# weiaicunzai/pytorch-camvid

Measured on AMD Instinct MI355X. Metric: images/sec fwd+bwd UNet 3x360x480 bs=8, higher is better.
Workload: dtype f32; 1 GPU; UNET(3,12) train fwd+bwd+CE, per-GPU batch 8 x 3x360x480 fp32 (BASELINE.json configs[1]); global_batch=8, parallelism=dp1

## Files before the change

include/cvk.h:

```cpp
#ifndef CVK_H
#define CVK_H

#include <stddef.h>
#include <stdint.h>

#ifdef __cplusplus
extern "C" {
#endif

#define CVK_VERSION 100
#define CVK_OK 0
#define CVK_EINVAL (-1)
#define CVK_EWORKSPACE (-2)
#define CVK_STAT_ROWS 64

typedef struct cvk_view {
    float*  ptr;
    int64_t sN, sY, sX;
} cvk_view;

typedef struct cvk_viewh {
    void*   ptr;
    int64_t sN, sY, sX;
} cvk_viewh;

int         cvk_version(void);
uint64_t    cvk_abi_hash(void);
const char* cvk_last_error_string(void);

int cvk_import_nchw(const float* src, int64_t sN, int64_t sC, int64_t sH, int64_t sW,
                    float* dst, int ld, int N, int C, int H, int W, void* stream);
int cvk_export_nchw(const float* src, int ld, float* dst, int64_t dN, int64_t dC, int64_t dH, int64_t dW,
                    int N, int C, int H, int W, void* stream);
int cvk_zero_frame(cvk_view buf, int N, int H, int W, int C, int y0, int x0, int h, int w, void* stream);

int cvk_conv3x3_fwd(const float* x, const float* w, const float* bias, float* y, float* stats,
                    int N, int H, int W, int Cin, int Cout, int ldy, void* stream);
int cvk_pack_weight_fwd(const float* w_src, float* dst, int Cout, int Cin, int Cin_pad, void* stream);
int cvk_pack_weight_dgrad(const float* w_src, float* dst, int Cout, int Cin, int Cin_pad, int Cout_pad, void* stream);
size_t cvk_conv3x3_wgrad_workspace_bytes(int N, int H, int W, int Cin_pad, int Cout);
int cvk_conv3x3_wgrad(const float* x, const float* dy, float* dw, int N, int H, int W, int Cin, int Cin_pad,
                      int Cout, int ld_dy, void* workspace, size_t workspace_bytes, void* stream);

int cvk_wino_weight_transform(const float* w, float* U, int Cout, int Cin, void* stream);
size_t cvk_conv3x3_wino_workspace_bytes(int N, int H, int W, int Cout_ld);
int cvk_conv3x3_wino_gemm(const float* x, const float* U, float* Mo, int N, int H, int W, int Cin, int Cout, int ldm,
                          void* stream);
int cvk_wino_output(const float* Mo, const float* bias, float* y, float* stats, int N, int H, int W, int Cout, int ldy,
                    void* stream);

int cvk_wino4_weight_transform(const float* w, float* U, int Cout, int Cin, void* stream);
int cvk_wino4_weight_transform_dgrad(const float* w, float* U, int Cout, int Cin, void* stream);
int cvk_conv3x3_wino4_ksplit(int N, int H, int W, int Cin, int Cout_ld);
size_t cvk_conv3x3_wino4_workspace_bytes(int N, int H, int W, int Cin, int Cout_ld);
int cvk_conv3x3_wino4_gemm(const float* x, const float* U, float* Mo, int N, int H, int W, int Cin, int Cout, int ldm,
                           void* stream);
int cvk_wino4_output(const float* Mo, const float* bias, float* y, float* stats, int N, int H, int W, int Cout, int ldy,
                     int ksplit, void* stream);

int cvk_w2d_tiles(int N, int H, int W);
int cvk_w2d_tpad(int T);
int cvk_w2d_stat_partials(int N, int H, int W);
size_t cvk_conv3x3_w2d_workspace_bytes(int N, int H, int W, int Cin, int Cout);
int cvk_w2d_weight_transform(const float* w, float* U, int Cout, int Cin, void* stream);
int cvk_w2d_weight_transform_dgrad(const float* w, float* U, int Cout, int Cin, void* stream);
int cvk_conv3x3_w2d(const float* x, const float* U, const float* bias, float* y, float* stats, float* counts, int N, int H,
                    int W, int Cin, int Cout, int ldy, void* workspace, size_t workspace_bytes, void* stream);
int cvk_w2d_ksplit(int T, int Cin, int Cout);
int cvk_w2d_input_transform(const float* x, float* V, int N, int H, int W, int Cin, void* stream);
int cvk_w2d_gemm(const float* V, const float* U, float* Mo, int T, int Cin, int Cout, void* stream);
int cvk_w2d_output(const float* Mo, const float* bias, float* y, float* stats, float* counts, int N, int H, int W, int Cin,
                   int Cout, int ldy, void* stream);
size_t cvk_conv3x3_wgrad_w2d_workspace_bytes(int N, int H, int W, int Cin_pad, int Cout);
int cvk_conv3x3_wgrad_w2d(const float* x, const float* dy, float* dw, int N, int H, int W, int Cin, int Cin_pad, int Cout,
                          int ld_dy, void* workspace, size_t workspace_bytes, void* stream);
int cvk_w2d_wgrad_ksplit(int T, int Cin_pad, int Cout);
int cvk_w2d_dy_transform(const float* dy, int ld_dy, float* E, int N, int H, int W, int Cout, void* stream);
int cvk_w2d_dy_transform_both(const float* dy, int ld_dy, float* Vp, float* E, int N, int H, int W, int Cout, void* stream);
int cvk_w2d_gemm_tn(const float* E, const float* V, float* P, int T, int Cin_pad, int Cout, void* stream);
int cvk_w2d_wgrad_output(const float* P, float* dw, int T, int Cin, int Cin_pad, int Cout, void* stream);

int cvk_w6_tiles(int N, int H, int W);
int cvk_w6_stat_partials(int N, int H, int W);
size_t cvk_conv3x3_w6_workspace_bytes(int N, int H, int W, int Cin, int Cout);
int cvk_w6_weight_transform(const float* w, float* U, int Cout, int Cin, void* stream);
int cvk_w6_weight_transform_dgrad(const float* w, float* U, int Cout, int Cin, void* stream);
int cvk_w6_ksplit(int T, int Cin, int Cout);
int cvk_w6_input_transform(const float* x, float* V, int N, int H, int W, int Cin, void* stream);
int cvk_w6_gemm(const float* V, const float* U, float* Mo, int T, int Cin, int Cout, void* stream);
int cvk_w6_output(const float* Mo, const float* bias, float* y, float* stats, float* counts, int N, int H, int W, int Cin,
                  int Cout, int ldy, void* stream);
int cvk_w6_wgrad_ksplit(int T, int Cin_pad, int Cout);
int cvk_w6_dy_transform(const float* dy, int ld_dy, float* E, int N, int H, int W, int Cout, void* stream);
int cvk_w6_dy_transform_both(const float* dy, int ld_dy, float* Vp, float* E, int N, int H, int W, int Cout, void* stream);
int cvk_w6_gemm_tn(const float* E, const float* V, float* P, int T, int Cin_pad, int Cout, void* stream);
int cvk_split3_rows_pad(int R, int mult);
int cvk_split3_planes(const float* P, void* S, int NX, int R, int Rpad, int C, void* stream);
int cvk_w2d_gemm_split3(const void* V3, const void* U3, float* Mo, int NX, int T, int Tpad, int Cin, int Cout, int Cpad, void* stream);
int cvk_amax_block_words(void);
unsigned cvk_amax_block_value(const unsigned* host_words, int n);
int cvk_absmax_f32(const float* x, long rows, int C, int ld, void* amax_block, void* stream);
int cvk_split_scale_exponent(int tile, int kind, int xi, unsigned amax_block);
int cvk_split_planes(int fmt, int tile, int kind, const float* P, void* S, const void* amax, int NX, int R, int Rpad, int C, void* stream);
int cvk_w2d_gemm_split(int fmt, int tile, const void* V, const void* U, float* Mo, const void* amax_v, const void* amax_u, int NX, int T, int Tpad,
                       int Cin, int Cout, int Cpad, void* stream);
int cvk_w2d_input_transform_split3(int tile, const float* x, void* V3, int N, int H, int W, int Cin, void* stream);
int cvk_w2d_dy_transform_both_split3(int tile, const float* dy, int ld_dy, void* Vp3, void* E, int e_split, int N, int H, int W, int C,
                                     void* stream);
int cvk_w2d_weight_transform_split3(int tile, const float* w, void* U3, float* tmp, int Cout, int Cin, int dgrad, void* stream);
int cvk_w2d_input_transform_split(int fmt, int tile, const float* x, void* V, const void* amax_x, int N, int H, int W, int Cin, void* stream);
int cvk_w2d_dy_transform_both_split(int fmt, int tile, const float* dy, int ld_dy, void* Vp, void* E, int e_split, const void* amax_dy, int N, int H,
                                    int W, int C, void* stream);
int cvk_w2d_weight_transform_split(int fmt, int tile, const float* w, void* U, const void* amax_w, int Cout, int Cin, int dgrad, void* stream);
int cvk_w2d_output_plain(int tile, const float* Mo, const float* bias, float* y, float* stats, float* counts, int N, int H, int W,
                         int Cout, int ldy, void* stream);
int cvk_w2d_gemm_tn_split3_ksplit(int NX, int Tpad, int Cin, int Cout);
int cvk_w2d_gemm_tn_split3(const void* E3, const void* V3, float* P, int NX, int Tpad, int Cin, int Cout, void* stream);
int cvk_w2d_gemm_tn_split(int fmt, int tile, const void* E, const void* V, float* P, const void* amax_e, const void* amax_v, int NX, int Tpad, int Cin,
                          int Cout, void* stream);
int cvk_w2d_wgrad_output_f(int tile, const float* P, float* dw, int Cin, int Cin_pad, int Cout, int f, void* stream);
int cvk_w6_wgrad_output(const float* P, float* dw, int T, int Cin, int Cin_pad, int Cout, void* stream);
int cvk_wino4h_weight_transform(const float* w, void* Uh, const void* amax_w, int Cn, int Ck, int dgrad, void* stream);
int cvk_conv3x3_wino4h(const float* x, const void* Uh, const float* bias, float* y, float* stats, float* counts, const void* amax_x,
                       const void* amax_w, int N, int H, int W, int Cin, int Cout, int ldy, int max_workgroups, void* stream);
int cvk_conv3x3_wino4h_bnred(const float* x, const void* Uh, float* y, const void* amax_x, const void* amax_w, int N, int H, int W, int Cin,
                             int Cout, int ldy, const float* yP, const float* scale, const float* shift, const float* mean,
                             const float* rstd, float* part, int max_workgroups, void* stream);
size_t cvk_wino4f_weight_floats(int Cn, int Ck);
int cvk_wino4f_weight_transform(const float* w, float* Uf, int Cn, int Ck, int dgrad, void* stream);
#define CVK_WT_BATCH_MAX 48
typedef struct cvk_wt_job { const float* w; float* out; int rows, cols, tile, dgrad; } cvk_wt_job;
int cvk_wino4f_weight_transform_batch(const cvk_wt_job* jobs, int n, void* stream);
int cvk_w2d_weight_transform_batch(const cvk_wt_job* jobs, int n, void* stream);
int cvk_wino4f_stat_partials(int N, int H, int W);
int cvk_conv3x3_wino4f_vplanes(const float* x, const float* Uf, const float* bias, float* y, float* stats, float* counts, float* Vsm,
                               int N, int H, int W, int Cin, int Cout, int ldy, int max_workgroups, void* stream);
int cvk_conv3x3_wino4f(const float* x, const float* Uf, const float* bias, float* y, float* stats, float* counts, int N, int H,
                       int W, int Cin, int Cout, int ldy, int max_workgroups, void* stream);
int cvk_conv3x3_wino4f_bnred(const float* x, const float* Uf, float* y, int N, int H, int W, int Cin, int Cout, int ldy,
                             const float* yP, const float* scale, const float* shift, const float* mean, const float* rstd,
                             float* part, int max_workgroups, void* stream);

int cvk_thin_fwd_supported(int Cin_ld, int Cout, int ldy);
int cvk_thin_stat_partials(int N, int H, int W, int Cin_ld);
int cvk_conv3x3_thin_fwd(const float* x, const float* w, const float* bias, float* y, float* stats, float* counts, int N, int H,
                         int W, int Cin_ld, int Cout, int ldy, void* stream);
int cvk_thin_wgrad_supported(int Cin, int Cin_ld, int Cout, int ld_dy);
size_t cvk_conv3x3_thin_wgrad_workspace_bytes(int N, int H, int W, int Cin_ld, int Cout);
int cvk_conv3x3_thin_wgrad(const float* x, const float* dy, float* dw, int N, int H, int W, int Cin, int Cin_ld, int Cout,
                           int ld_dy, void* workspace, size_t workspace_bytes, void* stream);

size_t cvk_conv3x3_wgradp_workspace_bytes(int N, int H, int W, int Cin_pad, int Cout);
int cvk_conv3x3_wgradp(const float* x, const float* dy, const float* E6_pre, float* dw, int N, int H, int W, int Cin, int Cin_pad,
                       int Cout, int ld_dy, void* workspace, size_t workspace_bytes, void* stream);
long cvk_wgradp_plane_rows(int N, int H, int W);
int cvk_wgradp_planes(const float* t, int ld, float* planes, int N, int H, int W, int C, int is_dy, void* stream);
size_t cvk_wgradp_gemm_workspace_bytes(int N, int H, int W, int Cin_pad, int Cout);
int cvk_wgradp_gemm(const float* E6, const float* V6, float* dw, int N, int H, int W, int Cin, int Cin_pad, int Cout, void* workspace,
                    size_t workspace_bytes, void* stream);
int cvk_wgradp_zero_pads(float* planes, int N, int H, int W, int C, void* stream);
int cvk_wgradp_zero_pads_sm(float* planes, int N, int H, int W, int C, void* stream);
int cvk_wgradp_planes_sm(const float* x, int ld, float* planes, int N, int H, int W, int C, void* stream);
int cvk_wgradp_gemm_sm(const float* E6, const float* V6sm, float* dw, int N, int H, int W, int Cin, int Cin_pad, int Cout, void* workspace,
                       size_t workspace_bytes, void* stream);
int cvk_wgradp_zero_pads4(float* planes, int N, int H, int W, int C, void* stream);
int cvk_bn_bwd_dx_e4p(cvk_view dout, const float* y, int ldy, const float* scale, const float* shift, const float* mean,
                      const float* rstd, const float* dgamma, const float* dbeta, float* dy, int ld_dy, float* E4p, float* part,
                      int N, int H, int W, int C, int use_batch_stats, void* stream);
int cvk_wgradp_dy_slack(int W);
int cvk_wgradp_gemm_sm_dy(const float* E4p, const float* dy, const float* V6sm, float* dw, int N, int H, int W, int Cin, int Cin_pad, int Cout,
                          void* workspace, size_t workspace_bytes, void* stream);
int cvk_bn_bwd_dx_e6(cvk_view dout, const float* y, int ldy, const float* scale, const float* shift, const float* mean,
                     const float* rstd, const float* dgamma, const float* dbeta, float* dy, int ld_dy, float* E6, float* part,
                     int N, int H, int W, int C, int use_batch_stats, void* stream);

size_t cvk_conv3x3_wgrad_wino4_workspace_bytes(int N, int H, int W, int Cin_pad, int Cout, int ld_dy);
int cvk_conv3x3_wgrad_wino4(const float* x, const float* dy, const float* E_pre, float* dw, int N, int H, int W, int Cin,
                            int Cin_pad, int Cout, int ld_dy, void* workspace, size_t workspace_bytes, void* stream);
int cvk_bn_bwd_e_blocks(int N, int H, int W);
int cvk_bn_bwd_dx_e(cvk_view dout, const float* y, int ldy, const float* scale, const float* shift, const float* mean,
                    const float* rstd, const float* dgamma, const float* dbeta, float* dy, int ld_dy, float* E, float* part,
                    int N, int H, int W, int C, int use_batch_stats, void* stream);

size_t cvk_conv3x3_wgrad_wino_workspace_bytes(int N, int H, int W, int Cin_pad, int Cout);
int cvk_conv3x3_wgrad_wino(const float* x, const float* dy, float* dw, int N, int H, int W, int Cin, int Cin_pad,
                           int Cout, int ld_dy, void* workspace, size_t workspace_bytes, void* stream);

size_t cvk_bn_finalize_workspace_bytes(int P, int C);
int cvk_bn_finalize(const float* stats, int P, int M, int C, const float* gamma, const float* beta,
                    float* mean, float* rstd, float* scale, float* shift,
                    float* running_mean, float* running_var, int64_t* num_batches_tracked,
                    float momentum, float eps, void* workspace, size_t workspace_bytes, void* stream);
int cvk_bn_eval_params(const float* gamma, const float* beta, const float* running_mean, const float* running_var,
                       float* mean, float* rstd, float* scale, float* shift, int C, float eps, void* stream);
int cvk_bn_relu_apply(const float* y, int ldy, const float* scale, const float* shift, cvk_view out,
                      int N, int H, int W, int C, void* stream);
int cvk_bn_relu_apply_pool(const float* y, int ldy, const float* scale, const float* shift, cvk_view out, float* pool,
                           unsigned char* code, int N, int H, int W, int C, void* stream);
int cvk_bn_bwd_blocks(int M);
int cvk_bn_bwd_reduce(cvk_view dout, const float* y, int ldy, const float* scale, const float* shift,
                      const float* mean, const float* rstd, float* part, int N, int H, int W, int C, void* stream);
int cvk_colsum_finalize(const float* part, int PB, int C, float* out0, float* out1, void* stream);
#define CVK_COLSUM_BATCH_MAX 64
typedef struct cvk_colsum_job { const float* part; float* out; int PB, C; } cvk_colsum_job;
int cvk_colsum_finalize_batch(const cvk_colsum_job* jobs, int n, void* stream);
int cvk_bn_relu_apply_amax(const float* y, int ldy, const float* scale, const float* shift, cvk_view out, int N, int H, int W, int C,
                           void* amax_block, void* stream);
int cvk_bn_relu_apply_pool_amax(const float* y, int ldy, const float* scale, const float* shift, cvk_view out, float* pool,
                                unsigned char* code, int N, int H, int W, int C, void* amax_out, void* amax_pool, void* stream);
int cvk_bn_bwd_dx_e_amax(int six, cvk_view dout, const float* y, int ldy, const float* scale, const float* shift, const float* mean,
                         const float* rstd, const float* dgamma, const float* dbeta, float* dy, int ld_dy, float* E, float* part, int N, int H,
                         int W, int C, int use_batch_stats, void* amax_block, void* stream);
int cvk_bn_bwd_dx_amax(cvk_view dout, const float* y, int ldy, const float* scale, const float* shift, const float* mean,
                       const float* rstd, const float* dgamma, const float* dbeta, float* dy, int ld_dy, float* dbias_part, int N,
                       int H, int W, int C, int use_batch_stats, void* amax_block, void* stream);
int cvk_bn_bwd_dx(cvk_view dout, const float* y, int ldy, const float* scale, const float* shift,
                  const float* mean, const float* rstd, const float* dgamma, const float* dbeta,
                  float* dy, int ld_dy, float* dbias_part, int N, int H, int W, int C, int use_batch_stats, void* stream);

int cvk_maxpool2x2_fwd(cvk_view x, float* out, uint8_t* code, int N, int H, int W, int C, void* stream);
int cvk_maxpool2x2_bwd(const float* dout, cvk_view x, const uint8_t* code, cvk_view dx, int accumulate,
                       int N, int H, int W, int C, void* stream);
int cvk_maxpool2x2_bwd_bnred_blocks(int N, int H, int W, int C);
int cvk_maxpool2x2_bwd_bnred(const float* dout, cvk_view x, const uint8_t* code, cvk_view dx, int accumulate, int N, int H, int W, int C,
                             const float* yP, int ldp, const float* scale, const float* shift, const float* mean, const float* rstd,
                             float* part, void* stream);
int cvk_maxunpool2x2_fwd(const float* v, const uint8_t* code, float* out, int N, int H, int W, int C, void* stream);
int cvk_maxunpool2x2_bwd(const float* dout, const uint8_t* code, float* dv, int N, int H, int W, int C, void* stream);
int cvk_pool_code_to_index(const uint8_t* code, int64_t* idx, int N, int H, int W, int C, void* stream);

int cvk_bilinear_up2_fwd(const float* x, float* out, int N, int H, int W, int C, void* stream);
int cvk_bilinear_up2_bwd(const float* dout, float* dx, int N, int H, int W, int C, void* stream);

int cvk_ce_blocks(int M);
int cvk_softmax_ce_fwd(const float* logits, int ld, const int64_t* target, float* part, float* loss,
                       int M, int C, int ignore_index, void* stream);
int cvk_softmax_ce_bwd(const float* logits, int ld, const int64_t* target, const float* loss3, const float* grad_out,
                       float scale, float* dlogits, int ld_d, int M, int C, int ignore_index, void* stream);

#define CVK_REDUCTION_NONE 0
#define CVK_REDUCTION_MEAN 1
#define CVK_REDUCTION_SUM 2
int cvk_ce_ex_part_floats(int M);
int cvk_softmax_ce_fwd_ex(const float* logits, int ld, const int64_t* target, const float* weight, float label_smoothing,
                          int reduction, float* part, float* loss, float* loss_px, int M, int C, int ignore_index, void* stream);
int cvk_softmax_ce_bwd_ex(const float* logits, int ld, const int64_t* target, const float* weight, float label_smoothing,
                          int reduction, const float* loss4, const float* grad_out, float scale, float* dlogits, int ld_d,
                          int M, int C, int ignore_index, void* stream);

#define CVK_DICE_PRESENT 0
#define CVK_DICE_ALL 1
int cvk_seg_loss_part_floats(int M, int C);
int cvk_seg_loss_record_floats(int C);
int cvk_seg_loss_fwd(const float* logits, int ld, const int64_t* target, const float* weight, float ce, float dice, float focal_gamma,
// ... 208 lines not shown
```

pytorch-camvid_amd/_lib.py:

```python
import ctypes
import os
import subprocess
import threading

_HERE = os.path.dirname(os.path.abspath(__file__))
LIB_PATH = os.environ.get("CVK_LIB_PATH") or os.path.join(_HERE, "lib", "libcvk.so")
CSRC = os.path.join(_HERE, "csrc")
HEADER = os.path.join(os.path.dirname(_HERE), "include", "cvk.h")

CVK_STAT_ROWS = 64

c_f32p = ctypes.c_void_p
c_i64 = ctypes.c_int64
c_int = ctypes.c_int
c_size = ctypes.c_size_t
c_float = ctypes.c_float
c_vp = ctypes.c_void_p


class View(ctypes.Structure):
    _fields_ = [("ptr", ctypes.c_void_p), ("sN", ctypes.c_int64), ("sY", ctypes.c_int64), ("sX", ctypes.c_int64)]


class ViewH(ctypes.Structure):
    _fields_ = [("ptr", ctypes.c_void_p), ("sN", ctypes.c_int64), ("sY", ctypes.c_int64), ("sX", ctypes.c_int64)]


SIGNATURES = {
    "cvk_version": (c_int, []),
    "cvk_abi_hash": (ctypes.c_uint64, []),
    "cvk_last_error_string": (ctypes.c_char_p, []),
    "cvk_import_nchw": (c_int, [c_vp, c_i64, c_i64, c_i64, c_i64, c_vp, c_int, c_int, c_int, c_int, c_int, c_vp]),
    "cvk_export_nchw": (c_int, [c_vp, c_int, c_vp, c_i64, c_i64, c_i64, c_i64, c_int, c_int, c_int, c_int, c_vp]),
    "cvk_zero_frame": (c_int, [View, c_int, c_int, c_int, c_int, c_int, c_int, c_int, c_int, c_vp]),
    "cvk_conv3x3_fwd": (c_int, [c_vp, c_vp, c_vp, c_vp, c_vp, c_int, c_int, c_int, c_int, c_int, c_int, c_vp]),
    "cvk_pack_weight_fwd": (c_int, [c_vp, c_vp, c_int, c_int, c_int, c_vp]),
    "cvk_pack_weight_dgrad": (c_int, [c_vp, c_vp, c_int, c_int, c_int, c_int, c_vp]),
    "cvk_conv3x3_wgrad_workspace_bytes": (c_size, [c_int, c_int, c_int, c_int, c_int]),
    "cvk_conv3x3_wgrad": (c_int, [c_vp, c_vp, c_vp, c_int, c_int, c_int, c_int, c_int, c_int, c_int, c_vp, c_size, c_vp]),
    "cvk_wino_weight_transform": (c_int, [c_vp, c_vp, c_int, c_int, c_vp]),
    "cvk_conv3x3_wino_workspace_bytes": (c_size, [c_int, c_int, c_int, c_int]),
    "cvk_conv3x3_wino_gemm": (c_int, [c_vp, c_vp, c_vp, c_int, c_int, c_int, c_int, c_int, c_int, c_vp]),
    "cvk_wino_output": (c_int, [c_vp, c_vp, c_vp, c_vp, c_int, c_int, c_int, c_int, c_int, c_vp]),
    "cvk_wino4_weight_transform": (c_int, [c_vp, c_vp, c_int, c_int, c_vp]),
    "cvk_wino4_weight_transform_dgrad": (c_int, [c_vp, c_vp, c_int, c_int, c_vp]),
    "cvk_conv3x3_wino4_ksplit": (c_int, [c_int, c_int, c_int, c_int, c_int]),
    "cvk_conv3x3_wino4_workspace_bytes": (c_size, [c_int, c_int, c_int, c_int, c_int]),
    "cvk_conv3x3_wino4_gemm": (c_int, [c_vp, c_vp, c_vp, c_int, c_int, c_int, c_int, c_int, c_int, c_vp]),
    "cvk_wino4_output": (c_int, [c_vp, c_vp, c_vp, c_vp, c_int, c_int, c_int, c_int, c_int, c_int, c_vp]),
    "cvk_wino4f_weight_floats": (c_size, [c_int, c_int]),
    "cvk_wino4f_weight_transform": (c_int, [c_vp, c_vp, c_int, c_int, c_int, c_vp]),
    "cvk_wino4f_weight_transform_batch": (c_int, [c_vp, c_int, c_vp]),
    "cvk_w2d_weight_transform_batch": (c_int, [c_vp, c_int, c_vp]),
    "cvk_wino4f_stat_partials": (c_int, [c_int, c_int, c_int]),
    "cvk_conv3x3_wino4f": (c_int, [c_vp, c_vp, c_vp, c_vp, c_vp, c_vp, c_int, c_int, c_int, c_int, c_int, c_int, c_int, c_vp]),
    "cvk_conv3x3_wino4f_bnred": (c_int, [c_vp, c_vp, c_vp, c_int, c_int, c_int, c_int, c_int, c_int, c_vp, c_vp, c_vp, c_vp, c_vp, c_vp, c_int, c_vp]),
    "cvk_wino4h_weight_transform": (c_int, [c_vp, c_vp, c_vp, c_int, c_int, c_int, c_vp]),
    "cvk_conv3x3_wino4h": (c_int, [c_vp, c_vp, c_vp, c_vp, c_vp, c_vp, c_vp, c_vp, c_int, c_int, c_int, c_int, c_int, c_int, c_int, c_vp]),
    "cvk_conv3x3_wino4h_bnred": (c_int, [c_vp, c_vp, c_vp, c_vp, c_vp, c_int, c_int, c_int, c_int, c_int, c_int, c_vp, c_vp, c_vp, c_vp, c_vp, c_vp,
                                         c_int, c_vp]),
    "cvk_thin_fwd_supported": (c_int, [c_int, c_int, c_int]),
    "cvk_thin_stat_partials": (c_int, [c_int, c_int, c_int, c_int]),
    "cvk_conv3x3_thin_fwd": (c_int, [c_vp, c_vp, c_vp, c_vp, c_vp, c_vp, c_int, c_int, c_int, c_int, c_int, c_int, c_vp]),
    "cvk_thin_wgrad_supported": (c_int, [c_int, c_int, c_int, c_int]),
    "cvk_conv3x3_thin_wgrad_workspace_bytes": (c_size, [c_int, c_int, c_int, c_int, c_int]),
    "cvk_conv3x3_thin_wgrad": (c_int, [c_vp, c_vp, c_vp, c_int, c_int, c_int, c_int, c_int, c_int, c_int, c_vp, c_size, c_vp]),
    "cvk_conv3x3_wgradp_workspace_bytes": (c_size, [c_int, c_int, c_int, c_int, c_int]),
    "cvk_conv3x3_wgradp": (c_int, [c_vp, c_vp, c_vp, c_vp, c_int, c_int, c_int, c_int, c_int, c_int, c_int, c_vp, c_size, c_vp]),
    "cvk_wgradp_plane_rows": (ctypes.c_long, [c_int, c_int, c_int]),
    "cvk_wgradp_planes": (c_int, [c_vp, c_int, c_vp, c_int, c_int, c_int, c_int, c_int, c_vp]),
    "cvk_wgradp_gemm_workspace_bytes": (c_size, [c_int, c_int, c_int, c_int, c_int]),
    "cvk_wgradp_gemm": (c_int, [c_vp, c_vp, c_vp, c_int, c_int, c_int, c_int, c_int, c_int, c_vp, c_size, c_vp]),
    "cvk_wgradp_zero_pads": (c_int, [c_vp, c_int, c_int, c_int, c_int, c_vp]),
    "cvk_wgradp_zero_pads_sm": (c_int, [c_vp, c_int, c_int, c_int, c_int, c_vp]),
    "cvk_wgradp_planes_sm": (c_int, [c_vp, c_int, c_vp, c_int, c_int, c_int, c_int, c_vp]),
    "cvk_wgradp_gemm_sm": (c_int, [c_vp, c_vp, c_vp, c_int, c_int, c_int, c_int, c_int, c_int, c_vp, c_size, c_vp]),
    "cvk_wgradp_zero_pads4": (c_int, [c_vp, c_int, c_int, c_int, c_int, c_vp]),
    "cvk_bn_bwd_dx_e4p": (c_int, [View, c_vp, c_int, c_vp, c_vp, c_vp, c_vp, c_vp, c_vp, c_vp, c_int, c_vp, c_vp,
                                  c_int, c_int, c_int, c_int, c_int, c_vp]),
    "cvk_wgradp_dy_slack": (c_int, [c_int]),
    "cvk_wgradp_gemm_sm_dy": (c_int, [c_vp, c_vp, c_vp, c_vp, c_int, c_int, c_int, c_int, c_int, c_int, c_vp, c_size, c_vp]),
    "cvk_conv3x3_wino4f_vplanes": (c_int, [c_vp, c_vp, c_vp, c_vp, c_vp, c_vp, c_vp, c_int, c_int, c_int, c_int, c_int, c_int, c_int, c_vp]),
    "cvk_bn_bwd_dx_e6": (c_int, [View, c_vp, c_int, c_vp, c_vp, c_vp, c_vp, c_vp, c_vp, c_vp, c_int, c_vp, c_vp,
                                 c_int, c_int, c_int, c_int, c_int, c_vp]),
    "cvk_w2d_tiles": (c_int, [c_int, c_int, c_int]),
    "cvk_w6_tiles": (c_int, [c_int, c_int, c_int]),
    "cvk_w6_stat_partials": (c_int, [c_int, c_int, c_int]),
    "cvk_conv3x3_w6_workspace_bytes": (c_size, [c_int, c_int, c_int, c_int, c_int]),
    "cvk_w6_weight_transform": (c_int, [c_vp, c_vp, c_int, c_int, c_vp]),
    "cvk_w6_weight_transform_dgrad": (c_int, [c_vp, c_vp, c_int, c_int, c_vp]),
    "cvk_w6_input_transform": (c_int, [c_vp, c_vp, c_int, c_int, c_int, c_int, c_vp]),
    "cvk_w6_gemm": (c_int, [c_vp, c_vp, c_vp, c_int, c_int, c_int, c_vp]),
    "cvk_w6_wgrad_ksplit": (c_int, [c_int, c_int, c_int]),
    "cvk_w6_dy_transform": (c_int, [c_vp, c_int, c_vp, c_int, c_int, c_int, c_int, c_vp]),
    "cvk_w6_gemm_tn": (c_int, [c_vp, c_vp, c_vp, c_int, c_int, c_int, c_vp]),
    "cvk_w6_wgrad_output": (c_int, [c_vp, c_vp, c_int, c_int, c_int, c_int, c_vp]),
    "cvk_w6_ksplit": (c_int, [c_int, c_int, c_int]),
    "cvk_w6_output": (c_int, [c_vp, c_vp, c_vp, c_vp, c_vp, c_int, c_int, c_int, c_int, c_int, c_int, c_vp]),
    "cvk_w2d_stat_partials": (c_int, [c_int, c_int, c_int]),
    "cvk_conv3x3_w2d_workspace_bytes": (c_size, [c_int, c_int, c_int, c_int, c_int]),
    "cvk_w2d_weight_transform": (c_int, [c_vp, c_vp, c_int, c_int, c_vp]),
    "cvk_w2d_weight_transform_dgrad": (c_int, [c_vp, c_vp, c_int, c_int, c_vp]),
    "cvk_w2d_input_transform": (c_int, [c_vp, c_vp, c_int, c_int, c_int, c_int, c_vp]),
    "cvk_w2d_gemm": (c_int, [c_vp, c_vp, c_vp, c_int, c_int, c_int, c_vp]),
    "cvk_conv3x3_wgrad_w2d_workspace_bytes": (c_size, [c_int, c_int, c_int, c_int, c_int]),
    "cvk_conv3x3_wgrad_w2d": (c_int, [c_vp, c_vp, c_vp, c_int, c_int, c_int, c_int, c_int, c_int, c_int, c_vp, c_size, c_vp]),
    "cvk_w2d_tpad": (c_int, [c_int]),
    "cvk_split3_rows_pad": (c_int, [c_int, c_int]),
    "cvk_split3_planes": (c_int, [c_vp, c_vp, c_int, c_int, c_int, c_int, c_vp]),
    "cvk_w2d_gemm_split3": (c_int, [c_vp, c_vp, c_vp, c_int, c_int, c_int, c_int, c_int, c_int, c_vp]),
    "cvk_w2d_input_transform_split3": (c_int, [c_int, c_vp, c_vp, c_int, c_int, c_int, c_int, c_vp]),
    "cvk_w2d_dy_transform_both_split3": (c_int, [c_int, c_vp, c_int, c_vp, c_vp, c_int, c_int, c_int, c_int, c_int, c_vp]),
    "cvk_w2d_weight_transform_split3": (c_int, [c_int, c_vp, c_vp, c_vp, c_int, c_int, c_int, c_vp]),
    "cvk_w2d_output_plain": (c_int, [c_int, c_vp, c_vp, c_vp, c_vp, c_vp, c_int, c_int, c_int, c_int, c_int, c_vp]),
    "cvk_w2d_gemm_tn_split3_ksplit": (c_int, [c_int, c_int, c_int, c_int]),
    "cvk_w2d_gemm_tn_split3": (c_int, [c_vp, c_vp, c_vp, c_int, c_int, c_int, c_int, c_vp]),
    "cvk_amax_block_words": (c_int, []),
    "cvk_amax_block_value": (ctypes.c_uint, [c_vp, c_int]),
    "cvk_absmax_f32": (c_int, [c_vp, ctypes.c_long, c_int, c_int, c_vp, c_vp]),
    "cvk_split_scale_exponent": (c_int, [c_int, c_int, c_int, ctypes.c_uint]),
    "cvk_split_planes": (c_int, [c_int, c_int, c_int, c_vp, c_vp, c_vp, c_int, c_int, c_int, c_int, c_vp]),
    "cvk_w2d_gemm_split": (c_int, [c_int, c_int, c_vp, c_vp, c_vp, c_vp, c_vp, c_int, c_int, c_int, c_int, c_int, c_int, c_vp]),
    "cvk_w2d_input_transform_split": (c_int, [c_int, c_int, c_vp, c_vp, c_vp, c_int, c_int, c_int, c_int, c_vp]),
    "cvk_w2d_dy_transform_both_split": (c_int, [c_int, c_int, c_vp, c_int, c_vp, c_vp, c_int, c_vp, c_int, c_int, c_int, c_int, c_vp]),
    "cvk_w2d_weight_transform_split": (c_int, [c_int, c_int, c_vp, c_vp, c_vp, c_int, c_int, c_int, c_vp]),
    "cvk_w2d_gemm_tn_split": (c_int, [c_int, c_int, c_vp, c_vp, c_vp, c_vp, c_vp, c_int, c_int, c_int, c_int, c_vp]),
    "cvk_w2d_wgrad_output_f": (c_int, [c_int, c_vp, c_vp, c_int, c_int, c_int, c_int, c_vp]),
    "cvk_w2d_wgrad_ksplit": (c_int, [c_int, c_int, c_int]),
    "cvk_w2d_dy_transform": (c_int, [c_vp, c_int, c_vp, c_int, c_int, c_int, c_int, c_vp]),
    "cvk_w2d_dy_transform_both": (c_int, [c_vp, c_int, c_vp, c_vp, c_int, c_int, c_int, c_int, c_vp]),
    "cvk_w6_dy_transform_both": (c_int, [c_vp, c_int, c_vp, c_vp, c_int, c_int, c_int, c_int, c_vp]),
    "cvk_w2d_gemm_tn": (c_int, [c_vp, c_vp, c_vp, c_int, c_int, c_int, c_vp]),
    "cvk_w2d_wgrad_output": (c_int, [c_vp, c_vp, c_int, c_int, c_int, c_int, c_vp]),
    "cvk_w2d_ksplit": (c_int, [c_int, c_int, c_int]),
    "cvk_w2d_output": (c_int, [c_vp, c_vp, c_vp, c_vp, c_vp, c_int, c_int, c_int, c_int, c_int, c_int, c_vp]),
    "cvk_conv3x3_w2d": (c_int, [c_vp, c_vp, c_vp, c_vp, c_vp, c_vp, c_int, c_int, c_int, c_int, c_int, c_int, c_vp, c_size, c_vp]),
    "cvk_conv3x3_wgrad_wino4_workspace_bytes": (c_size, [c_int, c_int, c_int, c_int, c_int, c_int]),
    "cvk_conv3x3_wgrad_wino4": (c_int, [c_vp, c_vp, c_vp, c_vp, c_int, c_int, c_int, c_int, c_int, c_int, c_int, c_vp, c_size, c_vp]),
    "cvk_bn_bwd_e_blocks": (c_int, [c_int, c_int, c_int]),
    "cvk_bn_bwd_dx_e": (c_int, [View, c_vp, c_int, c_vp, c_vp, c_vp, c_vp, c_vp, c_vp, c_vp, c_int, c_vp, c_vp,
                                c_int, c_int, c_int, c_int, c_int, c_vp]),
    "cvk_conv3x3_wgrad_wino_workspace_bytes": (c_size, [c_int, c_int, c_int, c_int, c_int]),
    "cvk_conv3x3_wgrad_wino": (c_int, [c_vp, c_vp, c_vp, c_int, c_int, c_int, c_int, c_int, c_int, c_int, c_vp, c_size, c_vp]),
    "cvk_bn_finalize_workspace_bytes": (c_size, [c_int, c_int]),
    "cvk_bn_finalize": (c_int, [c_vp, c_int, c_int, c_int, c_vp, c_vp, c_vp, c_vp, c_vp, c_vp, c_vp, c_vp, c_vp,
                                c_float, c_float, c_vp, c_size, c_vp]),
    "cvk_bn_eval_params": (c_int, [c_vp, c_vp, c_vp, c_vp, c_vp, c_vp, c_vp, c_vp, c_int, c_float, c_vp]),
    "cvk_bn_relu_apply": (c_int, [c_vp, c_int, c_vp, c_vp, View, c_int, c_int, c_int, c_int, c_vp]),
    "cvk_bn_relu_apply_pool": (c_int, [c_vp, c_int, c_vp, c_vp, View, c_vp, c_vp, c_int, c_int, c_int, c_int, c_vp]),
    "cvk_bn_bwd_blocks": (c_int, [c_int]),
    "cvk_bn_bwd_reduce": (c_int, [View, c_vp, c_int, c_vp, c_vp, c_vp, c_vp, c_vp, c_int, c_int, c_int, c_int, c_vp]),
    "cvk_colsum_finalize": (c_int, [c_vp, c_int, c_int, c_vp, c_vp, c_vp]),
    "cvk_colsum_finalize_batch": (c_int, [c_vp, c_int, c_vp]),
    "cvk_bn_bwd_dx": (c_int, [View, c_vp, c_int, c_vp, c_vp, c_vp, c_vp, c_vp, c_vp, c_vp, c_int, c_vp,
                              c_int, c_int, c_int, c_int, c_int, c_vp]),
    "cvk_bn_relu_apply_amax": (c_int, [c_vp, c_int, c_vp, c_vp, View, c_int, c_int, c_int, c_int, c_vp, c_vp]),
    "cvk_bn_relu_apply_pool_amax": (c_int, [c_vp, c_int, c_vp, c_vp, View, c_vp, c_vp, c_int, c_int, c_int, c_int, c_vp, c_vp, c_vp]),
    "cvk_bn_bwd_dx_e_amax": (c_int, [c_int, View, c_vp, c_int, c_vp, c_vp, c_vp, c_vp, c_vp, c_vp, c_vp, c_int, c_vp, c_vp,
                                     c_int, c_int, c_int, c_int, c_int, c_vp, c_vp]),
    "cvk_bn_bwd_dx_amax": (c_int, [View, c_vp, c_int, c_vp, c_vp, c_vp, c_vp, c_vp, c_vp, c_vp, c_int, c_vp,
                                   c_int, c_int, c_int, c_int, c_int, c_vp, c_vp]),
    "cvk_maxpool2x2_fwd": (c_int, [View, c_vp, c_vp, c_int, c_int, c_int, c_int, c_vp]),
    "cvk_maxpool2x2_bwd": (c_int, [c_vp, View, c_vp, View, c_int, c_int, c_int, c_int, c_int, c_vp]),
    "cvk_maxpool2x2_bwd_bnred_blocks": (c_int, [c_int, c_int, c_int, c_int]),
# ... 227 lines not shown
```

pytorch-camvid_amd/conv_fp32.py:

```python
import torch

from . import _lib
from ._lib import check
from .engine import _BF16, _F32, Op, Saved, _empty, _timed, amax_blocks, channels_last
from .route import pad4


def w2fn(lib, tile, name):
    return getattr(lib, ("cvk_w6_" if tile == 6 else "cvk_w2d_") + name)


_PLANE_DT = {0: _F32, 2: torch.float16, 3: _BF16}


def planes2d(lib, tile, N, H, W, fmt=0):
    T = w2fn(lib, tile, "tiles")(N, H, W)
    return 64 if tile == 6 else 36, T, lib.cvk_split3_rows_pad(T, 256) if fmt else lib.cvk_w2d_tpad(T)


def plane_elems(NX, Tp, C, fmt=0):
    return NX * (C // 32) * fmt * Tp * 32 if fmt else NX * Tp * C + 128


def absmax(R, t, rows, cols, ld, s, what):
# ... 114 lines not shown
        return (P2, cnt) if self.sp is not None else None

    def w4f(self, vplanes=False, bnred=None, h2=False, x_amax=None):
        R, lib, s, x, d, wt = self.R, self.lib, self.s, self.x, self.dgrad_of, self.wt
        N, H, W, M, k_ch, cout, ldy, flops = self.N, self.H, self.W, self.M, self.k_ch, self.cout, self.ldy, self.flops
        floats, dg, f = lib.cvk_wino4f_weight_floats(cout, k_ch), int(d is not None), "h" if h2 else "f"
        am_w = self._amax_w() if h2 else None

        def build():
            u, name = _empty(floats, x.device), "cvk_wino4%s_weight_transform" % f
            _timed(R, "k_wino4%s_weight" % f, 4.0 * (9 + 18) * cout * k_ch, lambda: check(getattr(lib, name)(
                wt.data_ptr(), u.data_ptr(), *((am_w.data_ptr(),) if h2 else ()), cout, k_ch, dg, s), name + ("(dgrad)" if dg and not h2 else "")), "byte")
            return u
        U = self._filter("w4" + f, build, None if h2 else ("w4f", floats, cout, k_ch, 0, dg))
        am = ()
        if h2:
            am_x = x_amax if x_amax is not None else absmax(R, x, M, k_ch, k_ch, s, "x")
            am = (am_x.data_ptr(), am_w.data_ptr())
        executed = (1.5 if h2 else 0.5) * flops
        Pf = lib.cvk_wino4f_stat_partials(N, H, W)
        cnt = self._counts(Pf)
        if bnred is not None:
            bpart = _empty(2 * Pf * cout, x.device)
            name = "cvk_conv3x3_wino4%s_bnred" % f
            _timed(R, "k_conv3x3_wino4%s<bnred>" % f, flops, lambda: check(getattr(lib, name)(
                x.data_ptr(), U.data_ptr(), self.y.data_ptr(), *am, N, H, W, k_ch, cout, ldy, *bnred, bpart.data_ptr(), R.launch_wgs(), s), name), executed=executed)
            self.bnred_sums = (bpart, Pf)
            return None
        if vplanes:
            self.v = _empty(6 * lib.cvk_wgradp_plane_rows(N, H, W) * k_ch, x.device)
            check(lib.cvk_wgradp_zero_pads_sm(self.v.data_ptr(), N, H, W, k_ch, s), "cvk_wgradp_zero_pads_sm")
            _timed(R, "k_conv3x3_wino4f<vplanes>", flops, lambda: check(
                lib.cvk_conv3x3_wino4f_vplanes(x.data_ptr(), U.data_ptr(), self.bias, self.y.data_ptr(), self.sp, cnt, self.v.data_ptr(), N, H, W,
                                               k_ch, cout, ldy, R.launch_wgs(), s), "cvk_conv3x3_wino4f_vplanes" + self.what), executed=executed)
        else:
            name = "cvk_conv3x3_wino4" + f
            _timed(R, "k_conv3x3_wino4" + f, flops, lambda: check(getattr(lib, name)(
                x.data_ptr(), U.data_ptr(), self.bias, self.y.data_ptr(), self.sp, cnt, *am, N, H, W, k_ch, cout, ldy, R.launch_wgs(), s),
                name + self.what), executed=executed)
        return (Pf, cnt) if self.sp is not None else None

    def w4(self):
        R, lib, s, x, d = self.R, self.lib, self.s, self.x, self.dgrad_of
        N, H, W, M, k_ch, cout, ldy = self.N, self.H, self.W, self.M, self.k_ch, self.cout, self.ldy

        dg = d is not None and d[1] == k_ch and d[2] == cout

        def build():
            u, wt = _empty(6 * cout * 3 * k_ch, x.device), d[0] if dg else (self.w() if callable(self.w) else self.w)
            kind = "weight_transform_dgrad" if dg else "weight_transform"
            _timed(R, "k_wino4_weight_dgrad" if dg else "k_wino4_weight", 4.0 * (9 + 18) * cout * k_ch, lambda: check(getattr(lib, "cvk_wino4_" + kind)(
                wt.data_ptr(), u.data_ptr(), *((d[1], d[2]) if dg else (cout, k_ch)), s), "cvk_wino4_" + kind), "byte")
            return u
        U = self._filter("w4", build)
        ws = R.workspace(lib.cvk_conv3x3_wino4_workspace_bytes(N, H, W, k_ch, ldy), x.device)
        ksplit = lib.cvk_conv3x3_wino4_ksplit(N, H, W, k_ch, ldy)
        _timed(R, conv_kernel_name("wino4", ldy), self.flops, lambda: check(
            lib.cvk_conv3x3_wino4_gemm(x.data_ptr(), U.data_ptr(), ws.data_ptr(), N, H, W, k_ch, cout, ldy, s), "cvk_conv3x3_wino4_gemm" + self.what))
        _timed(R, "k_wino4_output", (4.0 + 6.0 * ksplit) * M * ldy, lambda: check(
            lib.cvk_wino4_output(ws.data_ptr(), self.bias, self.y.data_ptr(), self.sp, N, H, W, cout, ldy, ksplit, s), "cvk_wino4_output"), "byte")

    def w2(self):
        R, lib, s, x = self.R, self.lib, self.s, self.x
        N, H, W, M, k_ch, cout, ldy = self.N, self.H, self.W, self.M, self.k_ch, self.cout, self.ldy

        def build():
            wt = self.w() if callable(self.w) else self.w
            u = _empty(4 * cout * 3 * k_ch, x.device)
            _timed(R, "k_wino_weight", 4.0 * (9 + 12) * cout * k_ch, lambda: check(
                lib.cvk_wino_weight_transform(wt.data_ptr(), u.data_ptr(), cout, k_ch, s), "cvk_wino_weight_transform"), "byte")
            return u
        U = self._filter("w", build)
        ws = R.workspace(lib.cvk_conv3x3_wino_workspace_bytes(N, H, W, ldy), x.device)
        _timed(R, conv_kernel_name("wino", ldy), self.flops, lambda: check(
            lib.cvk_conv3x3_wino_gemm(x.data_ptr(), U.data_ptr(), ws.data_ptr(), N, H, W, k_ch, cout, ldy, s), "cvk_conv3x3_wino_gemm" + self.what))
        _timed(R, "k_wino_output", 12.0 * M * ldy, lambda: check(
            lib.cvk_wino_output(ws.data_ptr(), self.bias, self.y.data_ptr(), self.sp, N, H, W, cout, ldy, s), "cvk_wino_output"), "byte")


class WeightGrad:

    def __init__(self, R, s, x, dy, gw, N, H, W, cin, k_ch, cout, ldy, flops):
        self.R, self.lib, self.s, self.x, self.dy, self.gw = R, R.lib, s, x, dy, gw
        self.N, self.H, self.W, self.M, self.cin, self.k_ch, self.cout, self.ldy, self.flops = N, H, W, N * H * W, cin, k_ch, cout, ldy, flops

    def run(self, fam, tile=0, fmt=0, V=None, am_v=None, E=None, dy_e=False, Eb=None, am_dy=None):
        if fam == "w2d":
            return self.w2d(tile, V, Eb)
        if fam == "w2d_split":
            return self.w2d_split(tile, fmt, V, am_v, Eb, am_dy)
        if fam in ("wgradp", "wgradp_sm"):
            return self.wgradp(fam == "wgradp", V, E, dy_e and E is not None)
        return self.w4(E) if fam == "w4" else self.direct(fam)

    def w2d(self, tile, V, Eb):
        R, lib, s, x, dy = self.R, self.lib, self.s, self.x, self.dy
        N, H, W, M, k_ch, C, ldy = self.N, self.H, self.W, self.M, self.k_ch, self.cout, self.ldy
        NX, T, Tp = planes2d(lib, tile, N, H, W)
        efl = plane_elems(NX, Tp, C)
        f = w2fn(lib, tile, "wgrad_ksplit")(T, k_ch, C)
        if V is None:
            V = _empty(plane_elems(NX, Tp, k_ch), x.device)
            _timed(R, "k_w2d_input", 4.0 * (M + NX * T) * k_ch, lambda: check(
                w2fn(lib, tile, "input_transform")(x.data_ptr(), V.data_ptr(), N, H, W, k_ch, s), "cvk_w2d_input_transform(wgrad)"), "byte")
        ws = R.workspace(4 * ((0 if Eb is not None else efl) + f * NX * C * k_ch), x.device)
        Ep, Pp = (Eb.data_ptr(), ws.data_ptr()) if Eb is not None else (ws.data_ptr(), ws.data_ptr() + 4 * efl)
        if Eb is None:
            _timed(R, "k_w2d_dy", 4.0 * (M + NX * T) * C, lambda: check(
                w2fn(lib, tile, "dy_transform")(dy.data_ptr(), ldy, Ep, N, H, W, C, s), "cvk_w2d_dy_transform"), "byte")
        _timed(R, "k_w2d_gemm_tn", self.flops, lambda: check(
            w2fn(lib, tile, "gemm_tn")(Ep, V.data_ptr(), Pp, T, k_ch, C, s), "cvk_w2d_gemm_tn"), executed=2.0 * NX * Tp * k_ch * C)
        _timed(R, "k_w2d_wgrad_out", 4.0 * (NX * f + 9) * C * self.cin, lambda: check(
            w2fn(lib, tile, "wgrad_output")(Pp, self.gw, T, self.cin, k_ch, C, s), "cvk_w2d_wgrad_output"), "byte")

    def w2d_split(self, tile, fmt, V, am_v, Eb, am_dy):
        R, lib, s, k_ch, C = self.R, self.lib, self.s, self.k_ch, self.cout
        NX, _, Tp = planes2d(lib, tile, self.N, self.H, self.W, fmt)
        f = lib.cvk_w2d_gemm_tn_split3_ksplit(NX, Tp, k_ch, C)
        ws = R.workspace(4 * f * NX * C * k_ch, self.x.device)
        _timed(R, "k_gemm_tn_" + ("split3" if fmt == 3 else "split2h"), self.flops, lambda: check(
            lib.cvk_w2d_gemm_tn_split(fmt, tile, Eb.data_ptr(), V.data_ptr(), ws.data_ptr(), am_dy.data_ptr() if am_dy is not None else None,
                                      am_v.data_ptr() if am_v is not None else None, NX, Tp, k_ch, C, s), "cvk_w2d_gemm_tn_split"),
            executed=2.0 * (6 if fmt == 3 else 3) * NX * Tp * k_ch * C)
        _timed(R, "k_w2d_wgrad_out", 4.0 * (NX * f + 9) * C * self.cin, lambda: check(
            lib.cvk_w2d_wgrad_output_f(tile, ws.data_ptr(), self.gw, self.cin, k_ch, C, f, s), "cvk_w2d_wgrad_output_f"), "byte")

    def wgradp(self, own_v, V, E, sm_dy):
        R, lib, s, x, dy = self.R, self.lib, self.s, self.x, self.dy
        N, H, W, M, k_ch, C, ldy = self.N, self.H, self.W, self.M, self.k_ch, self.cout, self.ldy
        rows6 = lib.cvk_wgradp_plane_rows(N, H, W)
        wsb = lib.cvk_wgradp_gemm_workspace_bytes(N, H, W, k_ch, C)
        nE = 0 if E is not None else 6 * rows6 * C
        nV = 6 * rows6 * k_ch if own_v else 0
        ws = R.workspace(4 * (nV + nE) + wsb, x.device)
        V6p = ws.data_ptr() if own_v else V.data_ptr()
        E6p = E.data_ptr() if E is not None else ws.data_ptr() + 4 * nV
        slabp = ws.data_ptr() + 4 * (nV + nE)
        if own_v:
            _timed(R, "k_wgradp_planes", 4.0 * (M + 6.0 * rows6) * k_ch, lambda: check(
                lib.cvk_wgradp_planes(x.data_ptr(), k_ch, V6p, N, H, W, k_ch, 0, s), "cvk_wgradp_planes(x)"), "byte")
        if E is None:
            _timed(R, "k_wgradp_planes", 4.0 * (M + 6.0 * rows6) * C, lambda: check(
                lib.cvk_wgradp_planes(dy.data_ptr(), ldy, E6p, N, H, W, C, 1, s), "cvk_wgradp_planes(dy)"), "byte")
        fn = "cvk_wgradp_gemm_sm_dy" if sm_dy else ("cvk_wgradp_gemm" if own_v else "cvk_wgradp_gemm_sm")
        ev = (E6p, dy.data_ptr(), V6p) if sm_dy else (E6p, V6p)
        _timed(R, "k_wgradp_gemm", self.flops, lambda: check(getattr(lib, fn)(*ev, self.gw, N, H, W, self.cin, k_ch, C, slabp, wsb, s), fn),
               executed=9.0 * M * C * self.cin)

    def w4(self, E):
        R, lib, N, H, W, k_ch, C, ldy = self.R, self.lib, self.N, self.H, self.W, self.k_ch, self.cout, self.ldy
        wsb = lib.cvk_conv3x3_wgrad_wino4_workspace_bytes(N, H, W, k_ch, C, ldy)
        ws = R.workspace(wsb, self.x.device)
        _timed(R, f"k_wgrad_wino4<{'128' if C > 64 else '64'}, 128, 2, 2>", self.flops, lambda: check(
            lib.cvk_conv3x3_wgrad_wino4(self.x.data_ptr(), self.dy.data_ptr(), E.data_ptr() if E is not None else None, self.gw, N, H, W,
                                        self.cin, k_ch, C, ldy, ws.data_ptr(), wsb, self.s), "cvk_conv3x3_wgrad_wino4"))

    def direct(self, fam):
        R, lib, N, H, W, M, k_ch, C, ldy = self.R, self.lib, self.N, self.H, self.W, self.M, self.k_ch, self.cout, self.ldy
        fn = {"thin": "cvk_conv3x3_thin_wgrad", "w2": "cvk_conv3x3_wgrad_wino", "direct": "cvk_conv3x3_wgrad"}[fam]
        wsb = getattr(lib, fn + "_workspace_bytes")(N, H, W, k_ch, C)
        ws = R.workspace(wsb, self.x.device)
        head = k_ch == 64
        name, kw = {"thin": ("k_thin_co_wgrad" if head else "k_thin_ci_wgrad",
                             dict(executed=18.0 * M * (16 * self.cin if head else C * 16 / 3.0), nbytes=4.0 * M * (k_ch + ldy))),
                    "w2": (f"k_wgrad_wino<{'128' if C > 64 else '64'}, 128, 2, 2>", {}), "direct": (conv_kernel_name("wgrad", C, k_ch), {})}[fam]
        _timed(R, name, self.flops, lambda: check(getattr(lib, fn)(
            self.x.data_ptr(), self.dy.data_ptr(), self.gw, N, H, W, self.cin, k_ch, C, ldy, ws.data_ptr(), wsb, self.s), fn), **kw)


def conv_kernel_name(kind, n_cols, k_ch=32):
    if kind in ("wino4", "wino"):
        return "k_conv3x3_%s<%s>" % (kind, "128, 128, 2, 2" if n_cols > 64 else ("128, 64, 2, 2" if n_cols > 32 else "128, 32, 4, 1"))
    if kind == "wgrad":
        if n_cols <= 16 and k_ch == 64:
            return "k_wgrad_smallco"
        t = "128, 128, 2, 2" if n_cols > 64 else ("64, 128, 2, 2" if n_cols > 32 else "32, 256, 1, 4")
        if 32 < n_cols <= 64 and k_ch * 9 <= 64:
            t = "64, 64, 2, 2"
        return f"k_conv3x3_wgrad<{t}>"
    t = "128, 128, 2, 2" if n_cols > 64 else ("128, 64, 2, 2" if n_cols > 32 else "256, 32, 4, 1")
    return f"k_conv3x3_igemm<{t}, {'true' if kind == 'fwd' else 'false'}, {'true' if k_ch % 32 == 0 else 'false'}>"


class ConvBnRelu(Op):
    _pitch, _ydt = staticmethod(pad4), _F32
# ... 121 lines not shown
            P, Pw = self._stat_partials(R, wk)
            stats = _empty(2 * Pw * C + Pw, dev)
        counted, kept = self._conv(R, st, rt, st.act[src.id], wk, b, y, stats, P)
        self._bn_params(R, st, stats, counted, P, Pw, gamma, beta, ptrs)
        self._bn_apply(R, st, y, ptrs[2], ptrs[3])
        if st.need_grad and self.active:
            st.saved[self.idx] = Saved(y, bnp, rt, kept)

    def _bn_sums(self, R, st, bn, gg, gbe):
        lib, s, src, C, (blocks, fn, name) = R.lib, st.stream, self.src, self.cout, self._BN
        PB = getattr(lib, blocks)(src.M)
        part = _empty(2 * PB * C, st.device)
        pre = st.bnred.pop(self.idx, None)
        if pre is not None:
            check(lib.cvk_colsum_finalize(pre[0].data_ptr(), pre[1], C, gbe, gg, s), "cvk_colsum_finalize")
        elif self.bn_train or self.g_req or self.be_req:
            _timed(R, name, float(self.dst.buf.esize + self._ydt.itemsize) * src.M * C, lambda: check(
                getattr(lib, fn)(*bn, part.data_ptr(), src.N, src.H, src.W, C, s), fn), "byte")
            check(lib.cvk_colsum_finalize(part.data_ptr(), PB, C, gbe, gg, s), "cvk_colsum_finalize")
        if self.w_req or self.b_req or self.src_needs_grad:
            return part, PB
        R.grads_ready(st, self.pslot)
        return None

    _BN_E = {"dx+E": (0, "cvk_bn_bwd_dx_e", 16.0), "dx+E6": (1, "cvk_bn_bwd_dx_e6", 24.0), "dx+E4p": (2, "cvk_bn_bwd_dx_e4p", 16.0)}

    def _bn_bwd(self, R, st, rt, bn, gg, gbe, part, PB, gb):
        lib, s, src, kind = R.lib, st.stream, self.src, rt.bn_bwd
        N, H, W, M, C, ldy = src.N, src.H, src.W, src.M, self.cout, pad4(self.cout)
        if kind == "dx+E4p":
            dyb = _empty(M * ldy + lib.cvk_wgradp_dy_slack(W) * ldy, st.device)
            dyb[M * ldy:].zero_()
            dy = dyb[:M * ldy]
        else:
            dy = torch.zeros(M * ldy, device=st.device, dtype=_F32) if ldy != C else _empty(M * ldy, st.device)
        want_amax = rt.dy_amax and bool(st.amax_spare)
        head, tail = (*bn, gg, gbe, dy.data_ptr(), ldy), (part.data_ptr(), N, H, W, C, 1 if self.bn_train else 0)
        if kind != "dx":
            mode, plain, eb = self._BN_E[kind]
            if kind == "dx+E":
                E = _empty(4 * N * H * ((W + 3) // 4) * ldy, st.device)
            else:
                E = _empty((4 if mode == 2 else 6) * lib.cvk_wgradp_plane_rows(N, H, W) * C, st.device)
                check((lib.cvk_wgradp_zero_pads4 if mode == 2 else lib.cvk_wgradp_zero_pads)(E.data_ptr(), N, H, W, C, s), "cvk_wgradp_zero_pads")
            blk = st.amax_spare[-1] if want_amax else None
            rc = _timed(R, "k_bn_bwd<%s>" % kind, (12.0 * M + eb * N * H * ((W + 3) // 4)) * C, lambda: (
                lib.cvk_bn_bwd_dx_e_amax(mode, *head, E.data_ptr(), *tail, blk.data_ptr(), s) if blk is not None
                else getattr(lib, plain)(*head, E.data_ptr(), *tail, s)), "byte")
            if rc == 0:
                if gb is not None:
                    R.defer_colsum(st, part, lib.cvk_bn_bwd_e_blocks(N, H, W), C, gb)
                return dy, E, (st.amax_spare.pop() if blk is not None else None)
        am = st.amax_spare.pop() if want_amax else None
        _timed(R, "k_bn_bwd<dx>", 12.0 * M * C, lambda: check(amax_call(lib, "cvk_bn_bwd_dx", (*head, *tail), (am,), s), "cvk_bn_bwd_dx"), "byte")
        if gb is not None:
            R.defer_colsum(st, part, PB, C, gb)
        return dy, None, am

    def _dy_both(self, R, st, rt, dy, am_dy):
        if rt is None or not rt.dy_both:
            return None, None, am_dy
        lib, s, src = R.lib, st.stream, self.src
        N, H, W, M, C, ldy = src.N, src.H, src.W, src.M, self.cout, pad4(self.cout)
        tile, fmt = rt.tile, rt.split
        NX, T, Tp = planes2d(lib, tile, N, H, W, fmt)
        Eb, Vb = (torch.empty(plane_elems(NX, Tp, C, fmt), device=st.device, dtype=_PLANE_DT[fmt]) for _ in range(2))
        if fmt:
            if fmt == 2 and am_dy is None:
                am_dy = absmax(R, dy, M, C, ldy, s, "dy")
            _timed(R, "k_w2d_dy<both,%s>" % ("split3" if fmt == 3 else "split2h"), (4.0 * M + 4.0 * fmt * NX * T) * C, lambda: check(
                lib.cvk_w2d_dy_transform_both_split(fmt, tile, dy.data_ptr(), ldy, Vb.data_ptr(), Eb.data_ptr(), 1,
                                                    am_dy.data_ptr() if am_dy is not None else None, N, H, W, C, s), "cvk_w2d_dy_transform_both_split"), "byte")
        else:
            _timed(R, "k_w2d_dy<both>", 4.0 * (M + 2 * NX * T) * C, lambda: check(
                w2fn(lib, tile, "dy_transform_both")(dy.data_ptr(), ldy, Vb.data_ptr(), Eb.data_ptr(), N, H, W, C, s), "cvk_w2d_dy_transform_both"), "byte")
        return Eb, Vb, am_dy

    def _data_grad(self, R, st, rt, dy, Vb, am_dy):
        lib, s, src = R.lib, st.stream, self.src
        N, H, W, M, C, ldy, dev = src.N, src.H, src.W, src.M, self.cout, pad4(self.cout), st.device
        flops = 18.0 * M * C * self.cin
        if src.id in st.grad:
            raise NotImplementedError("conv data-grad must be the first writer of its input's gradient buffer")
        w = st.params[4 * self.pslot]
        wc = channels_last(w)

        def packed():
            wd_ = _empty(src.ld * 9 * ldy, dev)
            _timed(R, "k_pack_weight_dgrad", 4.0 * 9 * (C * self.cin + src.ld * ldy), lambda: check(
                lib.cvk_pack_weight_dgrad(wc.data_ptr(), wd_.data_ptr(), C, self.cin, src.ld, ldy, s), "cvk_pack_weight_dgrad"), "byte")
            return wd_
        dX = _empty(M * src.ld, dev).view(N, H, W, src.ld)
        wd = R.derived(((self.pslot, "d"), "pack"), w, packed) if rt.dgrad in ("thin", "direct") else None
        if rt.dgrad == "thin":
            _timed(R, "k_thin_ci_fwd(dgrad)", flops, lambda: check(
                lib.cvk_conv3x3_thin_fwd(dy.data_ptr(), wd.data_ptr(), None, dX.data_ptr(), None, None, N, H, W, ldy, src.ld, src.ld, s),
                "cvk_conv3x3_thin_fwd(dgrad)"), executed=18.0 * M * ldy * src.ld, nbytes=4.0 * M * (src.ld + ldy))
        elif rt.dgrad == "direct":
            _timed(R, conv_kernel_name("dgrad", src.ld, ldy), flops, lambda: check(
                lib.cvk_conv3x3_fwd(dy.data_ptr(), wd.data_ptr(), None, dX.data_ptr(), None, N, H, W, ldy, src.ld, src.ld, s), "cvk_conv3x3_fwd(dgrad)"))
        else:
            prod = st.plan.sole_producer(src) if rt.dgrad_bnred else None
            bnred = None
            if prod is not None and prod.bn_train and prod.idx in st.saved and pad4(prod.cout) == prod.cout == src.ld:
                bnred = st.saved[prod.idx].pointers(src.ld)
            c = WinoConv(R, s, dy, packed, None, dX, None, N, H, W, ldy, src.ld, src.ld, flops, w, (self.pslot, "d"), "(dgrad)", dgrad_of=(wc, C, self.cin))
            c.run(rt.dgrad, rt.dgrad_tile, rt.split, v_pre=Vb, x_amax=am_dy, bnred=bnred)
            if c.bnred_sums is not None:
                st.bnred[prod.idx] = c.bnred_sums
        st.grad[src.id] = dX

    def _dout(self, st):
        return (self.dst.cview(st.grad[self.dst.buf.id]),)

    def _weight_grad(self, R, st, saved, dy, gw, E, Eb, am_dy):
        src, rt = self.src, saved.rt
        WeightGrad(R, st.stream, st.act[src.id], dy, gw, src.N, src.H, src.W, self.cin, src.ld, self.cout, pad4(self.cout),
                   18.0 * src.M * self.cout * self.cin).run(rt.wgrad, rt.tile, rt.split, *(saved.kept or (None, None)), E, rt.bn_bwd == "dx+E4p", Eb, am_dy)

    def bwd(self, R, st):
        saved = st.saved.pop(self.idx, None)
        if not self.active:
            return
        rt, ld = saved.rt, self._pitch(self.cout)
        gw, gb, gg, gbe = self._grad_targets(R, st, ld)
        yp, *bnp = saved.pointers(ld)
        bn = (*self._dout(st), yp, ld, *bnp)
        sums = self._bn_sums(R, st, bn, gg, gbe)
        if sums is None:
            return
        dy, E, am_dy = self._bn_bwd(R, st, rt, bn, gg, gbe, *sums, gb)
        Eb, Vb, am_dy = self._dy_both(R, st, rt, dy, am_dy)
        if self.src_needs_grad:
            self._data_grad(R, st, rt, dy, Vb, am_dy)
        if gw is not None:
            self._weight_grad(R, st, saved, dy, gw, E, Eb, am_dy)
        R.grads_ready(st, self.pslot)
```

pytorch-camvid_amd/csrc/wgradp.hip:

```cpp
#include "conv_tile.h"
#include "lds_dma.h"
#include <utility>

namespace {

template <int... Ks, class F>
__device__ __forceinline__ void p_static_for(std::integer_sequence<int, Ks...>, F&& f) {
    (f(std::integral_constant<int, Ks>{}), ...);
}

__device__ __forceinline__ void p_dma16(const void* sbase, unsigned voff, unsigned lds_byte_addr) {
    asm volatile("s_mov_b32 m0, %2\n\ts_nop 0\n\tglobal_load_lds_dwordx4 %0, %1" : : "v"(voff), "s"(sbase), "s"(lds_byte_addr) : "memory");
}

__host__ __device__ inline long p_rows(int N, int H, int Wtp) { return (long)N * (H + 2) * Wtp + 2L * Wtp; }

template <int MODE, bool SM = false>
__global__ __launch_bounds__(256) void k_wgradp_planes(const float* __restrict__ X, int ld, float* __restrict__ P, int N, int H, int W,
                                                      int Wt, int Wtp, int C) {
    const int cvn = C >> 2;
    const long rows = p_rows(N, H, Wtp);
    const long idx = (long)blockIdx.x * 256 + threadIdx.x;
    if (idx >= rows * cvn) return;
    const long row = idx / cvn;
    const int c = (int)(idx - row * cvn) * 4;
    const f32x4 z = {0.f, 0.f, 0.f, 0.f};
    f32x4 v[6] = {z, z, z, z, z, z};
    const long q = row - Wtp;
    if (q >= 0 && q < (long)N * (H + 2) * Wtp) {
        const int xt = (int)(q % Wtp);
        const long ry = q / Wtp;
        const int yp = (int)(ry % (H + 2)), n = (int)(ry / (H + 2));
        if (yp >= 1 && yp <= H && xt < Wt) {
            const float* p = X + (((size_t)n * H + (yp - 1)) * W + 4 * (size_t)xt) * ld + c;
            if (MODE == 0) {
                f32x4 d[6];
#pragma unroll
                for (int j = 0; j < 6; ++j) {
                    const int col = 4 * xt - 1 + j;
                    d[j] = (col >= 0 && col < W) ? *reinterpret_cast<const f32x4*>(p + (long)(j - 1) * ld) : z;
                }
                const f32x4 a = d[4] - 4.f * d[2], b = d[3] - 4.f * d[1], e = d[4] - d[2], f = d[3] - d[1];
                v[0] = 4.f * d[0] - 5.f * d[2] + d[4];
                v[1] = a + b;
                v[2] = a - b;
                v[3] = e + 2.f * f;
                v[4] = e - 2.f * f;
                v[5] = 4.f * d[1] - 5.f * d[3] + d[5];
            } else {
                f32x4 d[4];
#pragma unroll
                for (int i = 0; i < 4; ++i) d[i] = (4 * xt + i < W) ? *reinterpret_cast<const f32x4*>(p + (long)i * ld) : z;
                const f32x4 a = d[0] + d[2], b = d[1] + d[3], cc = d[0] + 4.f * d[2], dd = 2.f * d[1] + 8.f * d[3];
                v[0] = d[0];
                v[1] = a + b;
                v[2] = a - b;
                v[3] = cc + dd;
                v[4] = cc - dd;
                v[5] = d[3];
            }
        }
    }
    float* o = SM ? P + ((size_t)(c >> 4) * rows + (size_t)row) * 16 + (c & 15) : P + (size_t)row * C + c;
    const size_t ps = (size_t)rows * C;
#pragma unroll
    for (int x = 0; x < 6; ++x) *reinterpret_cast<f32x4*>(o + x * ps) = v[x];
}

template <bool SM = false>
__global__ __launch_bounds__(256) void k_wgradp_zero_pads(float* __restrict__ P, int N, int H, int Wt, int Wtp, int C, int nplanes) {
    const int cvn = C >> 2;
    const long rows = p_rows(N, H, Wtp);
    const int padc = Wtp - Wt;
    const long n_end = 2L * Wtp, n_border = (long)N * 2 * Wtp, n_col = (long)N * H * padc;
    const long idx = (long)blockIdx.x * 256 + threadIdx.x;
    const long pr = idx / cvn;
    const int c = (int)(idx - pr * cvn) * 4;
    if (pr >= n_end + n_border + n_col) return;
    long row;
    if (pr < n_end) {
        row = pr < Wtp ? pr : rows - Wtp + (pr - Wtp);
    } else if (pr < n_end + n_border) {
        const long k = pr - n_end;
        const int n = (int)(k / (2 * Wtp)), rem = (int)(k - (long)n * 2 * Wtp);
        const int yp = rem < Wtp ? 0 : H + 1, xt = rem < Wtp ? rem : rem - Wtp;
        row = (long)Wtp + ((long)n * (H + 2) + yp) * Wtp + xt;
    } else {
        const long k = pr - n_end - n_border;
        const long ry = k / padc;
        const int xt = Wt + (int)(k - ry * padc);
        const int n = (int)(ry / H), yy = (int)(ry - (long)n * H);
        row = (long)Wtp + ((long)n * (H + 2) + yy + 1) * Wtp + xt;
    }
    const f32x4 z = {0.f, 0.f, 0.f, 0.f};
    const size_t ps = (size_t)rows * C;
    for (int x = 0; x < nplanes; ++x)
        *reinterpret_cast<f32x4*>(P + x * ps + (SM ? ((size_t)(c >> 4) * rows + (size_t)row) * 16 + (c & 15) : (size_t)row * C + c)) = z;
}

template <bool VSM, bool EDY>
__global__ __launch_bounds__(64, 2) void k_wgradp_gemm(const float* __restrict__ E6, const float* __restrict__ V6, float* __restrict__ slab,
                                                      int H, int Wtp, int Cin_ld, int Cout, long rows, int Q, int runs, int nci, int nco,
                                                      const float* __restrict__ dy, int W) {
    __shared__ __attribute__((aligned(1024))) char smem[12 * 1024];
    const unsigned smem_addr = cvk_lds_addr(smem);
    const int lane = threadIdx.x;
    const int lj = lane & 15, kq = lane >> 4;

    const int per = 6 * nci * nco;
    const int id = cvk_xcd_remap(blockIdx.x, gridDim.x);
    const int run = id / per, u = id - run * per;
    const int xi = u % 6, cit = (u / 6) % nci, cot = u / (6 * nci);
    const int qb = (int)((long)run * Q / runs), qe = (int)((long)(run + 1) * Q / runs);
    if (qb >= qe) return;
    const int so = Wtp >> 3;

    const bool edy = EDY && (xi == 0 || xi == 5);
    const float* const Eb = edy ? dy + cot * 64 + (xi == 5 ? 3 * Cout : 0) : E6 + (size_t)(EDY ? xi - 1 : xi) * rows * Cout + cot * 64;
    const int epitch = edy ? 4 * Cout : Cout;
    const float* const Vb = V6 + (size_t)xi * rows * Cin_ld + (VSM ? (size_t)cit * 4 * rows * 16 : (size_t)cit * 64);
    const int vpitch = VSM ? 16 : Cin_ld;
    const unsigned evoff = (unsigned)(((lane >> 4) * epitch + (lane & 15) * 4) * 4);
    const unsigned vvoff = VSM ? (unsigned)((((unsigned long)((lane & 15) >> 2) * (unsigned long)rows + (lane >> 4)) * 16 + (lane & 3) * 4) * 4)
                               : (unsigned)(((lane >> 4) * Cin_ld + (lane & 15) * 4) * 4);
    auto block_row = [&](int strip, int yp) -> long {
        const int n = strip / so, xg = strip - n * so;
        return (long)Wtp + ((long)n * (H + 2) + yp) * Wtp + 8 * xg;
    };
    auto dma_V = [&](int strip, int yp) {
        const float* src = Vb + (size_t)block_row(strip, yp) * vpitch;
        const unsigned dst = smem_addr + (yp & 3) * 2048;
        p_dma16(src, vvoff, dst);
        p_dma16(src + 4 * (size_t)vpitch, vvoff, dst + 1024);
    };
    auto dma_E = [&](int strip, int yp, int slot) {
        const int en = strip / so, exg = strip - en * so;
        const float* src = edy ? Eb + (((size_t)en * H + (yp - 1)) * W + 32 * (size_t)exg) * Cout : Eb + (size_t)block_row(strip, yp) * Cout;
        const unsigned dst = smem_addr + 8192 + slot * 2048;
        p_dma16(src, evoff, dst);
        p_dma16(src + 4 * (size_t)epitch, evoff, dst + 1024);
    };

    f32x4 acc[3][16];
#pragma unroll
    for (int r = 0; r < 3; ++r)
#pragma unroll
        for (int b = 0; b < 16; ++b) acc[r][b] = f32x4{0.f, 0.f, 0.f, 0.f};

    const int frag = kq * 256 + lj * 16;

    int strip = qb / H, y = qb - strip * H;
    dma_V(strip, y);
    dma_V(strip, y + 1);
    dma_V(strip, y + 2);
    dma_E(strip, y + 1, 0);
    int es = 0;
    for (int q = qb; q < qe; ++q) {
        const bool last_in_strip = (y == H - 1);
        const bool more = q + 1 < qe;
        asm volatile("s_waitcnt lgkmcnt(0)" ::: "memory");
        if (more && !last_in_strip) {
            dma_V(strip, y + 3);
            dma_E(strip, y + 2, es ^ 1);
            cvk_wait_vm<4>();
        } else {
            cvk_wait_vm<0>();
        }
        __builtin_amdgcn_s_setprio(1);
        const char* const eblk = smem + 8192 + es * 2048;
        const char* const v0 = smem + ((y + 0) & 3) * 2048;
        const char* const v1 = smem + ((y + 1) & 3) * 2048;
        const char* const v2 = smem + ((y + 2) & 3) * 2048;
#pragma unroll
        for (int ks = 0; ks < 2; ++ks) {
            const f32x4 a = *reinterpret_cast<const f32x4*>(eblk + ks * 1024 + frag);
            const f32x4 b0 = *reinterpret_cast<const f32x4*>(v0 + ks * 1024 + frag);
            const f32x4 b1 = *reinterpret_cast<const f32x4*>(v1 + ks * 1024 + frag);
            const f32x4 b2 = *reinterpret_cast<const f32x4*>(v2 + ks * 1024 + frag);
#pragma unroll
            for (int i = 0; i < 4; ++i)
#pragma unroll
                for (int j = 0; j < 4; ++j) {
                    acc[0][i * 4 + j] = __builtin_amdgcn_mfma_f32_16x16x4f32(a[i], b0[j], acc[0][i * 4 + j], 0, 0, 0);
                    acc[1][i * 4 + j] = __builtin_amdgcn_mfma_f32_16x16x4f32(a[i], b1[j], acc[1][i * 4 + j], 0, 0, 0);
                    acc[2][i * 4 + j] = __builtin_amdgcn_mfma_f32_16x16x4f32(a[i], b2[j], acc[2][i * 4 + j], 0, 0, 0);
                }
        }
        __builtin_amdgcn_s_setprio(0);
        if (more) {
            if (last_in_strip) {
                ++strip;
                y = 0;
                asm volatile("s_waitcnt lgkmcnt(0)" ::: "memory");
                dma_V(strip, 0);
                dma_V(strip, 1);
                dma_V(strip, 2);
                dma_E(strip, 1, es ^ 1);
            } else {
                ++y;
            }
            es ^= 1;
        }
    }

    const int K3 = 3 * Cin_ld;
    float* const out = slab + ((size_t)(run * 6 + xi) * Cout + cot * 64) * K3 + cit * 64 + 4 * lj;
#pragma unroll
    for (int r = 0; r < 3; ++r)
#pragma unroll
        for (int i = 0; i < 4; ++i)
#pragma unroll
            for (int e = 0; e < 4; ++e) {
                const int co = 4 * (4 * kq + e) + i;
                const f32x4 v = {acc[r][i * 4 + 0][e], acc[r][i * 4 + 1][e], acc[r][i * 4 + 2][e], acc[r][i * 4 + 3][e]};
                *reinterpret_cast<f32x4*>(out + (size_t)co * K3 + r * Cin_ld) = v;
            }
}

__global__ __launch_bounds__(1024) void k_wgradp_reduce(const float* __restrict__ slab, float* __restrict__ dw, int runs, int Cout, int Cin,
                                                       int Cin_pad) {
    __shared__ float red[6][16][64];
    const int o = threadIdx.x & 63, g = threadIdx.x >> 6;
    const size_t total = (size_t)Cout * 3 * Cin;
    const size_t i = (size_t)blockIdx.x * 64 + o;
    const size_t plane = (size_t)Cout * 3 * Cin_pad;
    const bool ok = i < total;
    const int ci = ok ? (int)(i % Cin) : 0;
    const size_t cr = ok ? i / Cin : 0;
    const float* p = slab + cr * Cin_pad + ci;
    float P[6] = {0.f, 0.f, 0.f, 0.f, 0.f, 0.f};
    if (ok)
        for (int s = g; s < runs; s += 16) {
#pragma unroll
            for (int x = 0; x < 6; ++x) P[x] += p[((size_t)s * 6 + x) * plane];
        }
#pragma unroll
    for (int x = 0; x < 6; ++x) red[x][g][o] = P[x];
    __syncthreads();
    if (g == 0 && ok) {
#pragma unroll
        for (int x = 0; x < 6; ++x) {
            float a = 0.f;
#pragma unroll
            for (int k = 0; k < 16; ++k) a += red[x][k][o];
            P[x] = a;
        }
        const float s12 = P[1] + P[2], d12 = P[2] - P[1], s34 = P[3] + P[4], d34 = P[3] - P[4];
        float* out = dw + (cr * 3) * Cin + ci;
        out[0] = 0.25f * P[0] - s12 * (1.f / 6.f) + s34 * (1.f / 24.f);
        out[Cin] = d12 * (1.f / 6.f) + d34 * (1.f / 12.f);
        out[2 * (size_t)Cin] = (s34 - s12) * (1.f / 6.f) + P[5];
    }
}

struct PPlan { int Wt, Wtp, nci, nco, Q, runs; long rows; };
PPlan plan_wgradp(int N, int H, int W, int Cin_ld, int Cout) {
    PPlan p;
    p.Wt = (W + 3) / 4;
    p.Wtp = (p.Wt + 7) / 8 * 8;
    p.nci = Cin_ld / 64;
    p.nco = Cout / 64;
    p.rows = p_rows(N, H, p.Wtp);
    p.Q = N * (p.Wtp / 8) * H;
    const int per = 6 * p.nci * p.nco;
    int runs = 2048 / per;
    if (runs < 1) runs = 1;
    if (runs > p.Q / 16) runs = p.Q / 16 > 0 ? p.Q / 16 : 1;
    p.runs = runs;
    return p;
}

}

extern "C" long cvk_wgradp_plane_rows(int N, int H, int W) {
    if (N <= 0 || H <= 0 || W <= 0) return 0;
    return p_rows(N, H, ((W + 3) / 4 + 7) / 8 * 8);
}

extern "C" int cvk_wgradp_zero_pads(float* planes, int N, int H, int W, int C, void* stream) {
    CVK_CHECK_ARG(planes && N > 0 && H > 0 && W > 0 && C > 0 && C % 4 == 0 && cvk_aligned16(planes), "cvk_wgradp_zero_pads: bad arguments");
    const int Wt = (W + 3) / 4, Wtp = (Wt + 7) / 8 * 8;
    const long pr = 2L * Wtp + (long)N * 2 * Wtp + (long)N * H * (Wtp - Wt);
    const long threads = pr * (C / 4);
    hipLaunchKernelGGL(k_wgradp_zero_pads<false>, dim3((unsigned)((threads + 255) / 256)), dim3(256), 0, (hipStream_t)stream, planes, N, H, Wt, Wtp, C, 6);
    CVK_LAUNCH_RETURN("cvk_wgradp_zero_pads");
}

extern "C" int cvk_wgradp_zero_pads4(float* planes, int N, int H, int W, int C, void* stream) {
    CVK_CHECK_ARG(planes && N > 0 && H > 0 && W > 0 && C > 0 && C % 4 == 0 && cvk_aligned16(planes), "cvk_wgradp_zero_pads4: bad arguments");
    const int Wt = (W + 3) / 4, Wtp = (Wt + 7) / 8 * 8;
    const long pr = 2L * Wtp + (long)N * 2 * Wtp + (long)N * H * (Wtp - Wt);
    const long threads = pr * (C / 4);
    hipLaunchKernelGGL(k_wgradp_zero_pads<false>, dim3((unsigned)((threads + 255) / 256)), dim3(256), 0, (hipStream_t)stream, planes, N, H, Wt, Wtp, C, 4);
    CVK_LAUNCH_RETURN("cvk_wgradp_zero_pads4");
}

extern "C" int cvk_wgradp_zero_pads_sm(float* planes, int N, int H, int W, int C, void* stream) {
    CVK_CHECK_ARG(planes && N > 0 && H > 0 && W > 0 && C > 0 && C % 16 == 0 && cvk_aligned16(planes), "cvk_wgradp_zero_pads_sm: bad arguments");
    const int Wt = (W + 3) / 4, Wtp = (Wt + 7) / 8 * 8;
    const long pr = 2L * Wtp + (long)N * 2 * Wtp + (long)N * H * (Wtp - Wt);
    const long threads = pr * (C / 4);
    hipLaunchKernelGGL(k_wgradp_zero_pads<true>, dim3((unsigned)((threads + 255) / 256)), dim3(256), 0, (hipStream_t)stream, planes, N, H, Wt, Wtp, C, 6);
    CVK_LAUNCH_RETURN("cvk_wgradp_zero_pads_sm");
}

extern "C" size_t cvk_conv3x3_wgradp_workspace_bytes(int N, int H, int W, int Cin_ld, int Cout) {
    if (N <= 0 || H <= 0 || W <= 0 || Cin_ld < 64 || Cout < 64 || Cin_ld % 64 || Cout % 64) return 0;
    const PPlan p = plan_wgradp(N, H, W, Cin_ld, Cout);
    return ((size_t)6 * p.rows * (Cin_ld + Cout) + (size_t)p.runs * 6 * Cout * 3 * Cin_ld) * sizeof(float);
}

extern "C" int cvk_wgradp_planes(const float* t, int ld, float* planes, int N, int H, int W, int C, int is_dy, void* stream) {
    CVK_CHECK_ARG(t && planes && N > 0 && H > 0 && W > 0 && C > 0 && C % 4 == 0 && ld >= C && ld % 4 == 0, "cvk_wgradp_planes: bad arguments");
    CVK_CHECK_ARG(cvk_aligned16(t) && cvk_aligned16(planes), "cvk_wgradp_planes: pointers must be 16-byte aligned");
    const int Wt = (W + 3) / 4, Wtp = (Wt + 7) / 8 * 8;
    const long th = p_rows(N, H, Wtp) * (C / 4);
    hipStream_t s = (hipStream_t)stream;
    if (is_dy) hipLaunchKernelGGL(k_wgradp_planes<1>, dim3((unsigned)((th + 255) / 256)), dim3(256), 0, s, t, ld, planes, N, H, W, Wt, Wtp, C);
    else hipLaunchKernelGGL(k_wgradp_planes<0>, dim3((unsigned)((th + 255) / 256)), dim3(256), 0, s, t, ld, planes, N, H, W, Wt, Wtp, C);
    CVK_LAUNCH_RETURN("cvk_wgradp_planes");
}

extern "C" int cvk_wgradp_planes_sm(const float* x, int ld, float* planes, int N, int H, int W, int C, void* stream) {
    CVK_CHECK_ARG(x && planes && N > 0 && H > 0 && W > 0 && C > 0 && C % 16 == 0 && ld >= C && ld % 4 == 0, "cvk_wgradp_planes_sm: bad arguments");
    CVK_CHECK_ARG(cvk_aligned16(x) && cvk_aligned16(planes), "cvk_wgradp_planes_sm: pointers must be 16-byte aligned");
    const int Wt = (W + 3) / 4, Wtp = (Wt + 7) / 8 * 8;
    const long th = p_rows(N, H, Wtp) * (C / 4);
    hipLaunchKernelGGL((k_wgradp_planes<0, true>), dim3((unsigned)((th + 255) / 256)), dim3(256), 0, (hipStream_t)stream, x, ld, planes, N, H, W, Wt, Wtp, C);
    CVK_LAUNCH_RETURN("cvk_wgradp_planes_sm");
}

extern "C" size_t cvk_wgradp_gemm_workspace_bytes(int N, int H, int W, int Cin_ld, int Cout) {
    if (N <= 0 || H <= 0 || W <= 0 || Cin_ld < 64 || Cout < 64 || Cin_ld % 64 || Cout % 64) return 0;
    const PPlan p = plan_wgradp(N, H, W, Cin_ld, Cout);
    return (size_t)p.runs * 6 * Cout * 3 * Cin_ld * sizeof(float);
}

static int wgradp_gemm_go(bool vsm, const float* E6, const float* V6, float* dw, int N, int H, int W, int Cin, int Cin_ld, int Cout,
                          void* workspace, size_t workspace_bytes, void* stream, const float* dy = nullptr) {
    CVK_CHECK_ARG(E6 && V6 && dw && workspace, "cvk_wgradp_gemm: null pointer");
    CVK_CHECK_ARG(N > 0 && H > 0 && W > 0 && Cin > 0 && Cin <= Cin_ld && Cin_ld % 64 == 0 && Cout % 64 == 0 && Cout >= 64,
                  "cvk_wgradp_gemm: Cin_ld=%d and Cout=%d must be multiples of 64", Cin_ld, Cout);
    CVK_CHECK_ARG(cvk_aligned16(E6) && cvk_aligned16(V6) && cvk_aligned16(workspace), "cvk_wgradp_gemm: pointers must be 16-byte aligned");
    const PPlan p = plan_wgradp(N, H, W, Cin_ld, Cout);
    if (workspace_bytes < cvk_wgradp_gemm_workspace_bytes(N, H, W, Cin_ld, Cout)) {
        cvk_set_error("cvk_wgradp_gemm: workspace too small");
        return CVK_EWORKSPACE;
    }
    hipStream_t s = (hipStream_t)stream;
    float* slab = (float*)workspace;
    const int per = 6 * p.nci * p.nco;
    if (vsm) {
        CVK_CHECK_ARG(3L * p.rows * 64 + 4096 < (1L << 32), "cvk_wgradp_gemm_sm: %ld plane rows exceed the 32-bit lane offset of the slice-major V block", p.rows);
        if (dy) hipLaunchKernelGGL((k_wgradp_gemm<true, true>), dim3(per * p.runs), dim3(64), 0, s, E6, V6, slab, H, p.Wtp, Cin_ld, Cout, p.rows, p.Q, p.runs, p.nci, p.nco, dy, W);
        else hipLaunchKernelGGL((k_wgradp_gemm<true, false>), dim3(per * p.runs), dim3(64), 0, s, E6, V6, slab, H, p.Wtp, Cin_ld, Cout, p.rows, p.Q, p.runs, p.nci, p.nco, dy, W);
    } else {
        hipLaunchKernelGGL((k_wgradp_gemm<false, false>), dim3(per * p.runs), dim3(64), 0, s, E6, V6, slab, H, p.Wtp, Cin_ld, Cout, p.rows, p.Q, p.runs, p.nci, p.nco, dy, W);
    }
    hipError_t e = hipGetLastError();
    if (e != hipSuccess) {
        cvk_set_error("cvk_wgradp_gemm: launch failed: %s", hipGetErrorString(e));
        return (int)e;
    }
    const size_t total = (size_t)Cout * 3 * Cin;
    hipLaunchKernelGGL(k_wgradp_reduce, dim3((unsigned)((total + 63) / 64)), dim3(1024), 0, s, slab, dw, p.runs, Cout, Cin, Cin_ld);
    CVK_LAUNCH_RETURN("cvk_wgradp_gemm");
}

extern "C" int cvk_wgradp_gemm(const float* E6, const float* V6, float* dw, int N, int H, int W, int Cin, int Cin_ld, int Cout,
                               void* workspace, size_t workspace_bytes, void* stream) {
    return wgradp_gemm_go(false, E6, V6, dw, N, H, W, Cin, Cin_ld, Cout, workspace, workspace_bytes, stream);
}
extern "C" int cvk_wgradp_gemm_sm(const float* E6, const float* V6sm, float* dw, int N, int H, int W, int Cin, int Cin_ld, int Cout,
                                  void* workspace, size_t workspace_bytes, void* stream) {
    return wgradp_gemm_go(true, E6, V6sm, dw, N, H, W, Cin, Cin_ld, Cout, workspace, workspace_bytes, stream);
}

extern "C" int cvk_wgradp_dy_slack(int W) { return W > 0 ? 4 * (((W + 3) / 4 + 7) / 8 * 8) - W + 4 : 0; }
extern "C" int cvk_wgradp_gemm_sm_dy(const float* E4p, const float* dy, const float* V6sm, float* dw, int N, int H, int W, int Cin, int Cin_ld, int Cout,
                                     void* workspace, size_t workspace_bytes, void* stream) {
    CVK_CHECK_ARG(dy && cvk_aligned16(dy), "cvk_wgradp_gemm_sm_dy: dy must be a 16-byte aligned pointer");
    CVK_CHECK_ARG(W % 4 == 0, "cvk_wgradp_gemm_sm_dy: W=%d must be a multiple of 4 (use cvk_wgradp_gemm_sm with six planes)", W);
    return wgradp_gemm_go(true, E4p, V6sm, dw, N, H, W, Cin, Cin_ld, Cout, workspace, workspace_bytes, stream, dy);
}

extern "C" int cvk_conv3x3_wgradp(const float* x, const float* dy, const float* E6_pre, float* dw, int N, int H, int W, int Cin, int Cin_ld,
                                  int Cout, int ld_dy, void* workspace, size_t workspace_bytes, void* stream) {
    CVK_CHECK_ARG(x && (dy || E6_pre) && dw && workspace, "cvk_conv3x3_wgradp: null pointer");
    CVK_CHECK_ARG(N > 0 && H > 0 && W > 0 && Cin > 0 && Cin <= Cin_ld, "cvk_conv3x3_wgradp: bad shape");
    CVK_CHECK_ARG(Cin_ld % 64 == 0 && Cout % 64 == 0 && Cout >= 64 && ld_dy >= Cout && ld_dy % 4 == 0,
                  "cvk_conv3x3_wgradp: Cin_ld=%d and Cout=%d must be multiples of 64", Cin_ld, Cout);
    CVK_CHECK_ARG(cvk_aligned16(workspace), "cvk_conv3x3_wgradp: workspace must be 16-byte aligned");
    const size_t need = cvk_conv3x3_wgradp_workspace_bytes(N, H, W, Cin_ld, Cout);
    if (workspace_bytes < need) {
        cvk_set_error("cvk_conv3x3_wgradp: workspace %zu < %zu bytes", workspace_bytes, need);
        return CVK_EWORKSPACE;
    }
    const PPlan p = plan_wgradp(N, H, W, Cin_ld, Cout);
    float* V6 = (float*)workspace;
    float* E6 = V6 + (size_t)6 * p.rows * Cin_ld;
    float* slab = E6 + (size_t)6 * p.rows * Cout;
    int rc = cvk_wgradp_planes(x, Cin_ld, V6, N, H, W, Cin_ld, 0, stream);
    if (rc == CVK_OK && E6_pre == nullptr) rc = cvk_wgradp_planes(dy, ld_dy, E6, N, H, W, Cout, 1, stream);
    if (rc == CVK_OK)
        rc = cvk_wgradp_gemm(E6_pre != nullptr ? E6_pre : E6, V6, dw, N, H, W, Cin, Cin_ld, Cout, slab,
                             cvk_wgradp_gemm_workspace_bytes(N, H, W, Cin_ld, Cout), stream);
    return rc;
}
```

pytorch-camvid_amd/csrc/wino2d.hip:

```cpp
#include "cvk_common.h"
#include "lds_dma.h"
#include "split_fmt.h"

namespace {

constexpr int W2_BN = 128;
__host__ __device__ inline int w2_tb(int T) { return T >= 8192 ? 16 : 4; }

template <typename T>
__host__ __device__ __forceinline__ void w2_bt(const T* d, T* v) {
    const T a = d[4] - 4.f * d[2], b = d[3] - 4.f * d[1], c = d[4] - d[2], e = 2.f * (d[3] - d[1]);
    v[0] = 4.f * d[0] - 5.f * d[2] + d[4];
    v[1] = a + b;
    v[2] = a - b;
    v[3] = c + e;
    v[4] = c - e;
    v[5] = 4.f * d[1] - 5.f * d[3] + d[5];
}
template <typename T>
__device__ __forceinline__ void w2_at(const T* m, T* y) {
    const T s12 = m[1] + m[2], d12 = m[1] - m[2], s34 = m[3] + m[4], d34 = m[3] - m[4];
    y[0] = m[0] + s12 + s34;
    y[1] = d12 + 2.f * d34;
    y[2] = s12 + 4.f * s34;
// ... 551 lines not shown
        if (cs >= C / 32) return;
    } else {
        t = (int)(idx / cvn); c = (int)(idx % cvn) * VW;
    }
    if (t >= Tpad) return;
    const VT zero = {};
    const size_t plane = (size_t)Tpad * C, planeE = (size_t)TpadE * C;
    float* const vb = Vp + (size_t)t * C + c;
    float* const eb = E + (size_t)t * C + c;
    SplitDst sv = {}, se = {};
    if (SPL & 1) sv = split_dst<VW, FMT>(Vp, C, Tpad, t, c, amax, tabB);
    if (SPL & 2) se = split_dst<VW, FMT>(E, C, TpadE, t, c, amax, tabA);
    if (t >= T) {
        for (int xi = 0; xi < NX; ++xi) {
            if (SPL & 1) split_store<VW, FMT>(sv, xi, 0, 0, zero); else *reinterpret_cast<VT*>(vb + (size_t)xi * plane) = zero;
            if (t < TpadE) { if (SPL & 2) split_store<VW, FMT>(se, xi, 0, 0, zero); else *reinterpret_cast<VT*>(eb + (size_t)xi * planeE) = zero; }
        }
        return;
    }
    const int n = t / (th * tw), r = t - n * th * tw, ty = r / tw, tx = r - ty * tw;
    const float* const db = DY + (size_t)n * H * W * ld + c;
    {
        const int y0 = MT * ty - 1, x0 = MT * tx - 1;
        VT w[NT][NT];
#pragma unroll
        for (int j = 0; j < NT; ++j) {
            VT d[NT], v[NT];
            const int xx = x0 + j;
#pragma unroll
            for (int i = 0; i < NT; ++i) {
                const int yy = y0 + i;
                const bool ok = ((unsigned)yy < (unsigned)H) & ((unsigned)xx < (unsigned)W);
                d[i] = ok ? *reinterpret_cast<const VT*>(db + ((size_t)yy * W + xx) * ld) : zero;
            }
            TR::bt(d, v);
#pragma unroll
            for (int i = 0; i < NT; ++i) w[i][j] = v[i];
        }
#pragma unroll
        for (int i = 0; i < NT; ++i) {
            VT v[NT];
            TR::bt(w[i], v);
#pragma unroll
            for (int j = 0; j < NT; ++j) {
                if (SPL & 1) split_store<VW, FMT>(sv, i * NT + j, i, j, v[j]);
                else *reinterpret_cast<VT*>(vb + (size_t)(i * NT + j) * plane) = v[j];
            }
        }
    }
    {
        VT w[NT][MT];
#pragma unroll
        for (int j = 0; j < MT; ++j) {
            VT d[MT], e[NT];
            const int xx = MT * tx + j;
#pragma unroll
            for (int i = 0; i < MT; ++i) {
                const int yy = MT * ty + i;
                d[i] = (yy < H && xx < W) ? *reinterpret_cast<const VT*>(db + ((size_t)yy * W + xx) * ld) : zero;
            }
            TR::a(d, e);
#pragma unroll
            for (int i = 0; i < NT; ++i) w[i][j] = e[i];
        }
#pragma unroll
        for (int i = 0; i < NT; ++i) {
            VT e[NT];
            TR::a(w[i], e);
#pragma unroll
            for (int j = 0; j < NT; ++j) {
                if (SPL & 2) split_store<VW, FMT>(se, i * NT + j, i, j, e[j]);
                else *reinterpret_cast<VT*>(eb + (size_t)(i * NT + j) * planeE) = e[j];
            }
        }
    }
}

#ifndef CVK_TN_SPLIT_ISSUE
#define CVK_TN_SPLIT_ISSUE 1
#endif
template <int ABL = 0>
__global__ __launch_bounds__(256, 2) void k_w2d_gemm_tn(const float* __restrict__ A, int lda, const float* __restrict__ B, int ldb,
                                                       float* __restrict__ D, int Kp, int Mm, int Nn, int tilesM, int tilesN,
                                                       int f, int NX) {
    constexpr int STAGE = 32 * 256 * 4, PPW = 8;
    __shared__ __attribute__((aligned(1024))) char smem[2 * STAGE];
    const unsigned smem_addr = cvk_lds_addr(smem);
    const int tid = threadIdx.x, lane = tid & 63;
    const int wave = __builtin_amdgcn_readfirstlane(tid >> 6);
    const int r = lane & 31, h = lane >> 5;
    const int wm = wave >> 1, wn = wave & 1;
    const int id = cvk_xcd_remap(blockIdx.x, gridDim.x);
    const int part = id % f, tile = id / f;
    const int tn = tile % tilesN, tm = (tile / tilesN) % tilesM, xi = tile / (tilesN * tilesM);
    const int nK = Kp / 32, kb = part * nK / f, ke = (part + 1) * nK / f;
    A += (size_t)xi * Kp * lda + tm * 128;
    B += (size_t)xi * Kp * ldb + tn * 128;
    D += ((size_t)part * NX + xi) * Mm * Nn;

    const float* src[PPW];
    int sstep[PPW];
#pragma unroll
    for (int q = 0; q < PPW; ++q) {
        const int p = wave * PPW + q, pa = p & 15;
        const int krow = pa * 2 + (lane >> 5), col = (lane & 31) * 4;
        src[q] = p < 16 ? A + (size_t)krow * lda + col : B + (size_t)krow * ldb + col;
        sstep[q] = p < 16 ? 32 * lda : 32 * ldb;
    }
    auto issue = [&](int ks, int buf) {
#pragma unroll
        for (int q = 0; q < PPW; ++q) cvk_dma16(src[q] + (size_t)ks * sstep[q], smem_addr + buf * STAGE + (wave * PPW + q) * 1024);
    };
    f32x16 acc[2][2];
#pragma unroll
    for (int i = 0; i < 2; ++i)
#pragma unroll
        for (int j = 0; j < 2; ++j)
#pragma unroll
            for (int e = 0; e < 16; ++e) acc[i][j][e] = 0.f;
    const int a_off = h * 512 + (wm * 64 + 2 * r) * 4, b_off = 16384 + h * 512 + (wn * 64 + 2 * r) * 4;
    typedef float f32x2 __attribute__((ext_vector_type(2)));

    if (kb < ke) issue(kb, 0);
    int buf = 0;
    for (int ks = kb; ks < ke; ++ks) {
        if (ABL != 2) cvk_wait_vm<0>();
        if (ABL != 1) cvk_lds_retire_barrier();
        const int ksn = ABL == 5 ? kb : min(ks + 1, ke - 1);
        if (!CVK_TN_SPLIT_ISSUE && ABL != 2) issue(ksn, buf ^ 1);
        __builtin_amdgcn_s_setprio(1);
        const char* const st = smem + buf * STAGE;
#pragma unroll
        for (int q = 0; q < 16; ++q) {
            f32x2 a, b;
            if (ABL == 4) { a = f32x2{acc[0][0][0], 1.f}; b = f32x2{acc[0][0][1], 2.f}; asm volatile("" : "+v"(a), "+v"(b)); }
            else {
                a = *reinterpret_cast<const f32x2*>(st + a_off + q * 1024);
                b = *reinterpret_cast<const f32x2*>(st + b_off + q * 1024);
            }
            if (CVK_TN_SPLIT_ISSUE && ABL != 2 && (q == 0 || q == 4)) {
#pragma unroll
                for (int p = (q ? PPW / 2 : 0); p < (q ? PPW : PPW / 2); ++p)
                    cvk_dma16(src[p] + (size_t)ksn * sstep[p], smem_addr + (buf ^ 1) * STAGE + (wave * PPW + p) * 1024);
            }
#pragma unroll
            for (int i = 0; i < 2; ++i)
#pragma unroll
                for (int j = 0; j < 2; ++j) acc[i][j] = __builtin_amdgcn_mfma_f32_32x32x2f32(a[i], b[j], acc[i][j], 0, 0, 0);
        }
        __builtin_amdgcn_s_setprio(0);
        buf ^= 1;
    }
    cvk_wait_vm<0>();
    const int col = tn * 128 + wn * 64 + 2 * r;
#pragma unroll
    for (int i = 0; i < 2; ++i)
#pragma unroll
        for (int e = 0; e < 16; ++e) {
            const int row = tm * 128 + wm * 64 + 2 * ((e & 3) + 8 * (e >> 2) + 4 * h) + i;
            if (ABL == 3 ? (row < Mm && acc[i][0][e] == 123.456f) : row < Mm) {
                float* const dp = D + (size_t)row * Nn + col;
                if (col + 1 < Nn) { const f32x2 v = {acc[i][0][e], acc[i][1][e]}; *reinterpret_cast<f32x2*>(dp) = v; }
                else if (col < Nn) dp[0] = acc[i][0][e];
            }
        }
}

template <int MT>
__global__ __launch_bounds__(256) void k_w2d_wgrad_out(const float* __restrict__ P, float* __restrict__ dw, int Co, int Ci, int Cip, int f) {
    typedef W2T<MT> TR;
    constexpr int NT = TR::NT, NX = TR::NX;
    const size_t total = (size_t)Co * Ci, plane = (size_t)Co * Cip;
    for (size_t idx = (size_t)blockIdx.x * 256 + threadIdx.x; idx < total; idx += (size_t)gridDim.x * 256) {
        const int ci = (int)(idx % Ci);
        const size_t co = idx / Ci;
        const float* const pp = P + co * Cip + ci;
        float mx[NX];
#pragma unroll
        for (int q = 0; q < NX; ++q) mx[q] = pp[(size_t)q * plane];
        for (int k = 1; k < f; ++k) {
            float v[NX];
#pragma unroll
            for (int q = 0; q < NX; ++q) v[q] = pp[(size_t)(k * NX + q) * plane];
#pragma unroll
            for (int q = 0; q < NX; ++q) mx[q] += v[q];
        }
        float t[NT][3];
#pragma unroll
        for (int a = 0; a < NT; ++a) TR::gt(mx + a * NT, t[a]);
#pragma unroll
        for (int kx = 0; kx < 3; ++kx) {
            float col[NT], w3[3];
#pragma unroll
            for (int a = 0; a < NT; ++a) col[a] = t[a][kx];
            TR::gt(col, w3);
            dw[(co * 9 + 0 + kx) * Ci + ci] = w3[0];
            dw[(co * 9 + 3 + kx) * Ci + ci] = w3[1];
            dw[(co * 9 + 6 + kx) * Ci + ci] = w3[2];
        }
    }
}

template <int MT, bool STATS>
__global__ __launch_bounds__(256) void k_w2d_output(const float* __restrict__ Mo, int ldm, const float* __restrict__ bias,
                                                   float* __restrict__ Y, int ldy, float* __restrict__ stats,
                                                   float* __restrict__ counts, int P, int H, int W, int th, int tw, int T,
                                                   int Cout, int cvn, int BM, int tmn, int tilesN, int split_start, int f) {
    typedef W2T<MT> TR;
    typedef typename TR::VT VT;
    constexpr int NT = TR::NT, NX = TR::NX, VW = TR::VW;
    __shared__ float red[2][256 * VW];
    const int t = threadIdx.x;
    const int pl = 256 / cvn, cv = t % cvn, lanep = t / cvn;
    const int c = (blockIdx.y * cvn + cv) * VW;
    const bool cok = c < Cout;
    VT sh = {};
    if (cok && bias != nullptr) sh = *reinterpret_cast<const VT*>(bias + c);
    VT s1 = {}, s2 = {};
    const size_t plane = (size_t)T * ldm;
    const int TB = w2_tb(T);
    const int tile_end = min(T, (int)(blockIdx.x + 1) * TB);
    for (int tile = blockIdx.x * TB + lanep; tile < tile_end && cok; tile += pl) {
        const int n = tile / (th * tw), rr = tile - n * th * tw, ty = rr / tw, tx = rr - ty * tw;
        const float* const mp = Mo + (size_t)tile * ldm + c;
        const int xi0 = f > 1 ? (split_start - ((tile / BM) * tilesN + c / W2_BN) + tmn - 1) / tmn : NX;
        VT o[MT][MT];
#pragma unroll
        for (int i = 0; i < MT; ++i)
#pragma unroll
            for (int jj = 0; jj < MT; ++jj) o[i][jj] = VT{};
#pragma unroll
        for (int j = 0; j < NT; ++j) {
            VT m[NT], z[MT];
#pragma unroll
            for (int i = 0; i < NT; ++i) {
                m[i] = *reinterpret_cast<const VT*>(mp + (size_t)(i * NT + j) * plane);
                if (i * NT + j >= xi0)
                    for (int k = 1; k < f; ++k) m[i] += *reinterpret_cast<const VT*>(mp + (size_t)(k * NX + i * NT + j) * plane);
            }
            if constexpr (MT == 4) {
                w2_at(m, z);
#pragma unroll
                for (int i = 0; i < 4; ++i) {
                    if (j == 0) { o[i][0] = z[i]; }
                    else if (j == 1) { o[i][0] += z[i]; o[i][1] = z[i]; o[i][2] = z[i]; o[i][3] = z[i]; }
                    else if (j == 2) { o[i][0] += z[i]; o[i][1] -= z[i]; o[i][2] += z[i]; o[i][3] -= z[i]; }
                    else if (j == 3) { o[i][0] += z[i]; o[i][1] += 2.f * z[i]; o[i][2] += 4.f * z[i]; o[i][3] += 8.f * z[i]; }
                    else if (j == 4) { o[i][0] += z[i]; o[i][1] -= 2.f * z[i]; o[i][2] += 4.f * z[i]; o[i][3] -= 8.f * z[i]; }
// ... 153 lines not shown
    const size_t part_stride = (size_t)nx * T * Cout;
    hipStream_t s = (hipStream_t)stream;
    static int cus = 0;
    if (cus == 0) {
        int dev = 0, v = 0;
        cus = (hipGetDevice(&dev) == hipSuccess && hipDeviceGetAttribute(&v, hipDeviceAttributeMultiprocessorCount, dev) == hipSuccess && v > 0) ? v : 256;
    }
    const int no_stagger = cvk_knob("CVK_W2D_NO_STAGGER", 0);
    const int stagger = (!no_stagger && (int)grid.x >= 2 * cus && p.split_start >= 2 * cus) ? cus : 0;
#ifdef CVK_EXPERIMENTS
#define CVK_W2D_ABL_GO(A_) hipLaunchKernelGGL((k_w2d_gemm<128, 32, 2, 2, A_>), grid, dim3(256), 0, s, V, U, Mo, T, w2_tpad(T), Cout, Cin, Cout, p.tilesM, p.tilesN, p.split_start, p.f, part_stride, stagger)
    switch (cvk_knob("CVK_W2D_ABL", 0)) {
        case 1: CVK_W2D_ABL_GO(1); CVK_LAUNCH_RETURN(who);
        case 2: CVK_W2D_ABL_GO(2); CVK_LAUNCH_RETURN(who);
        case 3: CVK_W2D_ABL_GO(3); CVK_LAUNCH_RETURN(who);
        case 4: CVK_W2D_ABL_GO(4); CVK_LAUNCH_RETURN(who);
        case 5: CVK_W2D_ABL_GO(5); CVK_LAUNCH_RETURN(who);
        case 6: CVK_W2D_ABL_GO(6); CVK_LAUNCH_RETURN(who);
        case 8: CVK_W2D_ABL_GO(8); CVK_LAUNCH_RETURN(who);
        case 10: CVK_W2D_ABL_GO(10); CVK_LAUNCH_RETURN(who);
        case 11: CVK_W2D_ABL_GO(11); CVK_LAUNCH_RETURN(who);
        case 12: CVK_W2D_ABL_GO(12); CVK_LAUNCH_RETURN(who);
        default: break;
    }
#endif
    hipLaunchKernelGGL((k_w2d_gemm<128, 32, 2, 2>), grid, dim3(256), 0, s, V, U, Mo, T, w2_tpad(T), Cout, Cin, Cout, p.tilesM, p.tilesN,
                       p.split_start, p.f, part_stride, stagger);
    CVK_LAUNCH_RETURN(who);
}

static int w2i_output(int mt, const char* who, const float* Mo, const float* bias, float* y, float* stats, float* counts, int N, int H,
                      int W, int Cin, int Cout, int ldy, void* stream) {
    CVK_CHECK_ARG(Mo && y && N > 0 && H > 0 && W > 0, "%s: bad arguments", who);
    CVK_CHECK_ARG(Cout >= 64 && Cout % 4 == 0 && ldy >= Cout && ldy % 4 == 0, "%s: needs Cout %% 4 == 0, Cout >= 64 (got %d)", who, Cout);
    CVK_CHECK_ARG((stats == nullptr) == (counts == nullptr), "%s: stats and counts go together", who);
    CVK_CHECK_ARG(cvk_aligned16(Mo) && cvk_aligned16(y), "%s: pointers must be 16-byte aligned", who);
    CVK_CHECK_ARG(Cin >= 32 && Cin % 32 == 0, "%s: Cin (the GEMM depth, which fixes the K split of the planes) must be a multiple of 32", who);
    const int th = (H + mt - 1) / mt, tw = (W + mt - 1) / mt, T = N * th * tw;
    const int vw = mt == 4 ? 4 : 2, nv = Cout / vw;
    const int cvn = nv >= 64 ? 64 : (nv >= 32 ? 32 : 16);
    const int P = cvk_cdiv(T, w2_tb(T));
    const W2Plan p = plan_w2d(w2_nx(mt), T, Cin, Cout);
    dim3 grid(P, cvk_cdiv(nv, cvn));
    hipStream_t s = (hipStream_t)stream;
#define CVK_W2_OUT(MT_, ST_) hipLaunchKernelGGL((k_w2d_output<MT_, ST_>), grid, dim3(256), 0, s, Mo, Cout, bias, y, ldy, stats, counts, P, H, W, th, tw, T, Cout, cvn, \
                                                p.BM, p.tilesM * p.tilesN, p.tilesN, p.split_start, p.f)
    if (mt == 4) { if (stats) CVK_W2_OUT(4, true); else CVK_W2_OUT(4, false); }
    else         { if (stats) CVK_W2_OUT(6, true); else CVK_W2_OUT(6, false); }
#undef CVK_W2_OUT
    CVK_LAUNCH_RETURN(who);
}

struct W2WPlan { int Tpad, tilesM, tilesN, f; };
static W2WPlan plan_w2d_wgrad(int nx, int T, int Cin_pad, int Cout) {
    W2WPlan p;
    p.Tpad = w2_tpad(T);
    p.tilesM = cvk_cdiv(Cout, 128);
    p.tilesN = cvk_cdiv(Cin_pad, 128);
    const int nt = nx * p.tilesM * p.tilesN, nK = p.Tpad / 32;
    int f = cvk_cdiv(1024, nt);
    if (f > nK / 4) f = nK / 4;
    if (f > 16) f = 16;
    if (f < 1) f = 1;
    p.f = f;
    return p;
}

static int w2i_wgrad_ksplit(int mt, int T, int Cin_pad, int Cout) {
    if (T <= 0 || Cin_pad <= 0 || Cout <= 0) return 0;
    return plan_w2d_wgrad(w2_nx(mt), T, Cin_pad, Cout).f;
}

static int w2i_dy_transform(int mt, const char* who, const float* dy, int ld_dy, float* E, int N, int H, int W, int Cout, void* stream) {
    CVK_CHECK_ARG(dy && E && N > 0 && H > 0 && W > 0 && Cout >= 4 && Cout % 4 == 0 && ld_dy >= Cout && ld_dy % 4 == 0, "%s: bad arguments", who);
    CVK_CHECK_ARG(cvk_aligned16(dy) && cvk_aligned16(E), "%s: pointers must be 16-byte aligned", who);
    const int th = (H + mt - 1) / mt, tw = (W + mt - 1) / mt, T = N * th * tw, Tpad = w2_tpad(T);
    const long threads = (long)Tpad * (Cout / (mt == 4 ? 4 : 2));
    const dim3 grid((unsigned)((threads + 255) / 256));
    if (mt == 4) hipLaunchKernelGGL(k_w2d_dy<4>, grid, dim3(256), 0, (hipStream_t)stream, dy, ld_dy, E, H, W, Cout, th, tw, T, Tpad);
    else hipLaunchKernelGGL(k_w2d_dy<6>, grid, dim3(256), 0, (hipStream_t)stream, dy, ld_dy, E, H, W, Cout, th, tw, T, Tpad);
    CVK_LAUNCH_RETURN(who);
}

static int w2i_gemm_tn(int mt, const char* who, const float* E, const float* V, float* P, int T, int Cin_pad, int Cout, void* stream) {
    CVK_CHECK_ARG(E && V && P && T > 0 && Cin_pad > 0 && Cin_pad % 4 == 0 && Cout > 0 && Cout % 4 == 0, "%s: bad arguments", who);
    CVK_CHECK_ARG(cvk_aligned16(E) && cvk_aligned16(V) && cvk_aligned16(P), "%s: pointers must be 16-byte aligned", who);
    const int nx = w2_nx(mt);
    const W2WPlan p = plan_w2d_wgrad(nx, T, Cin_pad, Cout);
#ifdef CVK_EXPERIMENTS
#define CVK_TN_ABL_GO(A_) hipLaunchKernelGGL(k_w2d_gemm_tn<A_>, dim3(nx * p.tilesM * p.tilesN * p.f), dim3(256), 0, (hipStream_t)stream, E, Cout, V, Cin_pad, P, p.Tpad, Cout, Cin_pad, p.tilesM, p.tilesN, p.f, nx)
    switch (cvk_knob("CVK_W2D_TN_ABL", 0)) {
        case 1: CVK_TN_ABL_GO(1); CVK_LAUNCH_RETURN(who);
        case 2: CVK_TN_ABL_GO(2); CVK_LAUNCH_RETURN(who);
        case 3: CVK_TN_ABL_GO(3); CVK_LAUNCH_RETURN(who);
        case 4: CVK_TN_ABL_GO(4); CVK_LAUNCH_RETURN(who);
        case 5: CVK_TN_ABL_GO(5); CVK_LAUNCH_RETURN(who);
        default: break;
    }
#endif
    hipLaunchKernelGGL(k_w2d_gemm_tn<0>, dim3(nx * p.tilesM * p.tilesN * p.f), dim3(256), 0, (hipStream_t)stream, E, Cout, V, Cin_pad, P, p.Tpad,
                       Cout, Cin_pad, p.tilesM, p.tilesN, p.f, nx);
    CVK_LAUNCH_RETURN(who);
}

static int w2i_wgrad_output(int mt, const char* who, const float* P, float* dw, int T, int Cin, int Cin_pad, int Cout, void* stream) {
    CVK_CHECK_ARG(P && dw && T > 0 && Cin > 0 && Cin <= Cin_pad && Cout > 0, "%s: bad arguments", who);
    const W2WPlan p = plan_w2d_wgrad(w2_nx(mt), T, Cin_pad, Cout);
    const size_t total = (size_t)Cout * Cin;
    const int blocks = (int)((total + 255) / 256 < 16384 ? (total + 255) / 256 : 16384);
    if (mt == 4) hipLaunchKernelGGL(k_w2d_wgrad_out<4>, dim3(blocks), dim3(256), 0, (hipStream_t)stream, P, dw, Cout, Cin, Cin_pad, p.f);
    else hipLaunchKernelGGL(k_w2d_wgrad_out<6>, dim3(blocks), dim3(256), 0, (hipStream_t)stream, P, dw, Cout, Cin, Cin_pad, p.f);
    CVK_LAUNCH_RETURN(who);
}

static size_t w2i_wgrad_workspace_bytes(int mt, int N, int H, int W, int Cin_pad, int Cout) {
    if (N <= 0 || H <= 0 || W <= 0 || Cin_pad <= 0 || Cout <= 0) return 0;
    const int nx = w2_nx(mt);
    const W2WPlan p = plan_w2d_wgrad(nx, w2_tiles(mt, N, H, W), Cin_pad, Cout);
    return ((size_t)nx * p.Tpad * ((size_t)Cin_pad + Cout) + 2 * 128 + (size_t)p.f * nx * Cout * Cin_pad) * sizeof(float);
}

static int w2i_dy_both(int mt, const char* who, const float* dy, int ld_dy, float* Vp, float* E, int N, int H, int W, int C, void* stream) {
    CVK_CHECK_ARG(dy && Vp && E && N > 0 && H > 0 && W > 0 && C >= 4 && C % 4 == 0 && ld_dy >= C && ld_dy % 4 == 0, "%s: bad arguments", who);
    CVK_CHECK_ARG(cvk_aligned16(dy) && cvk_aligned16(Vp) && cvk_aligned16(E), "%s: pointers must be 16-byte aligned", who);
    const int th = (H + mt - 1) / mt, tw = (W + mt - 1) / mt, T = N * th * tw, Tpad = w2_tpad(T);
    const long threads = (long)Tpad * (C / (mt == 4 ? 4 : 2));
    const dim3 grid((unsigned)((threads + 255) / 256));
    if (mt == 4) hipLaunchKernelGGL(k_w2d_dy_both<4>, grid, dim3(256), 0, (hipStream_t)stream, dy, ld_dy, Vp, E, H, W, C, th, tw, T, Tpad, Tpad, (const unsigned*)nullptr, CvkSplitTab{}, CvkSplitTab{});
    else hipLaunchKernelGGL(k_w2d_dy_both<6>, grid, dim3(256), 0, (hipStream_t)stream, dy, ld_dy, Vp, E, H, W, C, th, tw, T, Tpad, Tpad, (const unsigned*)nullptr, CvkSplitTab{}, CvkSplitTab{});
    CVK_LAUNCH_RETURN(who);
}

template <int MT>
static CvkSplitTab w2_split_tab(int kind) {
    typedef W2T<MT> TR;
    constexpr int NT = TR::NT;
    const int nin = kind == CVK_SPLIT_KIND_B ? NT : (kind == CVK_SPLIT_KIND_G ? 3 : MT);
    double rs[8] = {};
    for (int k = 0; k < nin; ++k) {
        float d[8] = {}, v[8] = {};
        d[k] = 1.f;
        if (kind == CVK_SPLIT_KIND_B) TR::bt(d, v);
        else if (kind == CVK_SPLIT_KIND_G) TR::g(d, v);
        else TR::a(d, v);
        for (int i = 0; i < NT; ++i) rs[i] += v[i] < 0.f ? -(double)v[i] : (double)v[i];
    }
    CvkSplitTab t;
    t.c8 = 0ull;
    t.nt = NT;
    for (int i = 0; i < NT; ++i) {
        int c = -20;
        while (rs[i] > ldexp(1.0, c) * (1.0 + 1e-6)) ++c;
        t.c8 |= (unsigned long long)(unsigned)(c + 64) << (8 * i);
    }
    return t;
}
CvkSplitTab cvk_split_tab(int tile, int kind) { return tile == 4 ? w2_split_tab<4>(kind) : w2_split_tab<6>(kind); }

extern "C" int cvk_split_scale_exponent(int tile, int kind, int xi, unsigned amax_bits) {
    if (!(tile == 4 || tile == 6) || kind < 0 || kind > 2 || xi < 0 || xi >= w2_nx(tile)) return 0;
    const CvkSplitTab t = cvk_split_tab(tile, kind);
    return cvk_split_exp(amax_bits, cvk_split_tab_c(t, xi / t.nt), cvk_split_tab_c(t, xi % t.nt));
}

typedef unsigned u32x4a __attribute__((ext_vector_type(4)));
__device__ __forceinline__ unsigned absmax4(u32x4a v, unsigned m) {
    v &= 0x7FFFFFFFu;
    const unsigned m01 = v[0] > v[1] ? v[0] : v[1], m23 = v[2] > v[3] ? v[2] : v[3];
    const unsigned mv = m01 > m23 ? m01 : m23;
    return mv > m ? mv : m;
}
template <bool DENSE>
__global__ __launch_bounds__(256) void k_absmax(const float* __restrict__ X, long rows, int C, int ld, unsigned* __restrict__ out) {
    const int c4n = C >> 2;
    const long total = rows * c4n;
    const long step = (long)gridDim.x * 256;
    unsigned m = 0u;
    auto piece = [&](long i) -> const u32x4a* {
        if (DENSE) return reinterpret_cast<const u32x4a*>(X) + i;
        const long r = i / c4n;
        return reinterpret_cast<const u32x4a*>(X + r * ld + ((int)(i - r * c4n) << 2));
    };
    long i = (long)blockIdx.x * 256 + threadIdx.x;
    for (; i + 3 * step < total; i += 4 * step) {
// ... 118 lines not shown
}
extern "C" int cvk_w2d_weight_transform_split3(int tile, const float* w, void* U3, float* tmp, int Cout, int Cin, int dgrad, void* stream) {
    (void)tmp;
    return cvk_w2d_weight_transform_split(3, tile, w, U3, nullptr, Cout, Cin, dgrad, stream);
}

extern "C" int cvk_w2d_output_plain(int tile, const float* Mo, const float* bias, float* y, float* stats, float* counts, int N, int H, int W,
                                    int Cout, int ldy, void* stream) {
    const char* who = "cvk_w2d_output_plain";
    CVK_CHECK_ARG((tile == 4 || tile == 6) && Mo && y && N > 0 && H > 0 && W > 0, "%s: bad arguments", who);
    CVK_CHECK_ARG(Cout >= 64 && Cout % 4 == 0 && ldy >= Cout && ldy % 4 == 0, "%s: needs Cout %% 4 == 0, Cout >= 64 (got %d)", who, Cout);
    CVK_CHECK_ARG((stats == nullptr) == (counts == nullptr), "%s: stats and counts go together", who);
    CVK_CHECK_ARG(cvk_aligned16(Mo) && cvk_aligned16(y), "%s: pointers must be 16-byte aligned", who);
    const int mt = tile, th = (H + mt - 1) / mt, tw = (W + mt - 1) / mt, T = N * th * tw;
    const int vw = mt == 4 ? 4 : 2, nv = Cout / vw;
    const int cvn = nv >= 64 ? 64 : (nv >= 32 ? 32 : 16);
    const int P = cvk_cdiv(T, w2_tb(T));
    const int tilesM = cvk_cdiv(T, 128), tilesN = cvk_cdiv(Cout, 128);
    dim3 grid(P, cvk_cdiv(nv, cvn));
    hipStream_t s = (hipStream_t)stream;
#define CVK_W2_OUTP(MT_, ST_) hipLaunchKernelGGL((k_w2d_output<MT_, ST_>), grid, dim3(256), 0, s, Mo, Cout, bias, y, ldy, stats, counts, P, H, W, th, tw, T, Cout, cvn, \
                                                 128, tilesM * tilesN, tilesN, tilesM * tilesN, 1)
    if (mt == 4) { if (stats) CVK_W2_OUTP(4, true); else CVK_W2_OUTP(4, false); }
    else         { if (stats) CVK_W2_OUTP(6, true); else CVK_W2_OUTP(6, false); }
#undef CVK_W2_OUTP
    CVK_LAUNCH_RETURN(who);
}

extern "C" int cvk_w2d_wgrad_output_f(int tile, const float* P, float* dw, int Cin, int Cin_pad, int Cout, int f, void* stream) {
    CVK_CHECK_ARG((tile == 4 || tile == 6) && P && dw && Cin > 0 && Cin <= Cin_pad && Cout > 0 && f >= 1 && f <= 64, "cvk_w2d_wgrad_output_f: bad arguments");
    const size_t total = (size_t)Cout * Cin;
    const int blocks = (int)((total + 255) / 256 < 16384 ? (total + 255) / 256 : 16384);
    if (tile == 4) hipLaunchKernelGGL(k_w2d_wgrad_out<4>, dim3(blocks), dim3(256), 0, (hipStream_t)stream, P, dw, Cout, Cin, Cin_pad, f);
    else hipLaunchKernelGGL(k_w2d_wgrad_out<6>, dim3(blocks), dim3(256), 0, (hipStream_t)stream, P, dw, Cout, Cin, Cin_pad, f);
    CVK_LAUNCH_RETURN("cvk_w2d_wgrad_output_f");
}

extern "C" int cvk_w2d_tiles(int N, int H, int W) { return w2i_tiles(4, N, H, W); }
extern "C" int cvk_w2d_stat_partials(int N, int H, int W) { return w2i_stat_partials(4, N, H, W); }
extern "C" int cvk_w2d_ksplit(int T, int Cin, int Cout) { return w2i_ksplit(4, T, Cin, Cout); }
extern "C" size_t cvk_conv3x3_w2d_workspace_bytes(int N, int H, int W, int Cin, int Cout) { return w2i_workspace_bytes(4, N, H, W, Cin, Cout); }
extern "C" int cvk_w2d_weight_transform(const float* w, float* U, int Cout, int Cin, void* stream) {
    return w2i_weight_transform(4, "cvk_w2d_weight_transform", w, U, Cout, Cin, stream);
}
extern "C" int cvk_w2d_weight_transform_dgrad(const float* w, float* U, int Cout, int Cin, void* stream) {
    return w2i_weight_transform_dgrad(4, "cvk_w2d_weight_transform_dgrad", w, U, Cout, Cin, stream);
}
extern "C" int cvk_w2d_input_transform(const float* x, float* V, int N, int H, int W, int Cin, void* stream) {
    return w2i_input_transform(4, "cvk_w2d_input_transform", x, V, N, H, W, Cin, stream);
}
extern "C" int cvk_w2d_gemm(const float* V, const float* U, float* Mo, int T, int Cin, int Cout, void* stream) {
    return w2i_gemm(4, "cvk_w2d_gemm", V, U, Mo, T, Cin, Cout, stream);
}
extern "C" int cvk_w2d_output(const float* Mo, const float* bias, float* y, float* stats, float* counts, int N, int H, int W,
                              int Cin, int Cout, int ldy, void* stream) {
    return w2i_output(4, "cvk_w2d_output", Mo, bias, y, stats, counts, N, H, W, Cin, Cout, ldy, stream);
}

extern "C" int cvk_conv3x3_w2d(const float* x, const float* U, const float* bias, float* y, float* stats, float* counts,
                               int N, int H, int W, int Cin, int Cout, int ldy, void* workspace, size_t workspace_bytes,
                               void* stream) {
    CVK_CHECK_ARG(workspace && N > 0 && H > 0 && W > 0, "cvk_conv3x3_w2d: bad arguments");
    CVK_CHECK_ARG(cvk_aligned16(workspace) && workspace_bytes >= cvk_conv3x3_w2d_workspace_bytes(N, H, W, Cin, Cout),
                  "cvk_conv3x3_w2d: workspace too small or misaligned");
    const int T = w2_tiles(4, N, H, W);
    float* const V = (float*)workspace;
    float* const Mo = V + (size_t)36 * w2_tpad(T) * Cin + 128;
    int rc = cvk_w2d_input_transform(x, V, N, H, W, Cin, stream);
    if (rc == CVK_OK) rc = cvk_w2d_gemm(V, U, Mo, T, Cin, Cout, stream);
    if (rc == CVK_OK) rc = cvk_w2d_output(Mo, bias, y, stats, counts, N, H, W, Cin, Cout, ldy, stream);
    return rc;
}

extern "C" int cvk_w2d_wgrad_ksplit(int T, int Cin_pad, int Cout) { return w2i_wgrad_ksplit(4, T, Cin_pad, Cout); }
extern "C" int cvk_w2d_dy_transform(const float* dy, int ld_dy, float* E, int N, int H, int W, int Cout, void* stream) {
    return w2i_dy_transform(4, "cvk_w2d_dy_transform", dy, ld_dy, E, N, H, W, Cout, stream);
}
extern "C" int cvk_w2d_dy_transform_both(const float* dy, int ld_dy, float* Vp, float* E, int N, int H, int W, int Cout, void* stream) {
    return w2i_dy_both(4, "cvk_w2d_dy_transform_both", dy, ld_dy, Vp, E, N, H, W, Cout, stream);
}
extern "C" int cvk_w2d_gemm_tn(const float* E, const float* V, float* P, int T, int Cin_pad, int Cout, void* stream) {
    return w2i_gemm_tn(4, "cvk_w2d_gemm_tn", E, V, P, T, Cin_pad, Cout, stream);
}
extern "C" int cvk_w2d_wgrad_output(const float* P, float* dw, int T, int Cin, int Cin_pad, int Cout, void* stream) {
    return w2i_wgrad_output(4, "cvk_w2d_wgrad_output", P, dw, T, Cin, Cin_pad, Cout, stream);
}
extern "C" size_t cvk_conv3x3_wgrad_w2d_workspace_bytes(int N, int H, int W, int Cin_pad, int Cout) {
    return w2i_wgrad_workspace_bytes(4, N, H, W, Cin_pad, Cout);
}

extern "C" int cvk_conv3x3_wgrad_w2d(const float* x, const float* dy, float* dw, int N, int H, int W, int Cin, int Cin_pad,
                                     int Cout, int ld_dy, void* workspace, size_t workspace_bytes, void* stream) {
    CVK_CHECK_ARG(dy && dw && workspace, "cvk_conv3x3_wgrad_w2d: null pointer");
    CVK_CHECK_ARG(N > 0 && H > 0 && W > 0 && Cin > 0 && Cin <= Cin_pad && Cin_pad % 4 == 0 && Cout > 0 && Cout % 4 == 0 && ld_dy >= Cout && ld_dy % 4 == 0,
                  "cvk_conv3x3_wgrad_w2d: bad shape (channel counts must be multiples of 4)");
    CVK_CHECK_ARG(cvk_aligned16(workspace) && workspace_bytes >= cvk_conv3x3_wgrad_w2d_workspace_bytes(N, H, W, Cin_pad, Cout),
                  "cvk_conv3x3_wgrad_w2d: workspace too small or misaligned");
    const int T = w2_tiles(4, N, H, W), Tpad = w2_tpad(T);
    float* const V = (float*)workspace;
    float* const E = V + (size_t)36 * Tpad * Cin_pad + 128;
    float* const P = E + (size_t)36 * Tpad * Cout + 128;
    int rc = x ? cvk_w2d_input_transform(x, V, N, H, W, Cin_pad, stream) : CVK_OK;
    if (rc == CVK_OK) rc = cvk_w2d_dy_transform(dy, ld_dy, E, N, H, W, Cout, stream);
    if (rc == CVK_OK) rc = cvk_w2d_gemm_tn(E, V, P, T, Cin_pad, Cout, stream);
    if (rc == CVK_OK) rc = cvk_w2d_wgrad_output(P, dw, T, Cin, Cin_pad, Cout, stream);
    return rc;
}

extern "C" int cvk_w6_tiles(int N, int H, int W) { return w2i_tiles(6, N, H, W); }
extern "C" int cvk_w6_stat_partials(int N, int H, int W) { return w2i_stat_partials(6, N, H, W); }
extern "C" int cvk_w6_ksplit(int T, int Cin, int Cout) { return w2i_ksplit(6, T, Cin, Cout); }
extern "C" size_t cvk_conv3x3_w6_workspace_bytes(int N, int H, int W, int Cin, int Cout) { return w2i_workspace_bytes(6, N, H, W, Cin, Cout); }
extern "C" int cvk_w6_weight_transform(const float* w, float* U, int Cout, int Cin, void* stream) {
    return w2i_weight_transform(6, "cvk_w6_weight_transform", w, U, Cout, Cin, stream);
}
extern "C" int cvk_w6_weight_transform_dgrad(const float* w, float* U, int Cout, int Cin, void* stream) {
    return w2i_weight_transform_dgrad(6, "cvk_w6_weight_transform_dgrad", w, U, Cout, Cin, stream);
}
extern "C" int cvk_w6_input_transform(const float* x, float* V, int N, int H, int W, int Cin, void* stream) {
    return w2i_input_transform(6, "cvk_w6_input_transform", x, V, N, H, W, Cin, stream);
}
extern "C" int cvk_w6_gemm(const float* V, const float* U, float* Mo, int T, int Cin, int Cout, void* stream) {
    return w2i_gemm(6, "cvk_w6_gemm", V, U, Mo, T, Cin, Cout, stream);
}
extern "C" int cvk_w6_output(const float* Mo, const float* bias, float* y, float* stats, float* counts, int N, int H, int W, int Cin,
                             int Cout, int ldy, void* stream) {
    return w2i_output(6, "cvk_w6_output", Mo, bias, y, stats, counts, N, H, W, Cin, Cout, ldy, stream);
}
extern "C" int cvk_w6_wgrad_ksplit(int T, int Cin_pad, int Cout) { return w2i_wgrad_ksplit(6, T, Cin_pad, Cout); }
extern "C" int cvk_w6_dy_transform(const float* dy, int ld_dy, float* E, int N, int H, int W, int Cout, void* stream) {
    return w2i_dy_transform(6, "cvk_w6_dy_transform", dy, ld_dy, E, N, H, W, Cout, stream);
}
extern "C" int cvk_w6_dy_transform_both(const float* dy, int ld_dy, float* Vp, float* E, int N, int H, int W, int Cout, void* stream) {
    return w2i_dy_both(6, "cvk_w6_dy_transform_both", dy, ld_dy, Vp, E, N, H, W, Cout, stream);
}
extern "C" int cvk_w6_gemm_tn(const float* E, const float* V, float* P, int T, int Cin_pad, int Cout, void* stream) {
    return w2i_gemm_tn(6, "cvk_w6_gemm_tn", E, V, P, T, Cin_pad, Cout, stream);
}
extern "C" int cvk_w6_wgrad_output(const float* P, float* dw, int T, int Cin, int Cin_pad, int Cout, void* stream) {
    return w2i_wgrad_output(6, "cvk_w6_wgrad_output", P, dw, T, Cin, Cin_pad, Cout, stream);
}
```

pytorch-camvid_amd/engine.py:

```python
import ctypes
import os
from collections import namedtuple

import torch

from . import _lib
from ._lib import View, ViewH, check
from .route import conv_route, pad4, split_fmt
from .route import layer_tile, wgrad2d_pays, wino2d_ok, wino2d_pays, wino4_pays

_F32, _BF16 = torch.float32, torch.bfloat16


class ActBuf:
    __slots__ = ("id", "N", "H", "W", "C", "ld", "name", "dtype")

    def __init__(self, id_, N, H, W, C, name="", dtype=_F32):
        self.id, self.N, self.H, self.W, self.C, self.name, self.dtype = id_, N, H, W, C, name, dtype
        self.ld = pad4(C) if dtype == _F32 else max(32, (C + 7) // 8 * 8)

    @property
    def esize(self):
        return 4 if self.dtype == _F32 else 2

    @property
    def M(self):
        return self.N * self.H * self.W

    def full_view(self):
        return BufView(self, 0, self.C, 0, 0, self.H, self.W)

    def __repr__(self):
        return f"ActBuf({self.name}#{self.id} {self.N}x{self.H}x{self.W}x{self.C}/{self.ld})"


class BufView:
    __slots__ = ("buf", "c0", "C", "y0", "x0", "H", "W")

    def __init__(self, buf, c0, C, y0, x0, H, W):
        assert 0 <= c0 and c0 + C <= buf.ld and 0 <= y0 and y0 + H <= buf.H and 0 <= x0 and x0 + W <= buf.W
        self.buf, self.c0, self.C, self.y0, self.x0, self.H, self.W = buf, c0, C, y0, x0, H, W

    def cview(self, tensor):
        b = self.buf
        ptr = tensor.data_ptr() + 4 * ((self.y0 * b.W + self.x0) * b.ld + self.c0)
        return View(ptr, b.H * b.W * b.ld, b.W * b.ld, b.ld)

    def hview(self, tensor):
        b = self.buf
        ptr = tensor.data_ptr() + b.esize * ((self.y0 * b.W + self.x0) * b.ld + self.c0)
        return ViewH(ptr, b.H * b.W * b.ld, b.W * b.ld, b.ld)

    @property
    def is_full(self):
        b = self.buf
        return self.c0 == 0 and self.C == b.C and self.y0 == 0 and self.x0 == 0 and self.H == b.H and self.W == b.W


class RunState:

    def __init__(self, params, training, need_grad):
        self.params = params
        self.training = training
        self.need_grad = need_grad
        self.act = {}
        self.saved = {}
        self.routes = None
        self.grad = {}
        self.gflat = None
        self.stream = None
        self.sync = None
        self.pooled_by_block = {}
        self.colsums = []
        self.wreduces = []
        self.pass_token = 0
        self.bnred = {}
        self.amax = {}
        self.amax_spare = []
        self.scratch = []
        self.fold = None


def _empty(n, dev, dtype=_F32):
    return torch.empty(n, device=dev, dtype=dtype)


def channels_last(w):
    return w if w.is_contiguous(memory_format=torch.channels_last) else w.contiguous(memory_format=torch.channels_last)


class Saved(namedtuple("Saved", "y bnp rt kept", defaults=(None, None))):
    def pointers(self, ld):
        pb = self.bnp.data_ptr()
        return self.y.data_ptr(), pb + 8 * ld, pb + 12 * ld, pb, pb + 4 * ld


WINO_DEFAULT = os.environ.get("CVK_WINO", "1") != "0"
WINO4_DEFAULT = {"0": False, "1": True, "always": "always"}[os.environ.get("CVK_WINO4", "1")]
WINO2D_DEFAULT = {"0": False, "1": True, "always": "always"}[os.environ.get("CVK_WINO2D", "1")]
W2TILE_DEFAULT = {"auto": None, "4": 4, "6": 6}[os.environ.get("CVK_W2D_TILE", "auto")]
WINO4F_DEFAULT = os.environ.get("CVK_WINO4F", "1") != "0"
WGRADP_DEFAULT = {"0": False, "1": True, "always": "always"}[os.environ.get("CVK_WGRADP", "1")]
VPLANES_DEFAULT = os.environ.get("CVK_VPLANES", "1") != "0"


def amax_blocks(lib, n, dev):
    nw = lib.cvk_amax_block_words()
    t = torch.zeros(n * nw, device=dev, dtype=torch.int32)
    return [t[i * nw:(i + 1) * nw] for i in range(n)]


WEIGHT_EPOCH = [0]
WCACHE_DEFAULT = os.environ.get("CVK_WEIGHT_CACHE", "1") != "0"


def _bump_epoch(*_a, **_k):
    WEIGHT_EPOCH[0] += 1


try:
    from torch.optim.optimizer import register_optimizer_step_post_hook as _reg_opt_hook
    _reg_opt_hook(_bump_epoch)
except ImportError:
    WCACHE_DEFAULT = False


def mark_weights_dirty(module):
    from .modules import runner_of
    runner_of(module).wepoch += 1


PROF = None
PROF_OPS = None
_CUR_OP = [None]


def _timed(R, name, work, fn, unit="flop", executed=None, nbytes=None):
    if PROF is None:
        return fn()
    e0, e1 = torch.cuda.Event(enable_timing=True), torch.cuda.Event(enable_timing=True)
    e0.record()
    r = fn()
    e1.record()
    PROF.append((name, work, e0, e1, unit, executed, nbytes))
    if PROF_OPS is not None:
        PROF_OPS.append(_CUR_OP[0])
    return r


class Op:
    idx = -1

    def fwd(self, R, st):
        raise NotImplementedError

    def bwd(self, R, st):
        pass


class MaxPool(Op):

    def __init__(self, src_view, dst_buf, keep_code):
        self.src, self.dst, self.keep_code = src_view, dst_buf, keep_code
        self.fused = False
        self.producer_idx = -1
        self.wants = True
        if src_view.H < 2 or src_view.W < 2:
            raise RuntimeError(f"max_pool2d: input {src_view.H}x{src_view.W} is too small for a 2x2 window")

    def fwd(self, R, st):
        v, d = self.src, self.dst
        X = st.act[v.buf.id]
        if st.plan.bf16:
            if not self.fused:
                raise NotImplementedError("bf16 mode: a max pool must directly follow a conv block (it is fused into its BN pass)")
            return
        if self.fused and st.pooled_by_block.get(self.producer_idx, False):
            return
        out = R.alloc_act(st, d, X.device)
        code = None
        if self.keep_code:
            code = torch.empty(d.M * d.ld, device=X.device, dtype=torch.uint8)
            st.saved[self.idx] = code
        _timed(R, "k_maxpool_fwd", 5.0 * v.buf.N * v.H * v.W * v.C, lambda: check(
            R.lib.cvk_maxpool2x2_fwd(v.cview(X), out.data_ptr(), code.data_ptr() if code is not None else None,
                                     v.buf.N, v.H, v.W, v.C, st.stream), "cvk_maxpool2x2_fwd"), "byte")
# ... 251 lines not shown
        v = pool_op.src
        dst = self.new_buf(v.C, v.H, v.W, "unpool")
        self._reads(src_buf)
        op = self.add(Unpool(src_buf, pool_op, dst))
        op.wants = self._needs_grad(src_buf)
        self._writes(dst, 0, dst.C, op)
        return dst

    def upsample(self, src_buf):
        dst = self.new_buf(src_buf.C, 2 * src_buf.H, 2 * src_buf.W, "up")
        self._reads(src_buf)
        op = self.add(Upsample(src_buf, dst))
        op.wants = self._needs_grad(src_buf)
        self._writes(dst, 0, dst.C, op)
        return dst

    def zero_frame(self, view):
        self.add(ZeroFrame(view))

    def seal(self, thin=True):
        if self.bf16:
            b = self.output.buf
            if not self.output.is_full:
                raise NotImplementedError("bf16 mode: the network output must be a whole buffer")
            b.dtype = _F32
            b.ld = pad4(b.C)
            readers = [op for op in self.ops if getattr(op, "src", None) is self.input]
            if (thin and not self.input_needs_grad and self.input.C <= 4 and readers and self.input is not self.output.buf
                    and all(isinstance(op, ConvBnRelu) and op.cout == 64 for op in readers)
                    and self.input.H * self.input.W * 64 * 2 < 2 ** 31):
                self.input.ld = 8


_SPLIT_ENV_LOGGED = False


def _split_mode_from_env():
    global _SPLIT_ENV_LOGGED
    raw = os.environ.get("CVK_W2D_SPLIT")
    if raw is None:
        return 0
    modes = {"0": 0, "1": 3, "3": 3, "2": 2}
    if raw.strip() not in modes:
        raise ValueError(f"CVK_W2D_SPLIT={raw!r}: allowed values are 0 (off, the default), 2 (two fp16 terms) and 3 or 1 (three bf16 terms); "
                         "or leave it unset and call pytorch_camvid_amd.set_split_operands(net, mode)")
    mode = modes[raw.strip()]
    if mode and not _SPLIT_ENV_LOGGED:
        _SPLIT_ENV_LOGGED = True
        import sys
        print(f"pytorch_camvid_amd: CVK_W2D_SPLIT={raw} — fp32 convolution products run as split {'fp16 x 2' if mode == 2 else 'bf16 x 3'} operands "
              "(opt-in, not the exact-fp32 default)", file=sys.stderr)
    return mode


class Runner:

    def __init__(self):
        self.lib = _lib.load()
        self._ws = None
        self._dp_wgs = None
        self._collectives_in_flight = False
        self.grad_sync = None
        self.accumulator = None
        self.wino = WINO_DEFAULT
        self.wino4 = WINO4_DEFAULT
        self.wino4f = WINO4F_DEFAULT
        self.wgradp = WGRADP_DEFAULT
        self.vplanes = VPLANES_DEFAULT
        self.thin = os.environ.get("CVK_THIN", "1") != "0"
        self.pool_bnred = os.environ.get("CVK_POOL_BNRED", "1") != "0"
        self.wino2d = WINO2D_DEFAULT
        self.w2d_split = _split_mode_from_env()
        self.w2tile_cfg = W2TILE_DEFAULT
        self.w2tile = 6
        self.w2tile_dgrad = 6
        self.bf16 = False
        self.wcache = WCACHE_DEFAULT
        self.wepoch = 0
        self._wc = {}
        self._wjobs, self._wjobs_cfg = {}, None
        self._pass_token = 0
        self._passes = 0
        self.wcache_builds = 0

    def persistent_wgs(self):
        gs = self.grad_sync
        if gs is None or (getattr(gs, "world", 1) <= 1 and not getattr(gs, "always_issue", False)):
            return 0
        if self._dp_wgs is None:
            cus = torch.cuda.get_device_properties(torch.cuda.current_device()).multi_processor_count
            self._dp_wgs = max(8, cus - int(os.environ.get("CVK_DP_RESERVE_CUS", "8")))
        return self._dp_wgs

    def launch_wgs(self):
        return self.persistent_wgs() if self._collectives_in_flight else 0

    def derived(self, key, src, build, job=None):
        if not self.wcache or key is None or torch.cuda.is_current_stream_capturing():
            self.wcache_builds += 1
            return build()
        if job is not None:
            self._wjobs[key] = (src, job)
        return self._cache(key, src, build)

    def _cache(self, key, src, build=None):
        sig = (WEIGHT_EPOCH[0], self.wepoch, src.data_ptr(), src._version, self._pass_token)
        ent = self._wc.get(key)
        if (ent is None or ent[0] != sig) and build is not None:
            ent = self._wc[key] = (sig, build())
            self.wcache_builds += 1
        return ent[1] if ent is not None and ent[0] == sig else None

    def prebuild_fp32(self, plan, st, need_grad):
        if not self.wcache or torch.cuda.is_current_stream_capturing():
            return
        cfg = (id(plan),) + self.kernel_config()
        if cfg != self._wjobs_cfg:
            self._wjobs, self._wjobs_cfg = {}, cfg
            return
        live = {p.data_ptr() for p in st.params}
        lib, fam_jobs = self.lib, {"w4f": [], "w2d": []}
        for key, (src, (fam, floats, rows, cols, tile, dgrad)) in self._wjobs.items():
            if src.data_ptr() not in live or (dgrad and not need_grad):
                continue
            if self._cache(key, src) is not None:
                continue
            t = self._cache(key, src, lambda: _empty(floats, src.device))
            fam_jobs[fam].append((_lib.WtJob(src.data_ptr(), t.data_ptr(), rows, cols, tile, dgrad), 4.0 * (src.numel() + floats)))
        for fam, fn in (("w4f", lib.cvk_wino4f_weight_transform_batch), ("w2d", lib.cvk_w2d_weight_transform_batch)):
            jobs = fam_jobs[fam]
            for i in range(0, len(jobs), _lib.WT_BATCH_MAX):
                chunk = jobs[i:i + _lib.WT_BATCH_MAX]
                arr = (_lib.WtJob * len(chunk))(*[j for j, _ in chunk])
                _timed(self, "k_weight_transform_batch", sum(b for _, b in chunk),
                       lambda: check(fn(ctypes.addressof(arr), len(chunk), st.stream), "cvk_%s_weight_transform_batch" % fam), "byte")

    def prepack_bf16(self, plan, st, need_grad):
        if not self.wcache or torch.cuda.is_current_stream_capturing():
            return
        lib, jobs, keep = self.lib, [], []
        for op in plan.ops:
            if not isinstance(op, ConvBnRelu):
                continue
            w = st.params[4 * op.pslot]
            for key, dgrad, rows, kpad in op.packs_wanted(self, need_grad):
                if self._cache(key, w) is not None:
                    continue
                wc = channels_last(w)
                t = self._cache(key, w, lambda: torch.empty(lib.cvk_bf16s_rows_pad(rows) * 9 * kpad, device=w.device, dtype=_BF16))
                jobs.append(_lib.PackJob(wc.data_ptr(), t.data_ptr(), op.cout, op.cin, kpad, dgrad))
                keep.append(wc)
        for i in range(0, len(jobs), _lib.PACK_BATCH_MAX):
            chunk = jobs[i:i + _lib.PACK_BATCH_MAX]
            arr = (_lib.PackJob * len(chunk))(*chunk)
            check(lib.cvk_pack_weights_bf16_batch(ctypes.addressof(arr), len(chunk), st.stream), "cvk_pack_weights_bf16_batch")

    def workspace(self, nbytes, dev):
        if self._ws is None or self._ws.numel() < nbytes or self._ws.device != dev:
            self._ws = torch.empty(max(nbytes, 1 << 20), device=dev, dtype=torch.uint8)
        return self._ws

    def alloc_act(self, st, buf, dev):
        t = st.act.get(buf.id)
        if t is None:
            shape = (buf.N, buf.H, buf.W, buf.ld)
            t = torch.zeros(shape, device=dev, dtype=buf.dtype) if buf.ld != buf.C else torch.empty(shape, device=dev, dtype=buf.dtype)
# ... 76 lines not shown
        want, ok = [], {}

        def fusable(buf):
            if buf.id in ok:
                return ok[buf.id]
            ok[buf.id] = False
            ws = writers(buf)
            good = bool(ws) and buf is not plan.input
            for op in ws:
                if isinstance(op, Upsample):
                    good = good and fusable(op.src)
                elif not isinstance(op, (ConvBnRelu, ZeroFrame)):
                    good = False
            ok[buf.id] = good
            if good:
                want.append(buf)
            return good
        for op in layers:
            fusable(op.src)
        blocks = amax_blocks(self.lib, len(want) + len(layers), st.device)
        for i, buf in enumerate(want):
            st.amax[buf.id] = blocks[i]
        st.amax_spare = blocks[len(want):]

    def kernel_config(self):
        return (self.wino, self.wino4, self.wino4f, self.wino2d, self.wgradp, self.vplanes, self.thin, self.pool_bnred, self.w2d_split,
                self.w2tile_cfg)

    def routes(self, plan, training, need_grad):
        key = (self.kernel_config(), training, need_grad)
        r = plan.routes.get(key)
        if r is None:
            if split_fmt(self):
                check_bn_modes(plan, training, "set_split_operands")
            self.w2tile, self.w2tile_dgrad = self.tile_for(plan)
            r = plan.routes[key] = {op.idx: conv_route(self, op, training, need_grad) for op in plan.ops if isinstance(op, ConvBnRelu)}
        return r

    def tile_for(self, plan):
        if self.w2tile_cfg in (4, 6):
            return self.w2tile_cfg, self.w2tile_cfg
        return (4, 6) if any(isinstance(op, Unpool) for op in plan.ops) else (6, 6)

    def forward(self, plan, x, params, training, need_grad):
        dev = x.device
        self._collectives_in_flight = False
        st = RunState(params, training, need_grad)
        st.device = dev
        st.plan = plan
        if training and need_grad:
            self._passes += 1
            st.pass_token = self._passes
        self._pass_token = st.pass_token
        st.stream = torch.cuda.current_stream(dev).cuda_stream
        st.act[plan.input.id] = self.import_nchw(st, x, plan.input, _BF16 if plan.bf16 else _F32)
        if plan.bf16:
            check_bn_modes(plan, training, "bf16 mode", need_grad, forward_only_ok=True)
            self.prepack_bf16(plan, st, need_grad)
        else:
            st.routes = self.routes(plan, training, need_grad)
            self.prebuild_fp32(plan, st, need_grad)
            self.plan_amax(plan, st)
        for op in plan.ops:
            _CUR_OP[0] = (op.idx, "fwd")
            op.fwd(self, st)
        _CUR_OP[0] = None
        ov = plan.output
        out = st.act[ov.buf.id][..., :ov.buf.C].permute(0, 3, 1, 2)
        if not need_grad:
            st.act.clear()
            st.saved.clear()
        return out, st

    def backward(self, plan, st, gout):
        dev = gout.device
        st.stream = torch.cuda.current_stream(dev).cuda_stream
        self._pass_token = st.pass_token
        params = st.params
        st.goffs, total = layout_grads(params)
        st.gflat = torch.empty(total, device=dev, dtype=_F32)
        fold = st.fold = self.accumulator.open_pass(st, plan, total) if self.accumulator is not None else None
        st.sync = self.begin_sync(st, plan, fold)
        self._collectives_in_flight = False
        st.grad[plan.output.buf.id] = self.import_nchw(st, gout, plan.output.buf, _F32, zero_pad=True)
        for op in reversed(plan.ops):
            _CUR_OP[0] = (op.idx, "bwd")
            op.bwd(self, st)
        _CUR_OP[0] = None
        self.flush_colsums(st)
        self.flush_wreduces(st)
        if fold is not None and st.sync is None:
            fold.whole(st)
        dx = None
        if plan.input_needs_grad:
            gi = st.grad[plan.input.id]
            dx = gi[..., :plan.input.C].permute(0, 3, 1, 2)
            if plan.bf16:
                dx = dx.float()
        grads = []
        hand_out = fold is None or fold.closing
        for i, p in enumerate(params):
            op = plan.convs[i // 4]
            if not hand_out or not (op.w_req, op.b_req, op.g_req, op.be_req)[i % 4]:
                grads.append(None)
                continue
            n = p.numel()
            seg = st.gflat[st.goffs[i]:st.goffs[i] + n]
            if p.dim() == 4:
                co, ci, kh, kw = p.shape
                seg = seg.view(co, kh, kw, ci).permute(0, 3, 1, 2)
            else:
                seg = seg.view(p.shape)
            grads.append(seg)
        if st.sync is not None:
            st.sync.finish(st)
        self._collectives_in_flight = False
        st.act.clear(); st.saved.clear(); st.grad.clear(); st.scratch.clear()
        if fold is not None:
            fold.done()
            st.fold = None
            if not hand_out:
                st.gflat = None
        return dx, grads


def check_bn_modes(plan, training, what, need_grad=True, forward_only_ok=False):
    for op in plan.convs:
        if forward_only_ok and not (need_grad and op.active):
            continue
        if op.bn_train != bool(training):
            raise NotImplementedError(f"{what}: BatchNorm of {op.label} is in {'training' if op.bn_train else 'eval'} mode inside a "
                                      f"{'training' if training else 'eval'} pass; per-block BatchNorm modes run in the fp32 mode only")


def layout_grads(params):
    offs = [0] * len(params)
    o = 0
    for slot in range(len(params) // 4 - 1, -1, -1):
        for j in range(4):
            i = 4 * slot + j
            offs[i] = o
            o += (params[i].numel() + 3) // 4 * 4
    return offs, o


class _PlanFunction(torch.autograd.Function):

    @staticmethod
    def forward(ctx, runner, plan, training, x, *params):
        out, st = runner.forward(plan, x, params, training, True)
        ctx.runner, ctx.plan, ctx.st = runner, plan, st
        return out

    @staticmethod
    def backward(ctx, gout):
        st = ctx.st
        if st is None:
            raise RuntimeError("Trying to backward through the plan a second time (activations were already freed)")
        ctx.st = None
        dx, grads = ctx.runner.backward(ctx.plan, st, gout)
        return (None, None, None, dx, *grads)


def run_plan(runner, plan, training, x, params):
    need = torch.is_grad_enabled() and (x.requires_grad or any(p.requires_grad for p in params))
    if not need:
        out, _ = runner.forward(plan, x, params, training, False)
        return out
    return _PlanFunction.apply(runner, plan, training, x, *params)


# ... 3 lines not shown
```

Baseline: 246.3 images/s.

## Run conv weight-gradient kernels on a low-priority side stream overlapping dgrad

Adds a per-device low-priority side HIP stream with fork/join events, and launches conv weight-gradient work (wgradp, w2d, thin families) on it so it can overlap the next data-gradient kernels on the main stream. Before each dgrad and at the end of backward the main stream joins the side stream, and the Python side keeps temporary tensors alive until the join. The wgrad GEMM kernels are also turned into grid-stride persistent loops with an optional workgroup cap, so they could leave compute units free for concurrent work. The cost is extra event traffic, a risk of workspace aliasing between streams, and contention that could slow the critical path.

```diff
diff --git a/include/cvk.h b/include/cvk.h
--- a/include/cvk.h
+++ b/include/cvk.h
@@ -94,6 +94,8 @@
 int cvk_w6_dy_transform(const float* dy, int ld_dy, float* E, int N, int H, int W, int Cout, void* stream);
 int cvk_w6_dy_transform_both(const float* dy, int ld_dy, float* Vp, float* E, int N, int H, int W, int Cout, void* stream);
 int cvk_w6_gemm_tn(const float* E, const float* V, float* P, int T, int Cin_pad, int Cout, void* stream);
+int cvk_w2d_gemm_tn_wg(const float* E, const float* V, float* P, int T, int Cin_pad, int Cout, int max_workgroups, void* stream);
+int cvk_w6_gemm_tn_wg(const float* E, const float* V, float* P, int T, int Cin_pad, int Cout, int max_workgroups, void* stream);
 int cvk_split3_rows_pad(int R, int mult);
 int cvk_split3_planes(const float* P, void* S, int NX, int R, int Rpad, int C, void* stream);
 int cvk_w2d_gemm_split3(const void* V3, const void* U3, float* Mo, int NX, int T, int Tpad, int Cin, int Cout, int Cpad, void* stream);
@@ -170,6 +172,15 @@
 int cvk_wgradp_dy_slack(int W);
 int cvk_wgradp_gemm_sm_dy(const float* E4p, const float* dy, const float* V6sm, float* dw, int N, int H, int W, int Cin, int Cin_pad, int Cout,
                           void* workspace, size_t workspace_bytes, void* stream);
+int cvk_wgradp_gemm_wg(const float* E6, const float* V6, float* dw, int N, int H, int W, int Cin, int Cin_pad, int Cout, void* workspace,
+                       size_t workspace_bytes, int max_workgroups, void* stream);
+int cvk_wgradp_gemm_sm_wg(const float* E6, const float* V6sm, float* dw, int N, int H, int W, int Cin, int Cin_pad, int Cout, void* workspace,
+                          size_t workspace_bytes, int max_workgroups, void* stream);
+int cvk_wgradp_gemm_sm_dy_wg(const float* E4p, const float* dy, const float* V6sm, float* dw, int N, int H, int W, int Cin, int Cin_pad, int Cout,
+                             void* workspace, size_t workspace_bytes, int max_workgroups, void* stream);
+void* cvk_side_begin(void* main_stream);
+int cvk_side_join(void* main_stream);
+long cvk_side_launches(void);
 int cvk_bn_bwd_dx_e6(cvk_view dout, const float* y, int ldy, const float* scale, const float* shift, const float* mean,
                      const float* rstd, const float* dgamma, const float* dbeta, float* dy, int ld_dy, float* E6, float* part,
                      int N, int H, int W, int C, int use_batch_stats, void* stream);
diff --git a/pytorch-camvid_amd/_lib.py b/pytorch-camvid_amd/_lib.py
--- a/pytorch-camvid_amd/_lib.py
+++ b/pytorch-camvid_amd/_lib.py
@@ -80,6 +80,14 @@
                                   c_int, c_int, c_int, c_int, c_int, c_vp]),
     "cvk_wgradp_dy_slack": (c_int, [c_int]),
     "cvk_wgradp_gemm_sm_dy": (c_int, [c_vp, c_vp, c_vp, c_vp, c_int, c_int, c_int, c_int, c_int, c_int, c_vp, c_size, c_vp]),
+    "cvk_wgradp_gemm_wg": (c_int, [c_vp, c_vp, c_vp, c_int, c_int, c_int, c_int, c_int, c_int, c_vp, c_size, c_int, c_vp]),
+    "cvk_wgradp_gemm_sm_wg": (c_int, [c_vp, c_vp, c_vp, c_int, c_int, c_int, c_int, c_int, c_int, c_vp, c_size, c_int, c_vp]),
+    "cvk_wgradp_gemm_sm_dy_wg": (c_int, [c_vp, c_vp, c_vp, c_vp, c_int, c_int, c_int, c_int, c_int, c_int, c_vp, c_size, c_int, c_vp]),
+    "cvk_w2d_gemm_tn_wg": (c_int, [c_vp, c_vp, c_vp, c_int, c_int, c_int, c_int, c_vp]),
+    "cvk_w6_gemm_tn_wg": (c_int, [c_vp, c_vp, c_vp, c_int, c_int, c_int, c_int, c_vp]),
+    "cvk_side_begin": (c_vp, [c_vp]),
+    "cvk_side_join": (c_int, [c_vp]),
+    "cvk_side_launches": (ctypes.c_long, []),
     "cvk_conv3x3_wino4f_vplanes": (c_int, [c_vp, c_vp, c_vp, c_vp, c_vp, c_vp, c_vp, c_int, c_int, c_int, c_int, c_int, c_int, c_int, c_vp]),
     "cvk_bn_bwd_dx_e6": (c_int, [View, c_vp, c_int, c_vp, c_vp, c_vp, c_vp, c_vp, c_vp, c_vp, c_int, c_vp, c_vp,
                                  c_int, c_int, c_int, c_int, c_int, c_vp]),
diff --git a/pytorch-camvid_amd/conv_fp32.py b/pytorch-camvid_amd/conv_fp32.py
--- a/pytorch-camvid_amd/conv_fp32.py
+++ b/pytorch-camvid_amd/conv_fp32.py
@@ -220,6 +220,7 @@
 
     def __init__(self, R, s, x, dy, gw, N, H, W, cin, k_ch, cout, ldy, flops):
         self.R, self.lib, self.s, self.x, self.dy, self.gw = R, R.lib, s, x, dy, gw
+        self.keep = []
         self.N, self.H, self.W, self.M, self.cin, self.k_ch, self.cout, self.ldy, self.flops = N, H, W, N * H * W, cin, k_ch, cout, ldy, flops
 
     def run(self, fam, tile=0, fmt=0, V=None, am_v=None, E=None, dy_e=False, Eb=None, am_dy=None):
@@ -239,6 +240,7 @@
         f = w2fn(lib, tile, "wgrad_ksplit")(T, k_ch, C)
         if V is None:
             V = _empty(plane_elems(NX, Tp, k_ch), x.device)
+            self.keep.append(V)
             _timed(R, "k_w2d_input", 4.0 * (M + NX * T) * k_ch, lambda: check(
                 w2fn(lib, tile, "input_transform")(x.data_ptr(), V.data_ptr(), N, H, W, k_ch, s), "cvk_w2d_input_transform(wgrad)"), "byte")
         ws = R.workspace(4 * ((0 if Eb is not None else efl) + f * NX * C * k_ch), x.device)
@@ -526,6 +528,7 @@
         flops = 18.0 * M * C * self.cin
         if src.id in st.grad:
             raise NotImplementedError("conv data-grad must be the first writer of its input's gradient buffer")
+        R.side_join(st)
         w = st.params[4 * self.pslot]
         wc = channels_last(w)
 
@@ -558,9 +561,18 @@
         return (self.dst.cview(st.grad[self.dst.buf.id]),)
 
     def _weight_grad(self, R, st, saved, dy, gw, E, Eb, am_dy):
-        src, rt = self.src, saved.rt
-        WeightGrad(R, st.stream, st.act[src.id], dy, gw, src.N, src.H, src.W, self.cin, src.ld, self.cout, pad4(self.cout),
-                   18.0 * src.M * self.cout * self.cin).run(rt.wgrad, rt.tile, rt.split, *(saved.kept or (None, None)), E, rt.bn_bwd == "dx+E4p", Eb, am_dy)
+        src, rt, s = self.src, saved.rt, st.stream
+        x = st.act[src.id]
+        side = st.side and rt.wgrad in R.side_families
+        if side:
+            s = R.side_begin(st, x, dy, E, Eb, am_dy, saved)
+        else:
+            R.side_join(st)
+        wg = WeightGrad(R, s, x, dy, gw, src.N, src.H, src.W, self.cin, src.ld, self.cout, pad4(self.cout), 18.0 * src.M * self.cout * self.cin)
+        wg.run(rt.wgrad, rt.tile, rt.split, *(saved.kept or (None, None)), E, rt.bn_bwd == "dx+E4p", Eb, am_dy)
+        if side:
+            st.side_keep.extend(wg.keep)
+            st.side_keep.append(R.workspace(0, x.device))
 
     def bwd(self, R, st):
         saved = st.saved.pop(self.idx, None)
diff --git a/pytorch-camvid_amd/csrc/side.cpp b/pytorch-camvid_amd/csrc/side.cpp
--- /dev/null
+++ b/pytorch-camvid_amd/csrc/side.cpp
@@ -0,0 +1,72 @@
+#include "cvk_common.h"
+#include <atomic>
+#include <mutex>
+
+namespace {
+
+constexpr int kMaxDev = 64;
+struct Side {
+    hipStream_t stream = nullptr;
+    hipEvent_t fork = nullptr, join = nullptr;
+};
+Side g_side[kMaxDev];
+std::mutex g_mu;
+std::atomic<long> g_forks{0};
+
+Side* side_of_current_device(const char* who) {
+    int dev = -1;
+    hipError_t e = hipGetDevice(&dev);
+    if (e != hipSuccess || dev < 0 || dev >= kMaxDev) {
+        cvk_set_error("%s: no current device (%s)", who, hipGetErrorString(e));
+        return nullptr;
+    }
+    Side& sd = g_side[dev];
+    if (sd.stream == nullptr) {
+        int least = 0, greatest = 0;
+        e = hipDeviceGetStreamPriorityRange(&least, &greatest);
+        if (e == hipSuccess) e = hipEventCreateWithFlags(&sd.fork, hipEventDisableTiming);
+        if (e == hipSuccess) e = hipEventCreateWithFlags(&sd.join, hipEventDisableTiming);
+        hipStream_t s = nullptr;
+        if (e == hipSuccess) e = hipStreamCreateWithPriority(&s, hipStreamNonBlocking, least);
+        if (e != hipSuccess) {
+            cvk_set_error("%s: creating the side stream failed: %s", who, hipGetErrorString(e));
+            if (sd.fork) (void)hipEventDestroy(sd.fork);
+            if (sd.join) (void)hipEventDestroy(sd.join);
+            sd.fork = sd.join = nullptr;
+            return nullptr;
+        }
+        sd.stream = s;
+    }
+    return &sd;
+}
+
+}
+
+extern "C" void* cvk_side_begin(void* main_stream) {
+    std::lock_guard<std::mutex> lock(g_mu);
+    Side* sd = side_of_current_device("cvk_side_begin");
+    if (sd == nullptr) return nullptr;
+    hipError_t e = hipEventRecord(sd->fork, (hipStream_t)main_stream);
+    if (e == hipSuccess) e = hipStreamWaitEvent(sd->stream, sd->fork, 0);
+    if (e != hipSuccess) {
+        cvk_set_error("cvk_side_begin: %s", hipGetErrorString(e));
+        return nullptr;
+    }
+    g_forks.fetch_add(1, std::memory_order_relaxed);
+    return sd->stream;
+}
+
+extern "C" int cvk_side_join(void* main_stream) {
+    std::lock_guard<std::mutex> lock(g_mu);
+    Side* sd = side_of_current_device("cvk_side_join");
+    if (sd == nullptr) return CVK_EINVAL;
+    hipError_t e = hipEventRecord(sd->join, sd->stream);
+    if (e == hipSuccess) e = hipStreamWaitEvent((hipStream_t)main_stream, sd->join, 0);
+    if (e != hipSuccess) {
+        cvk_set_error("cvk_side_join: %s", hipGetErrorString(e));
+        return (int)e;
+    }
+    return CVK_OK;
+}
+
+extern "C" long cvk_side_launches(void) { return g_forks.load(std::memory_order_relaxed); }
diff --git a/pytorch-camvid_amd/csrc/wgradp.hip b/pytorch-camvid_amd/csrc/wgradp.hip
--- a/pytorch-camvid_amd/csrc/wgradp.hip
+++ b/pytorch-camvid_amd/csrc/wgradp.hip
@@ -101,120 +101,123 @@
 template <bool VSM, bool EDY>
 __global__ __launch_bounds__(64, 2) void k_wgradp_gemm(const float* __restrict__ E6, const float* __restrict__ V6, float* __restrict__ slab,
                                                       int H, int Wtp, int Cin_ld, int Cout, long rows, int Q, int runs, int nci, int nco,
-                                                      const float* __restrict__ dy, int W) {
+                                                      const float* __restrict__ dy, int W, int njobs) {
     __shared__ __attribute__((aligned(1024))) char smem[12 * 1024];
     const unsigned smem_addr = cvk_lds_addr(smem);
     const int lane = threadIdx.x;
     const int lj = lane & 15, kq = lane >> 4;
 
     const int per = 6 * nci * nco;
-    const int id = cvk_xcd_remap(blockIdx.x, gridDim.x);
-    const int run = id / per, u = id - run * per;
-    const int xi = u % 6, cit = (u / 6) % nci, cot = u / (6 * nci);
-    const int qb = (int)((long)run * Q / runs), qe = (int)((long)(run + 1) * Q / runs);
-    if (qb >= qe) return;
-    const int so = Wtp >> 3;
-
-    const bool edy = EDY && (xi == 0 || xi == 5);
-    const float* const Eb = edy ? dy + cot * 64 + (xi == 5 ? 3 * Cout : 0) : E6 + (size_t)(EDY ? xi - 1 : xi) * rows * Cout + cot * 64;
-    const int epitch = edy ? 4 * Cout : Cout;
-    const float* const Vb = V6 + (size_t)xi * rows * Cin_ld + (VSM ? (size_t)cit * 4 * rows * 16 : (size_t)cit * 64);
-    const int vpitch = VSM ? 16 : Cin_ld;
-    const unsigned evoff = (unsigned)(((lane >> 4) * epitch + (lane & 15) * 4) * 4);
-    const unsigned vvoff = VSM ? (unsigned)((((unsigned long)((lane & 15) >> 2) * (unsigned long)rows + (lane >> 4)) * 16 + (lane & 3) * 4) * 4)
-                               : (unsigned)(((lane >> 4) * Cin_ld + (lane & 15) * 4) * 4);
-    auto block_row = [&](int strip, int yp) -> long {
-        const int n = strip / so, xg = strip - n * so;
-        return (long)Wtp + ((long)n * (H + 2) + yp) * Wtp + 8 * xg;
-    };
-    auto dma_V = [&](int strip, int yp) {
-        const float* src = Vb + (size_t)block_row(strip, yp) * vpitch;
-        const unsigned dst = smem_addr + (yp & 3) * 2048;
-        p_dma16(src, vvoff, dst);
-        p_dma16(src + 4 * (size_t)vpitch, vvoff, dst + 1024);
-    };
-    auto dma_E = [&](int strip, int yp, int slot) {
-        const int en = strip / so, exg = strip - en * so;
-        const float* src = edy ? Eb + (((size_t)en * H + (yp - 1)) * W + 32 * (size_t)exg) * Cout : Eb + (size_t)block_row(strip, yp) * Cout;
-        const unsigned dst = smem_addr + 8192 + slot * 2048;
-        p_dma16(src, evoff, dst);
-        p_dma16(src + 4 * (size_t)epitch, evoff, dst + 1024);
-    };
-
-    f32x4 acc[3][16];
-#pragma unroll
-    for (int r = 0; r < 3; ++r)
-#pragma unroll
-        for (int b = 0; b < 16; ++b) acc[r][b] = f32x4{0.f, 0.f, 0.f, 0.f};
-
-    const int frag = kq * 256 + lj * 16;
-
-    int strip = qb / H, y = qb - strip * H;
-    dma_V(strip, y);
-    dma_V(strip, y + 1);
-    dma_V(strip, y + 2);
-    dma_E(strip, y + 1, 0);
-    int es = 0;
-    for (int q = qb; q < qe; ++q) {
-        const bool last_in_strip = (y == H - 1);
-        const bool more = q + 1 < qe;
-        asm volatile("s_waitcnt lgkmcnt(0)" ::: "memory");
-        if (more && !last_in_strip) {
-            dma_V(strip, y + 3);
-            dma_E(strip, y + 2, es ^ 1);
-            cvk_wait_vm<4>();
-        } else {
-            cvk_wait_vm<0>();
+    for (int job = blockIdx.x; job < njobs; job += gridDim.x) {
+        asm volatile("s_waitcnt vmcnt(0) lgkmcnt(0)" ::: "memory");
+        const int id = cvk_xcd_remap(job, njobs);
+        const int run = id / per, u = id - run * per;
+        const int xi = u % 6, cit = (u / 6) % nci, cot = u / (6 * nci);
+        const int qb = (int)((long)run * Q / runs), qe = (int)((long)(run + 1) * Q / runs);
+        if (qb >= qe) continue;
+        const int so = Wtp >> 3;
+
+        const bool edy = EDY && (xi == 0 || xi == 5);
+        const float* const Eb = edy ? dy + cot * 64 + (xi == 5 ? 3 * Cout : 0) : E6 + (size_t)(EDY ? xi - 1 : xi) * rows * Cout + cot * 64;
+        const int epitch = edy ? 4 * Cout : Cout;
+        const float* const Vb = V6 + (size_t)xi * rows * Cin_ld + (VSM ? (size_t)cit * 4 * rows * 16 : (size_t)cit * 64);
+        const int vpitch = VSM ? 16 : Cin_ld;
+        const unsigned evoff = (unsigned)(((lane >> 4) * epitch + (lane & 15) * 4) * 4);
+        const unsigned vvoff = VSM ? (unsigned)((((unsigned long)((lane & 15) >> 2) * (unsigned long)rows + (lane >> 4)) * 16 + (lane & 3) * 4) * 4)
+                                   : (unsigned)(((lane >> 4) * Cin_ld + (lane & 15) * 4) * 4);
+        auto block_row = [&](int strip, int yp) -> long {
+            const int n = strip / so, xg = strip - n * so;
+            return (long)Wtp + ((long)n * (H + 2) + yp) * Wtp + 8 * xg;
+        };
+        auto dma_V = [&](int strip, int yp) {
+            const float* src = Vb + (size_t)block_row(strip, yp) * vpitch;
+            const unsigned dst = smem_addr + (yp & 3) * 2048;
+            p_dma16(src, vvoff, dst);
+            p_dma16(src + 4 * (size_t)vpitch, vvoff, dst + 1024);
+        };
+        auto dma_E = [&](int strip, int yp, int slot) {
+            const int en = strip / so, exg = strip - en * so;
+            const float* src = edy ? Eb + (((size_t)en * H + (yp - 1)) * W + 32 * (size_t)exg) * Cout : Eb + (size_t)block_row(strip, yp) * Cout;
+            const unsigned dst = smem_addr + 8192 + slot * 2048;
+            p_dma16(src, evoff, dst);
+            p_dma16(src + 4 * (size_t)epitch, evoff, dst + 1024);
+        };
+
+        f32x4 acc[3][16];
+#pragma unroll
+        for (int r = 0; r < 3; ++r)
+#pragma unroll
+            for (int b = 0; b < 16; ++b) acc[r][b] = f32x4{0.f, 0.f, 0.f, 0.f};
+
+        const int frag = kq * 256 + lj * 16;
+
+        int strip = qb / H, y = qb - strip * H;
+        dma_V(strip, y);
+        dma_V(strip, y + 1);
+        dma_V(strip, y + 2);
+        dma_E(strip, y + 1, 0);
+        int es = 0;
+        for (int q = qb; q < qe; ++q) {
+            const bool last_in_strip = (y == H - 1);
+            const bool more = q + 1 < qe;
+            asm volatile("s_waitcnt lgkmcnt(0)" ::: "memory");
+            if (more && !last_in_strip) {
+                dma_V(strip, y + 3);
+                dma_E(strip, y + 2, es ^ 1);
+                cvk_wait_vm<4>();
+            } else {
+                cvk_wait_vm<0>();
+            }
+            __builtin_amdgcn_s_setprio(1);
+            const char* const eblk = smem + 8192 + es * 2048;
+            const char* const v0 = smem + ((y + 0) & 3) * 2048;
+            const char* const v1 = smem + ((y + 1) & 3) * 2048;
+            const char* const v2 = smem + ((y + 2) & 3) * 2048;
+#pragma unroll
+            for (int ks = 0; ks < 2; ++ks) {
+                const f32x4 a = *reinterpret_cast<const f32x4*>(eblk + ks * 1024 + frag);
+                const f32x4 b0 = *reinterpret_cast<const f32x4*>(v0 + ks * 1024 + frag);
+                const f32x4 b1 = *reinterpret_cast<const f32x4*>(v1 + ks * 1024 + frag);
+                const f32x4 b2 = *reinterpret_cast<const f32x4*>(v2 + ks * 1024 + frag);
+#pragma unroll
+                for (int i = 0; i < 4; ++i)
+#pragma unroll
+                    for (int j = 0; j < 4; ++j) {
+                        acc[0][i * 4 + j] = __builtin_amdgcn_mfma_f32_16x16x4f32(a[i], b0[j], acc[0][i * 4 + j], 0, 0, 0);
+                        acc[1][i * 4 + j] = __builtin_amdgcn_mfma_f32_16x16x4f32(a[i], b1[j], acc[1][i * 4 + j], 0, 0, 0);
+                        acc[2][i * 4 + j] = __builtin_amdgcn_mfma_f32_16x16x4f32(a[i], b2[j], acc[2][i * 4 + j], 0, 0, 0);
+                    }
+            }
+            __builtin_amdgcn_s_setprio(0);
+            if (more) {
+                if (last_in_strip) {
+                    ++strip;
+                    y = 0;
+                    asm volatile("s_waitcnt lgkmcnt(0)" ::: "memory");
+                    dma_V(strip, 0);
+                    dma_V(strip, 1);
+                    dma_V(strip, 2);
+                    dma_E(strip, 1, es ^ 1);
+                } else {
+                    ++y;
+                }
+                es ^= 1;
+            }
         }
-        __builtin_amdgcn_s_setprio(1);
-        const char* const eblk = smem + 8192 + es * 2048;
-        const char* const v0 = smem + ((y + 0) & 3) * 2048;
-        const char* const v1 = smem + ((y + 1) & 3) * 2048;
-        const char* const v2 = smem + ((y + 2) & 3) * 2048;
-#pragma unroll
-        for (int ks = 0; ks < 2; ++ks) {
-            const f32x4 a = *reinterpret_cast<const f32x4*>(eblk + ks * 1024 + frag);
-            const f32x4 b0 = *reinterpret_cast<const f32x4*>(v0 + ks * 1024 + frag);
-            const f32x4 b1 = *reinterpret_cast<const f32x4*>(v1 + ks * 1024 + frag);
-            const f32x4 b2 = *reinterpret_cast<const f32x4*>(v2 + ks * 1024 + frag);
+
+        const int K3 = 3 * Cin_ld;
+        float* const out = slab + ((size_t)(run * 6 + xi) * Cout + cot * 64) * K3 + cit * 64 + 4 * lj;
+#pragma unroll
+        for (int r = 0; r < 3; ++r)
 #pragma unroll
             for (int i = 0; i < 4; ++i)
 #pragma unroll
-                for (int j = 0; j < 4; ++j) {
-                    acc[0][i * 4 + j] = __builtin_amdgcn_mfma_f32_16x16x4f32(a[i], b0[j], acc[0][i * 4 + j], 0, 0, 0);
-                    acc[1][i * 4 + j] = __builtin_amdgcn_mfma_f32_16x16x4f32(a[i], b1[j], acc[1][i * 4 + j], 0, 0, 0);
-                    acc[2][i * 4 + j] = __builtin_amdgcn_mfma_f32_16x16x4f32(a[i], b2[j], acc[2][i * 4 + j], 0, 0, 0);
+                for (int e = 0; e < 4; ++e) {
+                    const int co = 4 * (4 * kq + e) + i;
+                    const f32x4 v = {acc[r][i * 4 + 0][e], acc[r][i * 4 + 1][e], acc[r][i * 4 + 2][e], acc[r][i * 4 + 3][e]};
+                    *reinterpret_cast<f32x4*>(out + (size_t)co * K3 + r * Cin_ld) = v;
                 }
-        }
-        __builtin_amdgcn_s_setprio(0);
-        if (more) {
-            if (last_in_strip) {
-                ++strip;
-                y = 0;
-                asm volatile("s_waitcnt lgkmcnt(0)" ::: "memory");
-                dma_V(strip, 0);
-                dma_V(strip, 1);
-                dma_V(strip, 2);
-                dma_E(strip, 1, es ^ 1);
-            } else {
-                ++y;
-            }
-            es ^= 1;
-        }
-    }
-
-    const int K3 = 3 * Cin_ld;
-    float* const out = slab + ((size_t)(run * 6 + xi) * Cout + cot * 64) * K3 + cit * 64 + 4 * lj;
-#pragma unroll
-    for (int r = 0; r < 3; ++r)
-#pragma unroll
-        for (int i = 0; i < 4; ++i)
-#pragma unroll
-            for (int e = 0; e < 4; ++e) {
-                const int co = 4 * (4 * kq + e) + i;
-                const f32x4 v = {acc[r][i * 4 + 0][e], acc[r][i * 4 + 1][e], acc[r][i * 4 + 2][e], acc[r][i * 4 + 3][e]};
-                *reinterpret_cast<f32x4*>(out + (size_t)co * K3 + r * Cin_ld) = v;
-            }
+    }
 }
 
 __global__ __launch_bounds__(1024) void k_wgradp_reduce(const float* __restrict__ slab, float* __restrict__ dw, int runs, int Cout, int Cin,
@@ -337,8 +340,9 @@
 }
 
 static int wgradp_gemm_go(bool vsm, const float* E6, const float* V6, float* dw, int N, int H, int W, int Cin, int Cin_ld, int Cout,
-                          void* workspace, size_t workspace_bytes, void* stream, const float* dy = nullptr) {
+                          void* workspace, size_t workspace_bytes, void* stream, const float* dy = nullptr, int max_workgroups = 0) {
     CVK_CHECK_ARG(E6 && V6 && dw && workspace, "cvk_wgradp_gemm: null pointer");
+    CVK_CHECK_ARG(max_workgroups >= 0, "cvk_wgradp_gemm: max_workgroups must be >= 0");
     CVK_CHECK_ARG(N > 0 && H > 0 && W > 0 && Cin > 0 && Cin <= Cin_ld && Cin_ld % 64 == 0 && Cout % 64 == 0 && Cout >= 64,
                   "cvk_wgradp_gemm: Cin_ld=%d and Cout=%d must be multiples of 64", Cin_ld, Cout);
     CVK_CHECK_ARG(cvk_aligned16(E6) && cvk_aligned16(V6) && cvk_aligned16(workspace), "cvk_wgradp_gemm: pointers must be 16-byte aligned");
@@ -350,12 +354,15 @@
     hipStream_t s = (hipStream_t)stream;
     float* slab = (float*)workspace;
     const int per = 6 * p.nci * p.nco;
+    const int njobs = per * p.runs;
+    int wgs = njobs;
+    if (max_workgroups > 0 && max_workgroups < njobs) wgs = max_workgroups >= 8 ? max_workgroups / 8 * 8 : max_workgroups;
     if (vsm) {
         CVK_CHECK_ARG(3L * p.rows * 64 + 4096 < (1L << 32), "cvk_wgradp_gemm_sm: %ld plane rows exceed the 32-bit lane offset of the slice-major V block", p.rows);
-        if (dy) hipLaunchKernelGGL((k_wgradp_gemm<true, true>), dim3(per * p.runs), dim3(64), 0, s, E6, V6, slab, H, p.Wtp, Cin_ld, Cout, p.rows, p.Q, p.runs, p.nci, p.nco, dy, W);
-        else hipLaunchKernelGGL((k_wgradp_gemm<true, false>), dim3(per * p.runs), dim3(64), 0, s, E6, V6, slab, H, p.Wtp, Cin_ld, Cout, p.rows, p.Q, p.runs, p.nci, p.nco, dy, W);
+        if (dy) hipLaunchKernelGGL((k_wgradp_gemm<true, true>), dim3(wgs), dim3(64), 0, s, E6, V6, slab, H, p.Wtp, Cin_ld, Cout, p.rows, p.Q, p.runs, p.nci, p.nco, dy, W, njobs);
+        else hipLaunchKernelGGL((k_wgradp_gemm<true, false>), dim3(wgs), dim3(64), 0, s, E6, V6, slab, H, p.Wtp, Cin_ld, Cout, p.rows, p.Q, p.runs, p.nci, p.nco, dy, W, njobs);
     } else {
-        hipLaunchKernelGGL((k_wgradp_gemm<false, false>), dim3(per * p.runs), dim3(64), 0, s, E6, V6, slab, H, p.Wtp, Cin_ld, Cout, p.rows, p.Q, p.runs, p.nci, p.nco, dy, W);
+        hipLaunchKernelGGL((k_wgradp_gemm<false, false>), dim3(wgs), dim3(64), 0, s, E6, V6, slab, H, p.Wtp, Cin_ld, Cout, p.rows, p.Q, p.runs, p.nci, p.nco, dy, W, njobs);
     }
     hipError_t e = hipGetLastError();
     if (e != hipSuccess) {
@@ -382,6 +389,21 @@
     CVK_CHECK_ARG(dy && cvk_aligned16(dy), "cvk_wgradp_gemm_sm_dy: dy must be a 16-byte aligned pointer");
     CVK_CHECK_ARG(W % 4 == 0, "cvk_wgradp_gemm_sm_dy: W=%d must be a multiple of 4 (use cvk_wgradp_gemm_sm with six planes)", W);
     return wgradp_gemm_go(true, E4p, V6sm, dw, N, H, W, Cin, Cin_ld, Cout, workspace, workspace_bytes, stream, dy);
+}
+
+extern "C" int cvk_wgradp_gemm_wg(const float* E6, const float* V6, float* dw, int N, int H, int W, int Cin, int Cin_ld, int Cout,
+                                  void* workspace, size_t workspace_bytes, int max_workgroups, void* stream) {
+    return wgradp_gemm_go(false, E6, V6, dw, N, H, W, Cin, Cin_ld, Cout, workspace, workspace_bytes, stream, nullptr, max_workgroups);
+}
+extern "C" int cvk_wgradp_gemm_sm_wg(const float* E6, const float* V6sm, float* dw, int N, int H, int W, int Cin, int Cin_ld, int Cout,
+                                     void* workspace, size_t workspace_bytes, int max_workgroups, void* stream) {
+    return wgradp_gemm_go(true, E6, V6sm, dw, N, H, W, Cin, Cin_ld, Cout, workspace, workspace_bytes, stream, nullptr, max_workgroups);
+}
+extern "C" int cvk_wgradp_gemm_sm_dy_wg(const float* E4p, const float* dy, const float* V6sm, float* dw, int N, int H, int W, int Cin, int Cin_ld,
+                                        int Cout, void* workspace, size_t workspace_bytes, int max_workgroups, void* stream) {
+    CVK_CHECK_ARG(dy && cvk_aligned16(dy), "cvk_wgradp_gemm_sm_dy_wg: dy must be a 16-byte aligned pointer");
+    CVK_CHECK_ARG(W % 4 == 0, "cvk_wgradp_gemm_sm_dy_wg: W=%d must be a multiple of 4 (use cvk_wgradp_gemm_sm_wg with six planes)", W);
+    return wgradp_gemm_go(true, E4p, V6sm, dw, N, H, W, Cin, Cin_ld, Cout, workspace, workspace_bytes, stream, dy, max_workgroups);
 }
 
 extern "C" int cvk_conv3x3_wgradp(const float* x, const float* dy, const float* E6_pre, float* dw, int N, int H, int W, int Cin, int Cin_ld,
diff --git a/pytorch-camvid_amd/csrc/wino2d.hip b/pytorch-camvid_amd/csrc/wino2d.hip
--- a/pytorch-camvid_amd/csrc/wino2d.hip
+++ b/pytorch-camvid_amd/csrc/wino2d.hip
@@ -657,7 +657,7 @@
 template <int ABL = 0>
 __global__ __launch_bounds__(256, 2) void k_w2d_gemm_tn(const float* __restrict__ A, int lda, const float* __restrict__ B, int ldb,
                                                        float* __restrict__ D, int Kp, int Mm, int Nn, int tilesM, int tilesN,
-                                                       int f, int NX) {
+                                                       int f, int NX, int njobs) {
     constexpr int STAGE = 32 * 256 * 4, PPW = 8;
     __shared__ __attribute__((aligned(1024))) char smem[2 * STAGE];
     const unsigned smem_addr = cvk_lds_addr(smem);
@@ -665,80 +665,86 @@
     const int wave = __builtin_amdgcn_readfirstlane(tid >> 6);
     const int r = lane & 31, h = lane >> 5;
     const int wm = wave >> 1, wn = wave & 1;
-    const int id = cvk_xcd_remap(blockIdx.x, gridDim.x);
-    const int part = id % f, tile = id / f;
-    const int tn = tile % tilesN, tm = (tile / tilesN) % tilesM, xi = tile / (tilesN * tilesM);
-    const int nK = Kp / 32, kb = part * nK / f, ke = (part + 1) * nK / f;
-    A += (size_t)xi * Kp * lda + tm * 128;
-    B += (size_t)xi * Kp * ldb + tn * 128;
-    D += ((size_t)part * NX + xi) * Mm * Nn;
-
-    const float* src[PPW];
-    int sstep[PPW];
-#pragma unroll
-    for (int q = 0; q < PPW; ++q) {
-        const int p = wave * PPW + q, pa = p & 15;
-        const int krow = pa * 2 + (lane >> 5), col = (lane & 31) * 4;
-        src[q] = p < 16 ? A + (size_t)krow * lda + col : B + (size_t)krow * ldb + col;
-        sstep[q] = p < 16 ? 32 * lda : 32 * ldb;
-    }
-    auto issue = [&](int ks, int buf) {
-#pragma unroll
-        for (int q = 0; q < PPW; ++q) cvk_dma16(src[q] + (size_t)ks * sstep[q], smem_addr + buf * STAGE + (wave * PPW + q) * 1024);
-    };
-    f32x16 acc[2][2];
-#pragma unroll
-    for (int i = 0; i < 2; ++i)
-#pragma unroll
-        for (int j = 0; j < 2; ++j)
-#pragma unroll
-            for (int e = 0; e < 16; ++e) acc[i][j][e] = 0.f;
-    const int a_off = h * 512 + (wm * 64 + 2 * r) * 4, b_off = 16384 + h * 512 + (wn * 64 + 2 * r) * 4;
-    typedef float f32x2 __attribute__((ext_vector_type(2)));
-
-    if (kb < ke) issue(kb, 0);
-    int buf = 0;
-    for (int ks = kb; ks < ke; ++ks) {
-        if (ABL != 2) cvk_wait_vm<0>();
-        if (ABL != 1) cvk_lds_retire_barrier();
-        const int ksn = ABL == 5 ? kb : min(ks + 1, ke - 1);
-        if (!CVK_TN_SPLIT_ISSUE && ABL != 2) issue(ksn, buf ^ 1);
-        __builtin_amdgcn_s_setprio(1);
-        const char* const st = smem + buf * STAGE;
-#pragma unroll
-        for (int q = 0; q < 16; ++q) {
-            f32x2 a, b;
-            if (ABL == 4) { a = f32x2{acc[0][0][0], 1.f}; b = f32x2{acc[0][0][1], 2.f}; asm volatile("" : "+v"(a), "+v"(b)); }
-            else {
-                a = *reinterpret_cast<const f32x2*>(st + a_off + q * 1024);
-                b = *reinterpret_cast<const f32x2*>(st + b_off + q * 1024);
-            }
-            if (CVK_TN_SPLIT_ISSUE && ABL != 2 && (q == 0 || q == 4)) {
-#pragma unroll
-                for (int p = (q ? PPW / 2 : 0); p < (q ? PPW : PPW / 2); ++p)
-                    cvk_dma16(src[p] + (size_t)ksn * sstep[p], smem_addr + (buf ^ 1) * STAGE + (wave * PPW + p) * 1024);
-            }
-#pragma unroll
-            for (int i = 0; i < 2; ++i)
-#pragma unroll
-                for (int j = 0; j < 2; ++j) acc[i][j] = __builtin_amdgcn_mfma_f32_32x32x2f32(a[i], b[j], acc[i][j], 0, 0, 0);
-        }
-        __builtin_amdgcn_s_setprio(0);
-        buf ^= 1;
-    }
-    cvk_wait_vm<0>();
-    const int col = tn * 128 + wn * 64 + 2 * r;
-#pragma unroll
-    for (int i = 0; i < 2; ++i)
-#pragma unroll
-        for (int e = 0; e < 16; ++e) {
-            const int row = tm * 128 + wm * 64 + 2 * ((e & 3) + 8 * (e >> 2) + 4 * h) + i;
-            if (ABL == 3 ? (row < Mm && acc[i][0][e] == 123.456f) : row < Mm) {
-                float* const dp = D + (size_t)row * Nn + col;
-                if (col + 1 < Nn) { const f32x2 v = {acc[i][0][e], acc[i][1][e]}; *reinterpret_cast<f32x2*>(dp) = v; }
-                else if (col < Nn) dp[0] = acc[i][0][e];
-            }
-        }
+    const float* const A0 = A;
+    const float* const B0 = B;
+    float* const D0 = D;
+    for (int job = blockIdx.x; job < njobs; job += gridDim.x) {
+        if (job != (int)blockIdx.x) cvk_lds_retire_barrier();
+        const int id = cvk_xcd_remap(job, njobs);
+        const int part = id % f, tile = id / f;
+        const int tn = tile % tilesN, tm = (tile / tilesN) % tilesM, xi = tile / (tilesN * tilesM);
+        const int nK = Kp / 32, kb = part * nK / f, ke = (part + 1) * nK / f;
+        A = A0 + (size_t)xi * Kp * lda + tm * 128;
+        B = B0 + (size_t)xi * Kp * ldb + tn * 128;
+        D = D0 + ((size_t)part * NX + xi) * Mm * Nn;
+
+        const float* src[PPW];
+        int sstep[PPW];
+#pragma unroll
+        for (int q = 0; q < PPW; ++q) {
+            const int p = wave * PPW + q, pa = p & 15;
+            const int krow = pa * 2 + (lane >> 5), col = (lane & 31) * 4;
+            src[q] = p < 16 ? A + (size_t)krow * lda + col : B + (size_t)krow * ldb + col;
+            sstep[q] = p < 16 ? 32 * lda : 32 * ldb;
+        }
+        auto issue = [&](int ks, int buf) {
+#pragma unroll
+            for (int q = 0; q < PPW; ++q) cvk_dma16(src[q] + (size_t)ks * sstep[q], smem_addr + buf * STAGE + (wave * PPW + q) * 1024);
+        };
+        f32x16 acc[2][2];
+#pragma unroll
+        for (int i = 0; i < 2; ++i)
+#pragma unroll
+            for (int j = 0; j < 2; ++j)
+#pragma unroll
+                for (int e = 0; e < 16; ++e) acc[i][j][e] = 0.f;
+        const int a_off = h * 512 + (wm * 64 + 2 * r) * 4, b_off = 16384 + h * 512 + (wn * 64 + 2 * r) * 4;
+        typedef float f32x2 __attribute__((ext_vector_type(2)));
+
+        if (kb < ke) issue(kb, 0);
+        int buf = 0;
+        for (int ks = kb; ks < ke; ++ks) {
+            if (ABL != 2) cvk_wait_vm<0>();
+            if (ABL != 1) cvk_lds_retire_barrier();
+            const int ksn = ABL == 5 ? kb : min(ks + 1, ke - 1);
+            if (!CVK_TN_SPLIT_ISSUE && ABL != 2) issue(ksn, buf ^ 1);
+            __builtin_amdgcn_s_setprio(1);
+            const char* const st = smem + buf * STAGE;
+#pragma unroll
+            for (int q = 0; q < 16; ++q) {
+                f32x2 a, b;
+                if (ABL == 4) { a = f32x2{acc[0][0][0], 1.f}; b = f32x2{acc[0][0][1], 2.f}; asm volatile("" : "+v"(a), "+v"(b)); }
+                else {
+                    a = *reinterpret_cast<const f32x2*>(st + a_off + q * 1024);
+                    b = *reinterpret_cast<const f32x2*>(st + b_off + q * 1024);
+                }
+                if (CVK_TN_SPLIT_ISSUE && ABL != 2 && (q == 0 || q == 4)) {
+#pragma unroll
+                    for (int p = (q ? PPW / 2 : 0); p < (q ? PPW : PPW / 2); ++p)
+                        cvk_dma16(src[p] + (size_t)ksn * sstep[p], smem_addr + (buf ^ 1) * STAGE + (wave * PPW + p) * 1024);
+                }
+#pragma unroll
+                for (int i = 0; i < 2; ++i)
+#pragma unroll
+                    for (int j = 0; j < 2; ++j) acc[i][j] = __builtin_amdgcn_mfma_f32_32x32x2f32(a[i], b[j], acc[i][j], 0, 0, 0);
+            }
+            __builtin_amdgcn_s_setprio(0);
+            buf ^= 1;
+        }
+        cvk_wait_vm<0>();
+        const int col = tn * 128 + wn * 64 + 2 * r;
+#pragma unroll
+        for (int i = 0; i < 2; ++i)
+#pragma unroll
+            for (int e = 0; e < 16; ++e) {
+                const int row = tm * 128 + wm * 64 + 2 * ((e & 3) + 8 * (e >> 2) + 4 * h) + i;
+                if (ABL == 3 ? (row < Mm && acc[i][0][e] == 123.456f) : row < Mm) {
+                    float* const dp = D + (size_t)row * Nn + col;
+                    if (col + 1 < Nn) { const f32x2 v = {acc[i][0][e], acc[i][1][e]}; *reinterpret_cast<f32x2*>(dp) = v; }
+                    else if (col < Nn) dp[0] = acc[i][0][e];
+                }
+            }
+    }
 }
 
 template <int MT>
@@ -1058,13 +1064,18 @@
     CVK_LAUNCH_RETURN(who);
 }
 
-static int w2i_gemm_tn(int mt, const char* who, const float* E, const float* V, float* P, int T, int Cin_pad, int Cout, void* stream) {
+static int w2i_gemm_tn(int mt, const char* who, const float* E, const float* V, float* P, int T, int Cin_pad, int Cout, void* stream,
+                       int max_workgroups = 0) {
     CVK_CHECK_ARG(E && V && P && T > 0 && Cin_pad > 0 && Cin_pad % 4 == 0 && Cout > 0 && Cout % 4 == 0, "%s: bad arguments", who);
     CVK_CHECK_ARG(cvk_aligned16(E) && cvk_aligned16(V) && cvk_aligned16(P), "%s: pointers must be 16-byte aligned", who);
+    CVK_CHECK_ARG(max_workgroups >= 0, "%s: max_workgroups must be >= 0", who);
     const int nx = w2_nx(mt);
     const W2WPlan p = plan_w2d_wgrad(nx, T, Cin_pad, Cout);
+    const int njobs = nx * p.tilesM * p.tilesN * p.f;
+    int wgs = njobs;
+    if (max_workgroups > 0 && max_workgroups < njobs) wgs = max_workgroups >= 8 ? max_workgroups / 8 * 8 : max_workgroups;
 #ifdef CVK_EXPERIMENTS
-#define CVK_TN_ABL_GO(A_) hipLaunchKernelGGL(k_w2d_gemm_tn<A_>, dim3(nx * p.tilesM * p.tilesN * p.f), dim3(256), 0, (hipStream_t)stream, E, Cout, V, Cin_pad, P, p.Tpad, Cout, Cin_pad, p.tilesM, p.tilesN, p.f, nx)
+#define CVK_TN_ABL_GO(A_) hipLaunchKernelGGL(k_w2d_gemm_tn<A_>, dim3(wgs), dim3(256), 0, (hipStream_t)stream, E, Cout, V, Cin_pad, P, p.Tpad, Cout, Cin_pad, p.tilesM, p.tilesN, p.f, nx, njobs)
     switch (cvk_knob("CVK_W2D_TN_ABL", 0)) {
         case 1: CVK_TN_ABL_GO(1); CVK_LAUNCH_RETURN(who);
         case 2: CVK_TN_ABL_GO(2); CVK_LAUNCH_RETURN(who);
@@ -1074,8 +1085,8 @@
         default: break;
     }
 #endif
-    hipLaunchKernelGGL(k_w2d_gemm_tn<0>, dim3(nx * p.tilesM * p.tilesN * p.f), dim3(256), 0, (hipStream_t)stream, E, Cout, V, Cin_pad, P, p.Tpad,
-                       Cout, Cin_pad, p.tilesM, p.tilesN, p.f, nx);
+    hipLaunchKernelGGL(k_w2d_gemm_tn<0>, dim3(wgs), dim3(256), 0, (hipStream_t)stream, E, Cout, V, Cin_pad, P, p.Tpad,
+                       Cout, Cin_pad, p.tilesM, p.tilesN, p.f, nx, njobs);
     CVK_LAUNCH_RETURN(who);
 }
 
@@ -1360,6 +1371,9 @@
 extern "C" int cvk_w2d_gemm_tn(const float* E, const float* V, float* P, int T, int Cin_pad, int Cout, void* stream) {
     return w2i_gemm_tn(4, "cvk_w2d_gemm_tn", E, V, P, T, Cin_pad, Cout, stream);
 }
+extern "C" int cvk_w2d_gemm_tn_wg(const float* E, const float* V, float* P, int T, int Cin_pad, int Cout, int max_workgroups, void* stream) {
+    return w2i_gemm_tn(4, "cvk_w2d_gemm_tn_wg", E, V, P, T, Cin_pad, Cout, stream, max_workgroups);
+}
 extern "C" int cvk_w2d_wgrad_output(const float* P, float* dw, int T, int Cin, int Cin_pad, int Cout, void* stream) {
     return w2i_wgrad_output(4, "cvk_w2d_wgrad_output", P, dw, T, Cin, Cin_pad, Cout, stream);
 }
@@ -1415,6 +1429,9 @@
 extern "C" int cvk_w6_gemm_tn(const float* E, const float* V, float* P, int T, int Cin_pad, int Cout, void* stream) {
     return w2i_gemm_tn(6, "cvk_w6_gemm_tn", E, V, P, T, Cin_pad, Cout, stream);
 }
+extern "C" int cvk_w6_gemm_tn_wg(const float* E, const float* V, float* P, int T, int Cin_pad, int Cout, int max_workgroups, void* stream) {
+    return w2i_gemm_tn(6, "cvk_w6_gemm_tn_wg", E, V, P, T, Cin_pad, Cout, stream, max_workgroups);
+}
 extern "C" int cvk_w6_wgrad_output(const float* P, float* dw, int T, int Cin, int Cin_pad, int Cout, void* stream) {
     return w2i_wgrad_output(6, "cvk_w6_wgrad_output", P, dw, T, Cin, Cin_pad, Cout, stream);
 }
diff --git a/pytorch-camvid_amd/engine.py b/pytorch-camvid_amd/engine.py
--- a/pytorch-camvid_amd/engine.py
+++ b/pytorch-camvid_amd/engine.py
@@ -79,6 +79,9 @@
         self.amax_spare = []
         self.scratch = []
         self.fold = None
+        self.side = False
+        self.side_open = False
+        self.side_keep = []
 
 
 def _empty(n, dev, dtype=_F32):
@@ -102,6 +105,8 @@
 WINO4F_DEFAULT = os.environ.get("CVK_WINO4F", "1") != "0"
 WGRADP_DEFAULT = {"0": False, "1": True, "always": "always"}[os.environ.get("CVK_WGRADP", "1")]
 VPLANES_DEFAULT = os.environ.get("CVK_VPLANES", "1") != "0"
+WGRAD_SIDE_DEFAULT = "1"
+WGRAD_SIDE_FAMILIES = frozenset(("wgradp", "wgradp_sm", "w2d", "thin"))
 
 
 def amax_blocks(lib, n, dev):
@@ -519,6 +524,26 @@
         self._pass_token = 0
         self._passes = 0
         self.wcache_builds = 0
+        self.wgrad_side = os.environ.get("CVK_WGRAD_SIDE", WGRAD_SIDE_DEFAULT) != "0"
+        self.side_families = WGRAD_SIDE_FAMILIES
+
+    def side_allowed(self, fold):
+        return (self.wgrad_side and not self.bf16 and self.grad_sync is None and self.accumulator is None and fold is None and PROF is None
+                and not torch.cuda.is_current_stream_capturing())
+
+    def side_begin(self, st, *keep):
+        s = self.lib.cvk_side_begin(st.stream)
+        if not s:
+            check(-1, "cvk_side_begin")
+        st.side_keep.extend(k for k in keep if k is not None)
+        st.side_open = True
+        return s
+
+    def side_join(self, st):
+        if st.side_open:
+            check(self.lib.cvk_side_join(st.stream), "cvk_side_join")
+            st.side_open = False
+            st.side_keep.clear()
 
     def persistent_wgs(self):
         gs = self.grad_sync
@@ -761,11 +786,15 @@
         fold = st.fold = self.accumulator.open_pass(st, plan, total) if self.accumulator is not None else None
         st.sync = self.begin_sync(st, plan, fold)
         self._collectives_in_flight = False
+        st.side = self.side_allowed(fold)
         st.grad[plan.output.buf.id] = self.import_nchw(st, gout, plan.output.buf, _F32, zero_pad=True)
-        for op in reversed(plan.ops):
-            _CUR_OP[0] = (op.idx, "bwd")
-            op.bwd(self, st)
-        _CUR_OP[0] = None
+        try:
+            for op in reversed(plan.ops):
+                _CUR_OP[0] = (op.idx, "bwd")
+                op.bwd(self, st)
+        finally:
+            _CUR_OP[0] = None
+            self.side_join(st)
         self.flush_colsums(st)
         self.flush_wreduces(st)
         if fold is not None and st.sync is None:
```

Measured after the change: 251.0 images/s (median of 6 runs). +1.9%, better.
